# Leonhard111/M3L

Hardware: AMD Instinct MI355X
Metric: MAE fwd+bwd samples/sec (image+tactile) (higher is better)
Workload: dtype bf16; 1 GPU; BASELINE configs[1]: VTT vision+tactile MAE, 64x64 RGB + 2x32x32 tactile, ViT-Tiny 192/12/3/768 + decoder 192/4/3/768, mask 0.75; batch_per_gpu=256, global_batch=256, parallelism=dp1, grad_allreduce=none (one rank), rccl_ranks=0, step=zero_grad + mask + fwd + bwd + grad all-reduce + Adam

## Files before the change

### include/m3l_amd.h

```cpp
#ifndef M3L_AMD_H
#define M3L_AMD_H
#include <stddef.h>
#include <stdint.h>

#ifdef __cplusplus
extern "C" {
#endif

#define M3L_MAX_TACTILES 8

typedef struct m3l_geom {
    int image_h, image_w, image_patch, image_channels;
    int tactile_h, tactile_w, tactile_patch, tactile_channels;
    int num_tactiles;
    int use_vision;
    int use_tactile;
} m3l_geom;

typedef struct m3l_tf_cfg {
    int dim, depth, heads, mlp_dim;
    int project_out;
    int dtype;
    int dim_head;
} m3l_tf_cfg;

typedef struct m3l_dropout {
    float p;
    uint64_t seed;
} m3l_dropout;

int m3l_version(void);
int m3l_last_error(char* buf, size_t n);
int m3l_set_rowln(int enable);
int m3l_set_attn_block(int mode);
int m3l_set_attn_bwd_heads(int mode);
int m3l_set_attn_t192_bwd_prefetch(int mode);
int m3l_set_enc_mega(int mode);
void m3l_set_attn_phase_buffer(void* dev_buf);
int m3l_set_defer_join(int on);
int m3l_set_wgrad_inline(int on);
int m3l_side_join(void* stream);
int m3l_comm_available(void);
int m3l_comm_unique_id(void* out128);
int m3l_comm_init(const void* id128, int rank, int world);
int m3l_comm_world(void);
int m3l_comm_allreduce(float* buf, size_t count, void* after_stream);
int m3l_comm_destroy(void);
int m3l_side_fork(void* after_stream, void** side_out);
int m3l_side_mark_pending(void);
void* m3l_side_stream(void);
int m3l_side_pending(void);
int m3l_set_drop_h(int on);
int m3l_set_t192(int on);
int m3l_set_t192_tt(int tt);
int m3l_set_residual_bf16(int on);
int m3l_set_t192_stagger(int lead_mask, int prio_mask);

int m3l_mask_counts(const m3l_geom* g, double ratio, int* counts_host);
int m3l_mask_sample(const m3l_geom* g, double ratio, int B, const float* const* noise, int64_t* masked, int64_t* unmasked,
                    void* stream);

int m3l_mask_sample_counts(const m3l_geom* g, int nm_img, int nm_tac, int B, const float* const* noise, int64_t* masked,
                           int64_t* unmasked, void* stream);

size_t m3l_embed_ws_bytes(const m3l_geom* g, int D, int dtype, int B, int L);
int m3l_embed_fwd(const m3l_geom* g, int D, int dtype, int B, int L, int cnt_img, const int64_t* idx, const float* image,
                  const float* const* tactiles, const void* const* tensors, void* ws, float* tokens, void* stream);
int m3l_embed_bwd(const m3l_geom* g, int D, int dtype, int B, int L, int cnt_img, const int64_t* idx, const float* image,
                  const float* const* tactiles, const void* const* tensors, void* ws, const float* dtokens, float* const* grads,
                  void* stream);

size_t m3l_transformer_ws_bytes(const m3l_tf_cfg* c, int B, int n);
int m3l_transformer_fwd(const m3l_tf_cfg* c, int B, int n, const float* x_in, const void* const* tensors, void* ws, void* y_t,
                        float* y32, void* stream);
int m3l_transformer_bwd(const m3l_tf_cfg* c, int B, int n, const float* x_in, const void* const* tensors, void* ws, const void* dy,
                        int dy_dtype, float* dx_in, float* const* grads, void* stream);

int m3l_transformer_bwd_range(const m3l_tf_cfg* c, int B, int n, const float* x_in, const void* const* tensors, void* ws,
                              const void* dy, int dy_dtype, float* dx_in, float* const* grads, int layer_hi, int layer_lo, void* stream);

size_t m3l_transformer_ws_bytes_dropout(const m3l_tf_cfg* c, int B, int n, const m3l_dropout* drop);
int m3l_transformer_fwd_dropout(const m3l_tf_cfg* c, int B, int n, const float* x_in, const void* const* tensors, void* ws, void* y_t,
                                float* y32, const m3l_dropout* drop, void* stream);
int m3l_transformer_bwd_dropout(const m3l_tf_cfg* c, int B, int n, const float* x_in, const void* const* tensors, void* ws, const void* dy,
                                int dy_dtype, float* dx_in, float* const* grads, const m3l_dropout* drop, void* stream);
int m3l_transformer_bwd_range_dropout(const m3l_tf_cfg* c, int B, int n, const float* x_in, const void* const* tensors, void* ws,
                                      const void* dy, int dy_dtype, float* dx_in, float* const* grads, int layer_hi, int layer_lo,
                                      const m3l_dropout* drop, void* stream);

enum {
    M3L_TF_PER_OP = 0,
    M3L_TF_BLOCK = 1,
    M3L_TF_T192 = 2,
    M3L_TF_ROWLN = 3,
    M3L_TF_IN_BLOCK = 4,
    M3L_TF_TAIL_T192 = 5,
    M3L_TF_IN_TAIL = 6,
    M3L_TF_GEMM = 7,
    M3L_TF_IDENTITY = 8
};
typedef struct m3l_tf_plan {
    int per_op;
    int rowln_cfg;
    int rowln;
    int rb;
    int drop_h;
    int h_from_u;
    int mega_fwd;
    int mega_bwd;
    int dropout;
    int fwd_attn;
    int fwd_outproj;
    int fwd_mlp;
    int bwd_mlp;
    int bwd_attn;
    int bwd_qkv;
    int row_tiles;
    int qkv_tiles;
    int cs_rows;
} m3l_tf_plan;
int m3l_transformer_plan(const m3l_tf_cfg* c, int B, int n, const m3l_dropout* drop, m3l_tf_plan* out);

size_t m3l_frozen_vit_ws_bytes(const m3l_tf_cfg* c, int B, int n);
int m3l_frozen_vit_fwd(const m3l_tf_cfg* c, float ln_eps, int B, int n, const float* x, const void* const* tensors, void* ws,
                       float* y32, void* stream);

size_t m3l_unshuffle_ws_bytes(const m3l_geom* g, int D, int dd, int dtype, int B, int nvis, int nmask);
int m3l_unshuffle_fwd(const m3l_geom* g, int D, int dd, int dtype, int B, int nvis, int nmask, const int64_t* unmasked,
                      const int64_t* masked, const float* enc32, const void* enc_t, const void* const* tensors, void* ws,
                      float* dec_in, void* stream);
int m3l_unshuffle_bwd(const m3l_geom* g, int D, int dd, int dtype, int B, int nvis, int nmask, const int64_t* unmasked,
                      const int64_t* masked, const void* enc_t, const void* const* tensors, void* ws, const float* d_dec_in,
                      void* d_enc, int* d_enc_dtype, float* const* grads, void* stream);

size_t m3l_heads_ws_bytes(const m3l_geom* g, int dd, int dtype, int B, int nmask);
int m3l_heads_loss_fwd(const m3l_geom* g, int dd, int dtype, int B, int N, int nmask, int nm_img, const int64_t* masked,
                       const float* image, const float* const* tactiles, const void* dec_t, const void* const* tensors, void* ws,
                       float* loss, float* pred_img, float* tgt_img, float* pred_tac, float* tgt_tac, void* stream);
int m3l_heads_loss_fwd2(const m3l_geom* g, int dd, int dtype, int B, int N, int nmask, int nm_img, const int64_t* masked,
                        const float* image, const float* const* tactiles, const void* dec_t, const void* const* tensors, void* ws,
                        float* loss, float* loss_parts, float* pred_img, float* tgt_img, float* pred_tac, float* tgt_tac, void* stream);
int m3l_heads_loss_bwd(const m3l_geom* g, int dd, int dtype, int B, int N, int nmask, int nm_img, const int64_t* masked,
                       const void* const* tensors, void* ws, const float* dloss, void* d_dec, float* const* grads, void* stream);

typedef struct m3l_mae_cfg {
    m3l_geom geom;
    m3l_tf_cfg enc, dec;
    double masking_ratio;
    int early_conv;
    int learned_pos;
} m3l_mae_cfg;
typedef struct m3l_comm_plan {
    float* flat;
    long total, min_bucket;
    int layers_per_chunk, n_stages;
    const long* stage_end;
    long* sent_out;
} m3l_comm_plan;
int m3l_mae_step_num_tensors(const m3l_mae_cfg* c);
size_t m3l_mae_step_ws_bytes(const m3l_mae_cfg* c, int B);
int m3l_mae_step_fwd(const m3l_mae_cfg* c, int B, const float* image, const float* const* tactiles, const float* const* noise,
                     const void* const* tensors, void* ws, float* loss, int64_t* masked, int64_t* unmasked, void* stream);
int m3l_mae_step_bwd(const m3l_mae_cfg* c, int B, const float* image, const float* const* tactiles, const int64_t* masked,
                     const int64_t* unmasked, const void* const* tensors, void* ws, const float* dloss, float* const* grads,
                     const m3l_comm_plan* comm, void* stream);
size_t m3l_mae_step_ws_bytes_dropout(const m3l_mae_cfg* c, int B, const m3l_dropout* enc_drop);
int m3l_mae_step_fwd_dropout(const m3l_mae_cfg* c, int B, const float* image, const float* const* tactiles, const float* const* noise,
                             const void* const* tensors, void* ws, float* loss, int64_t* masked, int64_t* unmasked, const m3l_dropout* enc_drop,
                             void* stream);
int m3l_mae_step_bwd_dropout(const m3l_mae_cfg* c, int B, const float* image, const float* const* tactiles, const int64_t* masked,
                             const int64_t* unmasked, const void* const* tensors, void* ws, const float* dloss, float* const* grads,
                             const m3l_comm_plan* comm, const m3l_dropout* enc_drop, void* stream);

int m3l_extractor_num_tensors(const m3l_mae_cfg* c, const m3l_tf_cfg* head);
size_t m3l_extractor_ws_bytes(const m3l_mae_cfg* c, const m3l_tf_cfg* head, int B);
int m3l_extractor_fwd(const m3l_mae_cfg* c, const m3l_tf_cfg* head, int B, const float* image, const float* const* tactiles,
                      const void* const* tensors, void* ws, float* out, void* stream);
int m3l_extractor_bwd(const m3l_mae_cfg* c, const m3l_tf_cfg* head, int B, const float* image, const float* const* tactiles,
                      const void* const* tensors, void* ws, const float* dout, float* const* grads, void* stream);
size_t m3l_extractor_ws_bytes_dropout(const m3l_mae_cfg* c, const m3l_tf_cfg* head, int B, const m3l_dropout* enc_drop, const m3l_dropout* head_drop);
int m3l_extractor_fwd_dropout(const m3l_mae_cfg* c, const m3l_tf_cfg* head, int B, const float* image, const float* const* tactiles,
                              const void* const* tensors, void* ws, float* out, const m3l_dropout* enc_drop, const m3l_dropout* head_drop,
                              void* stream);
int m3l_extractor_bwd_dropout(const m3l_mae_cfg* c, const m3l_tf_cfg* head, int B, const float* image, const float* const* tactiles,
                              const void* const* tensors, void* ws, const float* dout, float* const* grads, const m3l_dropout* enc_drop,
                              const m3l_dropout* head_drop, void* stream);

typedef struct m3l_cnn_cfg {
    int in_channels, height, width, dim;
    int tactile;
    int dtype;
} m3l_cnn_cfg;
int m3l_set_direct_conv(int on);
size_t m3l_earlycnn_ws_bytes(const m3l_cnn_cfg* c, int B, int nsrc);
int m3l_earlycnn_fwd(const m3l_cnn_cfg* c, int B, int nsrc, const float* const* srcs, const void* const* tensors, void* ws, float* out,
                     void* stream);
int m3l_earlycnn_bwd(const m3l_cnn_cfg* c, int B, int nsrc, const float* const* srcs, const void* const* tensors, void* ws, const float* dout,
                     float* const* grads, void* stream);
size_t m3l_tokens_assemble_ws_bytes(const m3l_geom* g, int D);
int m3l_tokens_assemble_fwd(const m3l_geom* g, int D, int B, const float* img_tok, const float* tac_tok, const void* const* tensors,
                            float* tokens, void* stream);
int m3l_tokens_assemble_bwd(const m3l_geom* g, int D, int B, const float* dtokens, float* d_img, float* d_tac, void* ws, float* dmod,
                            void* stream);

size_t m3l_layernorm_ws_bytes(int D);
int m3l_layernorm_fwd(int out_dtype, const float* x, int M, int D, const float* gamma, const float* beta, float eps, void* y,
                      float* y32, void* stream);
int m3l_layernorm_bwd(int dy_dtype, const void* dy, const float* x, int M, int D, const float* gamma, float eps, const float* dres,
                      float* dx, void* ws, float* dgamma, float* dbeta, void* stream);
int m3l_gather_tokens(const float* src, int B, int N, int D, const int64_t* idx, int K, float* dst, void* stream);
int m3l_scatter_tokens(const float* src, int B, int N, int D, const int64_t* idx, int K, float* dst_zeroed, void* stream);
int m3l_vt_load(const float* image_nhwc, int B, int H, int W, int C, float* image_nchw, const float* tactile, int th, int tw,
                int n_sensors, int frame_stack, float* const* tactile_out, void* stream);
int m3l_vt_load2(const void* image_nhwc, int image_u8, int B, int H, int W, int C, double img_lo, double img_hi, float* image_nchw,
                 const void* tactile, int tactile_u8, int th, int tw, int n_sensors, int frame_stack, double tac_lo, double tac_hi,
                 float* const* tactile_out, void* stream);

int m3l_adam_step(float* params, const float* grads, float* exp_avg, float* exp_avg_sq, long n, float lr, float beta1, float beta2,
                  float eps, float weight_decay, int step, void* stream);
int m3l_adam_step_scaled(float* params, const float* grads, float* exp_avg, float* exp_avg_sq, long n, float lr, float beta1, float beta2,
                         float eps, float weight_decay, int step, float grad_scale, void* stream);
int m3l_adamw_step(float* params, float* grads, float* exp_avg, float* exp_avg_sq, long n, float lr, float beta1, float beta2, float eps,
                   float weight_decay, int step, float grad_scale, float max_grad_norm, float* norm_ws, int scale_grads, void* stream);
int m3l_adam_step_dev(float* params, const float* grads, float* exp_avg, float* exp_avg_sq, long n, float lr, float beta1,
                      float beta2, float eps, float weight_decay, int* step_dev, float* bias_corr_dev, void* stream);
int m3l_dino_opt_step(float* params, float* grads, float* exp_avg, float* exp_avg_sq, float* teacher, long n, const int64_t* seg_start,
                      const int32_t* seg_group, int n_segments, const float* group_lr, const float* group_weight_decay, int n_groups,
                      double beta1, double beta2, float eps, int step, float grad_scale, float max_grad_norm, float* norm_ws, int scale_grads,
                      double ema_beta, void* stream);

void m3l_prof_begin(const char* filter, int stride);
void m3l_prof_end(void);
double m3l_prof_event_overhead_us(void* stream, int n);
int m3l_prof_count(void);
int m3l_prof_get(int i, char* name, size_t n, double* ms_total, long* launches, double* flops_total, double* bytes_total);

int m3l_op_gemm_nt(int dtype, const void* A, int lda, const void* W, int ldw, int M, int N, int K, const float* bias,
                   const float* res, float* out_f32, void* out_t, void* out_pre, const void* gelu_u, int act, int ldc, void* stream);
size_t m3l_op_gemm_tn_ws_bytes(int M, int N, int K);
int m3l_op_gemm_tn(int dtype, const void* Y, int ldy, const void* X, int ldx, int M, int N, int K, void* ws, size_t ws_bytes,
                   float* out, int ldo, void* stream);
int m3l_op_gemm_tn_acc(int dtype, const void* Y, int ldy, const void* X, int ldx, int M, int N, int K, void* ws, size_t ws_bytes, float* out, int ldo,
                       int accumulate, void* stream);
size_t m3l_op_gemm_tn_grouped_ws_bytes(int dtype, int count, int M, const int* N, const int* K);
int m3l_op_gemm_tn_grouped(int dtype, int count, int M, const void* const* Y, const int* ldy, const void* const* X, const int* ldx, const int* N,
                           const int* K, float* const* out, void* ws, size_t ws_bytes, void* stream);
size_t m3l_op_colsum_ws_bytes(int N);
int m3l_op_colsum(int dtype, const void* Y, int M, int N, int ld, void* ws, float* out, void* stream);
int m3l_op_prep_weight(int dtype, const float* src, int rows, int cols, void* dst, void* dstT, void* stream);
int m3l_op_mask_scale(int mode, const float* src, const void* ref, float scale, long count, float* out, void* stream);
int m3l_op_concat2(float* a, int na, float* b, int nb, int rows, float* cat, int split, void* stream);
int m3l_op_patch_cols(int dtype, const float* x, int B, int C, int H, int W, int P, int Kpad, void* col, void* stream);
int m3l_op_vit_tokens(const float* emb, const float* cls, const float* regs, const float* pos, int B, int npatch, int R, int D, float* tok,
                      void* stream);
int m3l_op_attn_fwd(int dtype, const void* qkv, void* o, float* lse, int B, int n, int H, void* stream);
int m3l_op_attn_bwd(int dtype, const void* qkv, const void* o, const void* dO, const float* lse, float* dsum, void* dqkv, int B,
                    int n, int H, void* stream);
int m3l_op_attn_fwd_dh(int dtype, const void* qkv, void* o, float* lse, int B, int n, int H, void* stream, int dim_head);
int m3l_op_attn_bwd_dh(int dtype, const void* qkv, const void* o, const void* dO, const float* lse, float* dsum, void* dqkv, int B,
                       int n, int H, void* stream, int dim_head);
int m3l_op_dropout_mask(float p, uint64_t seed, int layer, int site, long rows, int N, uint8_t* out, void* stream);

int m3l_op_l2norm_fwd(int out_dtype, const float* x, int M, int D, float eps, void* y, float* y32, float* norm, void* stream);
int m3l_op_l2norm_bwd(const float* dy, const float* x, const float* norm, int M, int D, float eps, float* dx, void* stream);
int m3l_op_weightnorm_fwd(int dtype, const float* v, const float* g, int K, int D, void* W, float* vnorm, void* stream);
int m3l_op_weightnorm_bwd(const float* dW, const float* v, const float* g, const float* vnorm, int K, int D, float* dv, float* dg, void* stream);
size_t m3l_op_dino_ws_bytes(int rows, int K);
int m3l_op_dino_rowstats(const float* logits, int rows, int K, const float* center, float inv_temp, void* ws, float* stats, void* stream);
int m3l_op_dino_loss(const float* S, int P, const float* T, int Q, int B, int K, const float* center, float inv_ts, float inv_tt, const float* s_stats,
                     const float* t_stats, void* ws, float* loss, void* stream);
int m3l_op_dino_grad(int out_dtype, const float* S, int P, const float* T, int Q, int B, int K, const float* center, float inv_ts, float inv_tt,
                     const float* s_stats, const float* t_stats, const float* dloss, void* dST, int ldr, void* stream);
int m3l_op_dino_center_sum(const float* T, int rows, int K, float* pending, void* stream);
int m3l_op_dino_center_apply(float* center, const float* pending, int K, float momentum, float one_minus_momentum, float count, void* stream);
int m3l_op_sk_row_splits(int rows, int K);
size_t m3l_op_sk_ws_bytes(int rows, int K);
int m3l_op_sk_colstats(const float* logits, int rows, int K, float inv_temp, const float* row_stats, void* ws, float* col_pairs, void* stream);
int m3l_op_sk_colcombine(const float* parts, int nparts, int K, float temp, float* center_out, void* stream);
int m3l_op_sk_probs(const float* logits, int rows, int K, const float* center, float inv_temp, const float* row_stats, float* probs, void* stream);
size_t m3l_op_koleo_ws_bytes(int groups, int n, int D);
int m3l_op_koleo_fwd(const float* x, int groups, int n, int D, float eps, void* ws, float* y, float* norm, int* nn, long long* nn64, float* dist,
                     float* loss, void* stream);
int m3l_op_koleo_bwd(const float* dloss, const float* x, const float* y, const float* norm, const int* nn, const float* dist, int groups, int n, int D,
                     float eps, float* dx, void* stream);
size_t m3l_op_ibot_ws_bytes(int rows, int K);
int m3l_op_ibot_loss(const float* S, const float* T, int Q, int R, int K, const float* center, float inv_ts, float inv_tt, const float* s_stats,
                     const float* t_stats, void* ws, float* loss, void* stream);
int m3l_op_ibot_grad(int out_dtype, const float* S, const float* T, int Q, int R, int K, const float* center, float inv_ts, float inv_tt,
                     const float* s_stats, const float* t_stats, const float* dloss, void* dST, int ldr, void* stream);
int m3l_op_ibot_center_sum(const float* T, int rows, int K, float scale, void* ws, float* pending, void* stream);
int m3l_op_ema(float* const* dst, const float* const* src, const long* len, int count, float beta, float one_minus_beta, void* stream);

#define M3L_POLICY_MAX_HIDDEN 3
typedef struct m3l_policy_desc {
    int features, actions;
    int n_pi, n_vf;
    int pi_width[M3L_POLICY_MAX_HIDDEN], vf_width[M3L_POLICY_MAX_HIDDEN];
    float* pi_weight[M3L_POLICY_MAX_HIDDEN];
    float* pi_bias[M3L_POLICY_MAX_HIDDEN];
    float* vf_weight[M3L_POLICY_MAX_HIDDEN];
    float* vf_bias[M3L_POLICY_MAX_HIDDEN];
    float* action_weight;
    float* action_bias;
    float* value_weight;
    float* value_bias;
    float* log_std;
} m3l_policy_desc;
size_t m3l_policy_ws_bytes(const m3l_policy_desc* head, int B);
int m3l_policy_act(const m3l_policy_desc* head, int B, const float* x, const float* noise, float* actions, float* values, float* logp, void* stream);
int m3l_policy_eval_fwd(const m3l_policy_desc* head, int B, const float* x, const float* actions, void* ws, float* values, float* logp, float* entropy,
                        void* stream);
int m3l_policy_eval_bwd(const m3l_policy_desc* head, int B, const float* x, const float* actions, const float* dvalues, const float* dlogp,
                        const float* dentropy, void* ws, float* dx, const m3l_policy_desc* grads, void* stream);
int m3l_policy_ppo_loss_fwd(const float* logp, const float* values, const float* entropy, const float* old_logp, const float* advantages, const float* returns,
                            const float* old_values, int B, float clip_range, float clip_range_vf, float ent_coef, float vf_coef, int normalize_advantage,
                            float* loss, float* stats, float* coef_logp, float* coef_values, void* stream);
int m3l_policy_ppo_loss_bwd(const float* dloss, const float* coef_logp, const float* coef_values, int B, float ent_coef, float* dlogp, float* dvalues,
                            float* dentropy, void* stream);

#define M3L_SAC_MAX_HIDDEN 3
typedef struct m3l_sac_desc {
    int features, actions;
    int n_pi, n_qf;
    int pi_width[M3L_SAC_MAX_HIDDEN], qf_width[M3L_SAC_MAX_HIDDEN];
    float* pi_weight[M3L_SAC_MAX_HIDDEN];
    float* pi_bias[M3L_SAC_MAX_HIDDEN];
    float* mu_weight;
    float* mu_bias;
    float* log_std_weight;
    float* log_std_bias;
    float* qf_weight[2][M3L_SAC_MAX_HIDDEN];
    float* qf_bias[2][M3L_SAC_MAX_HIDDEN];
    float* q_weight[2];
    float* q_bias[2];
} m3l_sac_desc;
size_t m3l_sac_ws_bytes(const m3l_sac_desc* head, int B);
int m3l_sac_actor_fwd(const m3l_sac_desc* head, int B, const float* x, const float* noise, void* ws, float* actions, float* logp, void* stream);
int m3l_sac_actor_bwd(const m3l_sac_desc* head, int B, const float* x, const float* noise, const float* dactions, const float* dlogp, void* ws,
                      float* dx, const m3l_sac_desc* grads, void* stream);
int m3l_sac_critic_fwd(const m3l_sac_desc* head, int B, const float* x, const float* actions, void* ws, float* q, void* stream);
int m3l_sac_critic_bwd(const m3l_sac_desc* head, int B, const float* dq, void* ws, float* dactions, const m3l_sac_desc* grads, void* stream);
int m3l_sac_td_target(const m3l_sac_desc* head, int B, const float* x_next, const float* noise, const float* rewards, const float* dones, float gamma,
                      float ent_coef, const float* log_ent_coef, float* target_q, void* stream);
int m3l_sac_critic_loss_fwd(const float* q, const float* target_q, int B, float* loss, float* coef, void* stream);
int m3l_sac_critic_loss_bwd(const float* dloss, const float* coef, int B, float* dq, void* stream);
int m3l_sac_actor_loss_fwd(const float* logp, const float* q, int B, float ent_coef, const float* log_ent_coef, float* loss, float* coef, void* stream);
int m3l_sac_actor_loss_bwd(const float* dloss, const float* coef, int B, float* dlogp_dq, void* stream);
int m3l_sac_ent_coef_loss(const float* log_ent_coef, const float* logp, float target_entropy, int B, const float* dloss, float* loss, float* ent_coef,
                          float* dlog_ent_coef, void* stream);

int m3l_rollout_gather_load(const void* image_store, int image_u8, int H, int W, double img_lo, double img_hi, float* image,
                            const void* tactile_store, int tactile_u8, int th, int tw, int n_sensors, double tac_lo, double tac_hi,
                            float* const* tactile_out, int T, int n_envs, int frame_stack, const int64_t* idx, int B, void* stream);
int m3l_rollout_gather_rows(const float* actions, const float* values, const float* log_probs, const float* advantages, const float* returns, int T,
                            int n_envs, int A, const int64_t* idx, int B, float* actions_out, float* values_out, float* log_probs_out,
                            float* advantages_out, float* returns_out, void* stream);
int m3l_rollout_gae(const float* rewards, const float* values, const float* episode_starts, const float* last_values, const float* dones, int T,
                    int n_envs, float gamma, float gae_lambda, float* advantages, float* returns, void* stream);

int m3l_replay_gather_load(const void* image_store, const void* image_next_store, int image_u8, int H, int W, double img_lo, double img_hi,
                           float* image, float* image_next, const void* tactile_store, const void* tactile_next_store, int tactile_u8, int th, int tw,
                           int n_sensors, double tac_lo, double tac_hi, float* const* tactile_out, float* const* tactile_next_out, int T, int n_envs,
                           int frame_stack, const int64_t* rows, long row_shift, int B, void* stream);
int m3l_replay_gather_rows(const float* actions, const float* rewards, const float* dones, const float* timeouts, int T, int n_envs, int A,
                           const int64_t* rows, long row_shift, int B, float reward_scale, float reward_clip, float* actions_out,
                           float* rewards_out, float* dones_out, int64_t* rows_out, void* stream);

int m3l_replay_gather_load_frames(const void* image_frames, const void* image_next_frames, int image_u8, int H, int W, double img_lo,
                                  double img_hi, float* image, float* image_next, const void* tactile_frames, const void* tactile_next_frames,
                                  int tactile_u8, int th, int tw, int n_sensors, double tac_lo, double tac_hi, float* const* tactile_out,
                                  float* const* tactile_next_out, const int32_t* ages, int T, int n_envs, int frame_stack, const int64_t* rows,
                                  long row_shift, int B, void* stream);

#ifdef __cplusplus
}
#endif
#endif
```

### m3l_amd/_lib.py

```python
import ctypes as C
import os

_HERE = os.path.dirname(os.path.abspath(__file__))
LIB_PATH = os.environ.get("M3L_LIB_PATH") or os.path.join(_HERE, "lib", "libm3l_amd.so")

c_p = C.c_void_p
c_i = C.c_int
c_sz = C.c_size_t


class Geom(C.Structure):
    _fields_ = [(n, c_i) for n in ("image_h", "image_w", "image_patch", "image_channels", "tactile_h", "tactile_w",
                                   "tactile_patch", "tactile_channels", "num_tactiles", "use_vision", "use_tactile")]


class CnnCfg(C.Structure):
    _fields_ = [(n, c_i) for n in ("in_channels", "height", "width", "dim", "tactile", "dtype")]


class TfCfg(C.Structure):
    _fields_ = [(n, c_i) for n in ("dim", "depth", "heads", "mlp_dim", "project_out", "dtype", "dim_head")]


class MaeCfg(C.Structure):
    _fields_ = [("geom", Geom), ("enc", TfCfg), ("dec", TfCfg), ("masking_ratio", C.c_double), ("early_conv", c_i), ("learned_pos", c_i)]


class Dropout(C.Structure):
    _fields_ = [("p", C.c_float), ("seed", C.c_uint64)]


class TfPlan(C.Structure):
    _fields_ = [(n, c_i) for n in ("per_op", "rowln_cfg", "rowln", "rb", "drop_h", "h_from_u", "mega_fwd", "mega_bwd", "dropout",
                                   "fwd_attn", "fwd_outproj", "fwd_mlp", "bwd_mlp", "bwd_attn", "bwd_qkv", "row_tiles", "qkv_tiles", "cs_rows")]


TF_PER_OP, TF_BLOCK, TF_T192, TF_ROWLN, TF_IN_BLOCK, TF_TAIL_T192, TF_IN_TAIL, TF_GEMM, TF_IDENTITY = range(9)


class CommPlan(C.Structure):
    _fields_ = [("flat", c_p), ("total", C.c_long), ("min_bucket", C.c_long), ("layers_per_chunk", c_i), ("n_stages", c_i),
                ("stage_end", C.POINTER(C.c_long)), ("sent_out", C.POINTER(C.c_long))]


class PolicyDesc(C.Structure):
    _fields_ = [("features", c_i), ("actions", c_i), ("n_pi", c_i), ("n_vf", c_i), ("pi_width", c_i * 3), ("vf_width", c_i * 3),
                ("pi_weight", c_p * 3), ("pi_bias", c_p * 3), ("vf_weight", c_p * 3), ("vf_bias", c_p * 3),
                ("action_weight", c_p), ("action_bias", c_p), ("value_weight", c_p), ("value_bias", c_p), ("log_std", c_p)]


class SacDesc(C.Structure):
    _fields_ = [("features", c_i), ("actions", c_i), ("n_pi", c_i), ("n_qf", c_i), ("pi_width", c_i * 3), ("qf_width", c_i * 3),
                ("pi_weight", c_p * 3), ("pi_bias", c_p * 3), ("mu_weight", c_p), ("mu_bias", c_p), ("log_std_weight", c_p), ("log_std_bias", c_p),
                ("qf_weight", (c_p * 3) * 2), ("qf_bias", (c_p * 3) * 2), ("q_weight", c_p * 2), ("q_bias", c_p * 2)]


_SIGS = {
    "m3l_version": (c_i, []),
    "m3l_last_error": (c_i, [C.c_char_p, c_sz]),
    "m3l_set_rowln": (c_i, [c_i]),
    "m3l_set_attn_block": (c_i, [c_i]),
    "m3l_set_attn_phase_buffer": (None, [c_p]),
    "m3l_set_attn_bwd_heads": (c_i, [c_i]),
    "m3l_set_attn_t192_bwd_prefetch": (c_i, [c_i]),
    "m3l_set_enc_mega": (c_i, [c_i]),
    "m3l_set_drop_h": (c_i, [c_i]),
    "m3l_set_direct_conv": (c_i, [c_i]),
    "m3l_set_t192": (c_i, [c_i]),
    "m3l_set_t192_tt": (c_i, [c_i]),
    "m3l_set_t192_stagger": (c_i, [c_i, c_i]),
    "m3l_set_residual_bf16": (c_i, [c_i]),
    "m3l_set_defer_join": (c_i, [c_i]),
    "m3l_set_wgrad_inline": (c_i, [c_i]),
    "m3l_side_join": (c_i, [c_p]),
    "m3l_side_stream": (c_p, []),
    "m3l_side_fork": (c_i, [c_p, C.POINTER(c_p)]),
    "m3l_side_mark_pending": (c_i, []),
    "m3l_comm_available": (c_i, []),
    "m3l_comm_unique_id": (c_i, [c_p]),
    "m3l_comm_init": (c_i, [c_p, c_i, c_i]),
    "m3l_comm_world": (c_i, []),
    "m3l_comm_allreduce": (c_i, [c_p, c_sz, c_p]),
    "m3l_comm_destroy": (c_i, []),
    "m3l_side_pending": (c_i, []),
    "m3l_mask_counts": (c_i, [C.POINTER(Geom), C.c_double, C.POINTER(c_i)]),
    "m3l_mask_sample": (c_i, [C.POINTER(Geom), C.c_double, c_i, c_p, c_p, c_p, c_p]),
    "m3l_mask_sample_counts": (c_i, [C.POINTER(Geom), c_i, c_i, c_i, c_p, c_p, c_p, c_p]),
    "m3l_embed_ws_bytes": (c_sz, [C.POINTER(Geom), c_i, c_i, c_i, c_i]),
    "m3l_embed_fwd": (c_i, [C.POINTER(Geom), c_i, c_i, c_i, c_i, c_i, c_p, c_p, c_p, c_p, c_p, c_p, c_p]),
    "m3l_embed_bwd": (c_i, [C.POINTER(Geom), c_i, c_i, c_i, c_i, c_i, c_p, c_p, c_p, c_p, c_p, c_p, c_p, c_p]),
    "m3l_transformer_ws_bytes": (c_sz, [C.POINTER(TfCfg), c_i, c_i]),
    "m3l_transformer_fwd": (c_i, [C.POINTER(TfCfg), c_i, c_i, c_p, c_p, c_p, c_p, c_p, c_p]),
    "m3l_transformer_bwd": (c_i, [C.POINTER(TfCfg), c_i, c_i, c_p, c_p, c_p, c_p, c_i, c_p, c_p, c_p]),
    "m3l_transformer_bwd_range": (c_i, [C.POINTER(TfCfg), c_i, c_i, c_p, c_p, c_p, c_p, c_i, c_p, c_p, c_i, c_i, c_p]),
    "m3l_transformer_ws_bytes_dropout": (c_sz, [C.POINTER(TfCfg), c_i, c_i, C.POINTER(Dropout)]),
    "m3l_transformer_fwd_dropout": (c_i, [C.POINTER(TfCfg), c_i, c_i, c_p, c_p, c_p, c_p, c_p, C.POINTER(Dropout), c_p]),
    "m3l_transformer_bwd_dropout": (c_i, [C.POINTER(TfCfg), c_i, c_i, c_p, c_p, c_p, c_p, c_i, c_p, c_p, C.POINTER(Dropout), c_p]),
    "m3l_transformer_bwd_range_dropout": (c_i, [C.POINTER(TfCfg), c_i, c_i, c_p, c_p, c_p, c_p, c_i, c_p, c_p, c_i, c_i, C.POINTER(Dropout), c_p]),
    "m3l_transformer_plan": (c_i, [C.POINTER(TfCfg), c_i, c_i, C.POINTER(Dropout), C.POINTER(TfPlan)]),
    "m3l_frozen_vit_ws_bytes": (c_sz, [C.POINTER(TfCfg), c_i, c_i]),
    "m3l_frozen_vit_fwd": (c_i, [C.POINTER(TfCfg), C.c_float, c_i, c_i, c_p, c_p, c_p, c_p, c_p]),
    "m3l_unshuffle_ws_bytes": (c_sz, [C.POINTER(Geom), c_i, c_i, c_i, c_i, c_i, c_i]),
    "m3l_unshuffle_fwd": (c_i, [C.POINTER(Geom), c_i, c_i, c_i, c_i, c_i, c_i, c_p, c_p, c_p, c_p, c_p, c_p, c_p, c_p]),
    "m3l_unshuffle_bwd": (c_i, [C.POINTER(Geom), c_i, c_i, c_i, c_i, c_i, c_i, c_p, c_p, c_p, c_p, c_p, c_p, c_p,
                                C.POINTER(c_i), c_p, c_p]),
    "m3l_heads_ws_bytes": (c_sz, [C.POINTER(Geom), c_i, c_i, c_i, c_i]),
    "m3l_heads_loss_fwd": (c_i, [C.POINTER(Geom), c_i, c_i, c_i, c_i, c_i, c_i, c_p, c_p, c_p, c_p, c_p, c_p, c_p, c_p, c_p,
                                 c_p, c_p, c_p]),
    "m3l_heads_loss_fwd2": (c_i, [C.POINTER(Geom), c_i, c_i, c_i, c_i, c_i, c_i, c_p, c_p, c_p, c_p, c_p, c_p, c_p, c_p, c_p,
                                  c_p, c_p, c_p, c_p]),
    "m3l_heads_loss_bwd": (c_i, [C.POINTER(Geom), c_i, c_i, c_i, c_i, c_i, c_i, c_p, c_p, c_p, c_p, c_p, c_p, c_p]),
    "m3l_mae_step_num_tensors": (c_i, [C.POINTER(MaeCfg)]),
    "m3l_mae_step_ws_bytes": (c_sz, [C.POINTER(MaeCfg), c_i]),
    "m3l_mae_step_fwd": (c_i, [C.POINTER(MaeCfg), c_i, c_p, c_p, c_p, c_p, c_p, c_p, c_p, c_p, c_p]),
    "m3l_mae_step_bwd": (c_i, [C.POINTER(MaeCfg), c_i, c_p, c_p, c_p, c_p, c_p, c_p, c_p, c_p, C.POINTER(CommPlan), c_p]),
    "m3l_mae_step_ws_bytes_dropout": (c_sz, [C.POINTER(MaeCfg), c_i, C.POINTER(Dropout)]),
    "m3l_mae_step_fwd_dropout": (c_i, [C.POINTER(MaeCfg), c_i, c_p, c_p, c_p, c_p, c_p, c_p, c_p, c_p, C.POINTER(Dropout), c_p]),
    "m3l_mae_step_bwd_dropout": (c_i, [C.POINTER(MaeCfg), c_i, c_p, c_p, c_p, c_p, c_p, c_p, c_p, c_p, C.POINTER(CommPlan), C.POINTER(Dropout), c_p]),
    "m3l_extractor_num_tensors": (c_i, [C.POINTER(MaeCfg), C.POINTER(TfCfg)]),
    "m3l_extractor_ws_bytes": (c_sz, [C.POINTER(MaeCfg), C.POINTER(TfCfg), c_i]),
    "m3l_extractor_fwd": (c_i, [C.POINTER(MaeCfg), C.POINTER(TfCfg), c_i, c_p, c_p, c_p, c_p, c_p, c_p]),
    "m3l_extractor_bwd": (c_i, [C.POINTER(MaeCfg), C.POINTER(TfCfg), c_i, c_p, c_p, c_p, c_p, c_p, c_p, c_p]),
    "m3l_extractor_ws_bytes_dropout": (c_sz, [C.POINTER(MaeCfg), C.POINTER(TfCfg), c_i, C.POINTER(Dropout), C.POINTER(Dropout)]),
    "m3l_extractor_fwd_dropout": (c_i, [C.POINTER(MaeCfg), C.POINTER(TfCfg), c_i, c_p, c_p, c_p, c_p, c_p, C.POINTER(Dropout), C.POINTER(Dropout), c_p]),
    "m3l_extractor_bwd_dropout": (c_i, [C.POINTER(MaeCfg), C.POINTER(TfCfg), c_i, c_p, c_p, c_p, c_p, c_p, c_p, C.POINTER(Dropout), C.POINTER(Dropout), c_p]),
    "m3l_earlycnn_ws_bytes": (c_sz, [C.POINTER(CnnCfg), c_i, c_i]),
    "m3l_earlycnn_fwd": (c_i, [C.POINTER(CnnCfg), c_i, c_i, c_p, c_p, c_p, c_p, c_p]),
    "m3l_earlycnn_bwd": (c_i, [C.POINTER(CnnCfg), c_i, c_i, c_p, c_p, c_p, c_p, c_p, c_p]),
    "m3l_tokens_assemble_ws_bytes": (c_sz, [C.POINTER(Geom), c_i]),
    "m3l_tokens_assemble_fwd": (c_i, [C.POINTER(Geom), c_i, c_i, c_p, c_p, c_p, c_p, c_p]),
    "m3l_tokens_assemble_bwd": (c_i, [C.POINTER(Geom), c_i, c_i, c_p, c_p, c_p, c_p, c_p, c_p]),
    "m3l_layernorm_ws_bytes": (c_sz, [c_i]),
    "m3l_layernorm_fwd": (c_i, [c_i, c_p, c_i, c_i, c_p, c_p, C.c_float, c_p, c_p, c_p]),
    "m3l_layernorm_bwd": (c_i, [c_i, c_p, c_p, c_i, c_i, c_p, C.c_float, c_p, c_p, c_p, c_p, c_p, c_p]),
    "m3l_gather_tokens": (c_i, [c_p, c_i, c_i, c_i, c_p, c_i, c_p, c_p]),
    "m3l_scatter_tokens": (c_i, [c_p, c_i, c_i, c_i, c_p, c_i, c_p, c_p]),
    "m3l_vt_load": (c_i, [c_p, c_i, c_i, c_i, c_i, c_p, c_p, c_i, c_i, c_i, c_i, c_p, c_p]),
    "m3l_vt_load2": (c_i, [c_p, c_i, c_i, c_i, c_i, c_i, C.c_double, C.c_double, c_p, c_p, c_i, c_i, c_i, c_i, c_i, C.c_double, C.c_double, c_p, c_p]),
    "m3l_adam_step_dev": (c_i, [c_p, c_p, c_p, c_p, C.c_long, C.c_float, C.c_float, C.c_float, C.c_float, C.c_float, c_p, c_p, c_p]),
    "m3l_adamw_step": (c_i, [c_p, c_p, c_p, c_p, C.c_long, C.c_float, C.c_float, C.c_float, C.c_float, C.c_float, c_i, C.c_float, C.c_float, c_p, c_i, c_p]),
    "m3l_adam_step": (c_i, [c_p, c_p, c_p, c_p, C.c_long, C.c_float, C.c_float, C.c_float, C.c_float, C.c_float, c_i, c_p]),
    "m3l_adam_step_scaled": (c_i, [c_p, c_p, c_p, c_p, C.c_long, C.c_float, C.c_float, C.c_float, C.c_float, C.c_float, c_i, C.c_float, c_p]),
    "m3l_dino_opt_step": (c_i, [c_p, c_p, c_p, c_p, c_p, C.c_long, c_p, c_p, c_i, C.POINTER(C.c_float), C.POINTER(C.c_float), c_i,
                                C.c_double, C.c_double, C.c_float, c_i, C.c_float, C.c_float, c_p, c_i, C.c_double, c_p]),
    "m3l_prof_begin": (None, [C.c_char_p, c_i]),
    "m3l_prof_end": (None, []),
    "m3l_prof_event_overhead_us": (C.c_double, [c_p, c_i]),
    "m3l_prof_count": (c_i, []),
    "m3l_prof_get": (c_i, [c_i, C.c_char_p, c_sz, C.POINTER(C.c_double), C.POINTER(C.c_long), C.POINTER(C.c_double),
                           C.POINTER(C.c_double)]),
    "m3l_op_gemm_nt": (c_i, [c_i, c_p, c_i, c_p, c_i, c_i, c_i, c_i, c_p, c_p, c_p, c_p, c_p, c_p, c_i, c_i, c_p]),
    "m3l_op_gemm_tn_ws_bytes": (c_sz, [c_i, c_i, c_i]),
    "m3l_op_gemm_tn": (c_i, [c_i, c_p, c_i, c_p, c_i, c_i, c_i, c_i, c_p, c_sz, c_p, c_i, c_p]),
    "m3l_op_gemm_tn_acc": (c_i, [c_i, c_p, c_i, c_p, c_i, c_i, c_i, c_i, c_p, c_sz, c_p, c_i, c_i, c_p]),
    "m3l_op_gemm_tn_grouped_ws_bytes": (c_sz, [c_i, c_i, c_i, c_p, c_p]),
    "m3l_op_gemm_tn_grouped": (c_i, [c_i, c_i, c_i, c_p, c_p, c_p, c_p, c_p, c_p, c_p, c_p, c_sz, c_p]),
    "m3l_op_colsum_ws_bytes": (c_sz, [c_i]),
    "m3l_op_colsum": (c_i, [c_i, c_p, c_i, c_i, c_i, c_p, c_p, c_p]),
    "m3l_op_prep_weight": (c_i, [c_i, c_p, c_i, c_i, c_p, c_p, c_p]),
    "m3l_op_mask_scale": (c_i, [c_i, c_p, c_p, C.c_float, C.c_long, c_p, c_p]),
    "m3l_op_concat2": (c_i, [c_p, c_i, c_p, c_i, c_i, c_p, c_i, c_p]),
    "m3l_op_patch_cols": (c_i, [c_i, c_p, c_i, c_i, c_i, c_i, c_i, c_i, c_p, c_p]),
    "m3l_op_vit_tokens": (c_i, [c_p, c_p, c_p, c_p, c_i, c_i, c_i, c_i, c_p, c_p]),
    "m3l_op_attn_fwd": (c_i, [c_i, c_p, c_p, c_p, c_i, c_i, c_i, c_p]),
    "m3l_op_attn_bwd": (c_i, [c_i, c_p, c_p, c_p, c_p, c_p, c_p, c_i, c_i, c_i, c_p]),
    "m3l_op_attn_fwd_dh": (c_i, [c_i, c_p, c_p, c_p, c_i, c_i, c_i, c_p, c_i]),
    "m3l_op_attn_bwd_dh": (c_i, [c_i, c_p, c_p, c_p, c_p, c_p, c_p, c_i, c_i, c_i, c_p, c_i]),
    "m3l_op_dropout_mask": (c_i, [C.c_float, C.c_uint64, c_i, c_i, C.c_long, c_i, c_p, c_p]),
    "m3l_op_l2norm_fwd": (c_i, [c_i, c_p, c_i, c_i, C.c_float, c_p, c_p, c_p, c_p]),
    "m3l_op_l2norm_bwd": (c_i, [c_p, c_p, c_p, c_i, c_i, C.c_float, c_p, c_p]),
    "m3l_op_weightnorm_fwd": (c_i, [c_i, c_p, c_p, c_i, c_i, c_p, c_p, c_p]),
    "m3l_op_weightnorm_bwd": (c_i, [c_p, c_p, c_p, c_p, c_i, c_i, c_p, c_p, c_p]),
    "m3l_op_dino_ws_bytes": (c_sz, [c_i, c_i]),
    "m3l_op_dino_rowstats": (c_i, [c_p, c_i, c_i, c_p, C.c_float, c_p, c_p, c_p]),
    "m3l_op_dino_loss": (c_i, [c_p, c_i, c_p, c_i, c_i, c_i, c_p, C.c_float, C.c_float, c_p, c_p, c_p, c_p, c_p]),
    "m3l_op_dino_grad": (c_i, [c_i, c_p, c_i, c_p, c_i, c_i, c_i, c_p, C.c_float, C.c_float, c_p, c_p, c_p, c_p, c_i, c_p]),
    "m3l_op_dino_center_sum": (c_i, [c_p, c_i, c_i, c_p, c_p]),
    "m3l_op_dino_center_apply": (c_i, [c_p, c_p, c_i, C.c_float, C.c_float, C.c_float, c_p]),
    "m3l_op_sk_row_splits": (c_i, [c_i, c_i]),
    "m3l_op_sk_ws_bytes": (c_sz, [c_i, c_i]),
    "m3l_op_sk_colstats": (c_i, [c_p, c_i, c_i, C.c_float, c_p, c_p, c_p, c_p]),
    "m3l_op_sk_colcombine": (c_i, [c_p, c_i, c_i, C.c_float, c_p, c_p]),
    "m3l_op_sk_probs": (c_i, [c_p, c_i, c_i, c_p, C.c_float, c_p, c_p, c_p]),
    "m3l_op_koleo_ws_bytes": (c_sz, [c_i, c_i, c_i]),
    "m3l_op_koleo_fwd": (c_i, [c_p, c_i, c_i, c_i, C.c_float, c_p, c_p, c_p, c_p, c_p, c_p, c_p, c_p]),
    "m3l_op_koleo_bwd": (c_i, [c_p, c_p, c_p, c_p, c_p, c_p, c_i, c_i, c_i, C.c_float, c_p, c_p]),
    "m3l_op_ibot_ws_bytes": (c_sz, [c_i, c_i]),
    "m3l_op_ibot_loss": (c_i, [c_p, c_p, c_i, c_i, c_i, c_p, C.c_float, C.c_float, c_p, c_p, c_p, c_p, c_p]),
    "m3l_op_ibot_grad": (c_i, [c_i, c_p, c_p, c_i, c_i, c_i, c_p, C.c_float, C.c_float, c_p, c_p, c_p, c_p, c_i, c_p]),
    "m3l_op_ibot_center_sum": (c_i, [c_p, c_i, c_i, C.c_float, c_p, c_p, c_p]),
    "m3l_op_ema": (c_i, [c_p, c_p, c_p, c_i, C.c_float, C.c_float, c_p]),
    "m3l_policy_ws_bytes": (c_sz, [C.POINTER(PolicyDesc), c_i]),
    "m3l_policy_act": (c_i, [C.POINTER(PolicyDesc), c_i, c_p, c_p, c_p, c_p, c_p, c_p]),
    "m3l_policy_eval_fwd": (c_i, [C.POINTER(PolicyDesc), c_i, c_p, c_p, c_p, c_p, c_p, c_p, c_p]),
    "m3l_policy_eval_bwd": (c_i, [C.POINTER(PolicyDesc), c_i, c_p, c_p, c_p, c_p, c_p, c_p, c_p, C.POINTER(PolicyDesc), c_p]),
    "m3l_policy_ppo_loss_fwd": (c_i, [c_p, c_p, c_p, c_p, c_p, c_p, c_p, c_i, C.c_float, C.c_float, C.c_float, C.c_float, c_i, c_p, c_p, c_p, c_p, c_p]),
    "m3l_policy_ppo_loss_bwd": (c_i, [c_p, c_p, c_p, c_i, C.c_float, c_p, c_p, c_p, c_p]),
    "m3l_sac_ws_bytes": (c_sz, [C.POINTER(SacDesc), c_i]),
    "m3l_sac_actor_fwd": (c_i, [C.POINTER(SacDesc), c_i, c_p, c_p, c_p, c_p, c_p, c_p]),
    "m3l_sac_actor_bwd": (c_i, [C.POINTER(SacDesc), c_i, c_p, c_p, c_p, c_p, c_p, c_p, C.POINTER(SacDesc), c_p]),
    "m3l_sac_critic_fwd": (c_i, [C.POINTER(SacDesc), c_i, c_p, c_p, c_p, c_p, c_p]),
    "m3l_sac_critic_bwd": (c_i, [C.POINTER(SacDesc), c_i, c_p, c_p, c_p, C.POINTER(SacDesc), c_p]),
    "m3l_sac_td_target": (c_i, [C.POINTER(SacDesc), c_i, c_p, c_p, c_p, c_p, C.c_float, C.c_float, c_p, c_p, c_p]),
    "m3l_sac_critic_loss_fwd": (c_i, [c_p, c_p, c_i, c_p, c_p, c_p]),
    "m3l_sac_critic_loss_bwd": (c_i, [c_p, c_p, c_i, c_p, c_p]),
    "m3l_sac_actor_loss_fwd": (c_i, [c_p, c_p, c_i, C.c_float, c_p, c_p, c_p, c_p]),
    "m3l_sac_actor_loss_bwd": (c_i, [c_p, c_p, c_i, c_p, c_p]),
    "m3l_sac_ent_coef_loss": (c_i, [c_p, c_p, C.c_float, c_i, c_p, c_p, c_p, c_p, c_p]),
    "m3l_rollout_gather_load": (c_i, [c_p, c_i, c_i, c_i, C.c_double, C.c_double, c_p, c_p, c_i, c_i, c_i, c_i, C.c_double, C.c_double, c_p,
                                      c_i, c_i, c_i, c_p, c_i, c_p]),
    "m3l_rollout_gather_rows": (c_i, [c_p, c_p, c_p, c_p, c_p, c_i, c_i, c_i, c_p, c_i, c_p, c_p, c_p, c_p, c_p, c_p]),
    "m3l_rollout_gae": (c_i, [c_p, c_p, c_p, c_p, c_p, c_i, c_i, C.c_float, C.c_float, c_p, c_p, c_p]),
    "m3l_replay_gather_load": (c_i, [c_p, c_p, c_i, c_i, c_i, C.c_double, C.c_double, c_p, c_p, c_p, c_p, c_i, c_i, c_i, c_i, C.c_double, C.c_double,
                                     c_p, c_p, c_i, c_i, c_i, c_p, C.c_long, c_i, c_p]),
    "m3l_replay_gather_rows": (c_i, [c_p, c_p, c_p, c_p, c_i, c_i, c_i, c_p, C.c_long, c_i, C.c_float, C.c_float, c_p, c_p, c_p, c_p, c_p]),
    "m3l_replay_gather_load_frames": (c_i, [c_p, c_p, c_i, c_i, c_i, C.c_double, C.c_double, c_p, c_p, c_p, c_p, c_i, c_i, c_i, c_i, C.c_double,
                                            C.c_double, c_p, c_p, c_p, c_i, c_i, c_i, c_p, C.c_long, c_i, c_p]),
}

EXPORTS = tuple(_SIGS.keys())
_lib = None


class M3LError(RuntimeError):
    pass


def lib():
    global _lib
    if _lib is None:
        if not os.path.exists(LIB_PATH):
            raise M3LError(
                f"{LIB_PATH} not found: the HIP extension has not been built. Run "
                "`python -c \"import __graft_entry__ as g; g.build()\"` (needs hipcc, --offload-arch=gfx950). "
                "m3l_amd has no CPU / eager fallback.")
        l = C.CDLL(LIB_PATH)
        for name, (res, args) in _SIGS.items():
            fn = getattr(l, name)
            fn.restype = res
            fn.argtypes = args
        _lib = l
    return _lib


def last_error() -> str:
    buf = C.create_string_buffer(512)
    lib().m3l_last_error(buf, 512)
    return buf.value.decode("utf-8", "replace")


def check(rc: int, what: str):
    if rc != 0:
        raise M3LError(f"{what} failed (code {rc}): {last_error()}")


def ptr(t):
    return None if t is None else t.data_ptr()


def ptr_array(tensors):
    arr = (c_p * max(1, len(tensors)))()
    for i, t in enumerate(tensors):
        arr[i] = None if t is None else t.data_ptr()
    return arr
```

### m3l_amd/csrc/elementwise.hip

```cpp
#include "common.cuh"
#include "kernels.h"
#include <cstring>
#include <vector>

namespace {

constexpr int MAXV = 16;
constexpr int WPB = 4;

__device__ __forceinline__ void store_val(float* p, float v) { *p = v; }
__device__ __forceinline__ void store_val(bf16* p, float v) { *p = (bf16)v; }


template <typename TO> __device__ __forceinline__ void store4(TO* p, f32x4 v);
template <> __device__ __forceinline__ void store4<float>(float* p, f32x4 v) { *reinterpret_cast<f32x4*>(p) = v; }
template <> __device__ __forceinline__ void store4<bf16>(bf16* p, f32x4 v) {
    bf16x4 o;
    o[0] = (bf16)v[0]; o[1] = (bf16)v[1]; o[2] = (bf16)v[2]; o[3] = (bf16)v[3];
    *reinterpret_cast<bf16x4*>(p) = o;
}
__device__ __forceinline__ f32x4 load4(const float* p) { return *reinterpret_cast<const f32x4*>(p); }
__device__ __forceinline__ f32x4 load4(const bf16* p) {
    const bf16x4 v = *reinterpret_cast<const bf16x4*>(p);
    return f32x4{(float)v[0], (float)v[1], (float)v[2], (float)v[3]};
}

template <int MAXC, typename TX>
__device__ __forceinline__ void row_stats(const TX* xr, int D, int lane, f32x4 (&v)[MAXC], float eps, float& mean, float& rstd) {
    float s = 0.f;
#pragma unroll
    for (int i = 0; i < MAXC; ++i) {
        const int e = 4 * (lane + 64 * i);
        v[i] = load4(xr + min(e, D - 4));
        if (e >= D) v[i] = f32x4{0.f, 0.f, 0.f, 0.f};
        s += (v[i][0] + v[i][1]) + (v[i][2] + v[i][3]);
    }
    mean = wave_sum(s) / D;
    float q = 0.f;
#pragma unroll
    for (int i = 0; i < MAXC; ++i) {
        const int e = 4 * (lane + 64 * i);
        if (e < D) {
            const f32x4 d = v[i] - mean;
            q += (d[0] * d[0] + d[1] * d[1]) + (d[2] * d[2] + d[3] * d[3]);
        }
    }
    rstd = rsqrtf(wave_sum(q) / D + eps);
}

template <typename TO, int MAXC, typename TX>
__global__ __launch_bounds__(256) void ln_fwd_kernel(const TX* __restrict__ x, int M, int D, const float* __restrict__ gamma,
                                                       const float* __restrict__ beta, float eps, TO* __restrict__ y,
                                                       float* __restrict__ y32) {
    const int lane = threadIdx.x & 63, row = blockIdx.x * WPB + (threadIdx.x >> 6);
    if (row >= M) return;
    f32x4 v[MAXC], gm[MAXC], bt[MAXC];
#pragma unroll
    for (int i = 0; i < MAXC; ++i) {
        const int ec = min(4 * (lane + 64 * i), D - 4);
        gm[i] = load4(gamma + ec);
        bt[i] = load4(beta + ec);
    }
    float mean, rstd;
    row_stats<MAXC>(x + (long)row * D, D, lane, v, eps, mean, rstd);
#pragma unroll
    for (int i = 0; i < MAXC; ++i) {
        const int e = 4 * (lane + 64 * i);
        if (e < D) {
            const f32x4 r = (v[i] - mean) * rstd * gm[i] + bt[i];
            if (y) store4<TO>(y + (long)row * D + e, r);
            if (y32) store4<float>(y32 + (long)row * D + e, r);
        }
    }
}

template <typename TD, typename TC, int MAXC, typename TX>
__global__ __launch_bounds__(256) void ln_bwd_kernel(const TD* __restrict__ dy, const TX* __restrict__ x, int M, int D,
                                                       const float* __restrict__ gamma, float eps, const float* __restrict__ dres,
                                                       float* __restrict__ dx_out, TC* __restrict__ dx_t_out, float* __restrict__ part) {
    __shared__ __attribute__((aligned(16))) float red[WPB][3][256];
    const int lane = threadIdx.x & 63, wave = threadIdx.x >> 6;
    f32x4 dg[MAXC], db[MAXC], dc[MAXC];
#pragma unroll
    for (int i = 0; i < MAXC; ++i) dg[i] = db[i] = dc[i] = f32x4{0.f, 0.f, 0.f, 0.f};
    f32x4 gm[MAXC];
#pragma unroll
    for (int i = 0; i < MAXC; ++i) gm[i] = load4(gamma + min(4 * (lane + 64 * i), D - 4));
    for (int row = blockIdx.x * WPB + wave; row < M; row += gridDim.x * WPB) {
        f32x4 v[MAXC], gdy[MAXC], dyv[MAXC], rs[MAXC];
        const TD* dyr = dy + (long)row * D;
#pragma unroll
        for (int i = 0; i < MAXC; ++i) {
            const int ec = min(4 * (lane + 64 * i), D - 4);
            dyv[i] = load4(dyr + ec);
            rs[i] = dres ? load4(reinterpret_cast<const TX*>(dres) + (long)row * D + ec) : f32x4{0.f, 0.f, 0.f, 0.f};
        }
        float mean, rstd;
        row_stats<MAXC>(x + (long)row * D, D, lane, v, eps, mean, rstd);
        float s1 = 0.f, s2 = 0.f;
#pragma unroll
        for (int i = 0; i < MAXC; ++i) {
            const int e = 4 * (lane + 64 * i);
            if (e < D) {
                const f32x4 xh = (v[i] - mean) * rstd;
                const f32x4 d = dyv[i];
                dg[i] += d * xh;
                db[i] += d;
                const f32x4 gd = d * gm[i];
                gdy[i] = gd;
                v[i] = xh;
                s1 += (gd[0] + gd[1]) + (gd[2] + gd[3]);
                const f32x4 t = gd * xh;
                s2 += (t[0] + t[1]) + (t[2] + t[3]);
            }
        }
        s1 = wave_sum(s1) / D;
        s2 = wave_sum(s2) / D;
#pragma unroll
        for (int i = 0; i < MAXC; ++i) {
            const int e = 4 * (lane + 64 * i);
            if (e < D) {
                f32x4 r = (gdy[i] - s1 - v[i] * s2) * rstd;
                if (dres) r += rs[i];
                dc[i] += r;
                if (dx_out) store4<float>(dx_out + (long)row * D + e, r);
                if (dx_t_out) store4<TC>(dx_t_out + (long)row * D + e, r);
            }
        }
    }
    float* out = part + (long)blockIdx.x * 3 * D;
#pragma unroll
    for (int i = 0; i < MAXC; ++i) {
        if (256 * i >= D) break;
        *reinterpret_cast<f32x4*>(&red[wave][0][4 * lane]) = dg[i];
        *reinterpret_cast<f32x4*>(&red[wave][1][4 * lane]) = db[i];
        *reinterpret_cast<f32x4*>(&red[wave][2][4 * lane]) = dc[i];
        __syncthreads();
        const int e = 256 * i + threadIdx.x;
        if (e < D) {
#pragma unroll
            for (int k = 0; k < 3; ++k)
                out[k * D + e] = (red[0][k][threadIdx.x] + red[1][k][threadIdx.x]) + (red[2][k][threadIdx.x] + red[3][k][threadIdx.x]);
        }
        __syncthreads();
    }
}

__device__ __forceinline__ void reduce_cols_32x32(const float* __restrict__ p, int G, int stride, int j, bool valid,
                                                  float* __restrict__ out, int accumulate) {
    __shared__ float red[32][33];
    const int cl = threadIdx.x & 31, sl = threadIdx.x >> 5;
    float s = 0.f;
    if (valid) {
        float a[8] = {0.f, 0.f, 0.f, 0.f, 0.f, 0.f, 0.f, 0.f};
        int g = sl;
        for (; g + 224 < G; g += 256) {
#pragma unroll
            for (int u = 0; u < 8; ++u) a[u] += p[(long)(g + 32 * u) * stride + j];
        }
        for (; g < G; g += 32) a[0] += p[(long)g * stride + j];
        s = ((a[0] + a[1]) + (a[2] + a[3])) + ((a[4] + a[5]) + (a[6] + a[7]));
    }
    red[sl][cl] = s;
    __syncthreads();
    if (sl == 0 && valid) {
        float t = red[0][cl];
#pragma unroll
        for (int i = 1; i < 32; ++i) t += red[i][cl];
        out[j] = accumulate ? out[j] + t : t;
    }
}

__global__ __launch_bounds__(1024) void reduce_rows_kernel(const float* __restrict__ part, int G, int stride, int count,
                                                             float* __restrict__ out, int accumulate) {
    const int j = blockIdx.x * 32 + (threadIdx.x & 31);
    reduce_cols_32x32(part, G, stride, j, j < count, out, accumulate);
}

__global__ __launch_bounds__(1024) void reduce_vec_kernel(const float* __restrict__ v, int G, float* __restrict__ out, int accumulate) {
    __shared__ float red[16];
    float a0 = 0.f, a1 = 0.f, a2 = 0.f, a3 = 0.f;
    int i = threadIdx.x;
    for (; i + 3072 < G; i += 4096) { a0 += v[i]; a1 += v[i + 1024]; a2 += v[i + 2048]; a3 += v[i + 3072]; }
    for (; i < G; i += 1024) a0 += v[i];
    float s = wave_sum((a0 + a1) + (a2 + a3));
    if ((threadIdx.x & 63) == 0) red[threadIdx.x >> 6] = s;
    __syncthreads();
    if (threadIdx.x == 0) {
        float t = 0.f;
#pragma unroll
        for (int w = 0; w < 16; ++w) t += red[w];
        out[0] = accumulate ? out[0] + t : t;
    }
}

struct ReduceSegs { float* out[4]; };
__global__ __launch_bounds__(1024) void reduce_rows_seg_kernel(const float* __restrict__ part, int G, int stride, int width,
                                                                 ReduceSegs segs, int accumulate) {
    float* out = segs.out[blockIdx.y];
    if (!out) return;
    const int j = blockIdx.x * 32 + (threadIdx.x & 31);
    reduce_cols_32x32(part + (long)blockIdx.y * width, G, stride, j, j < width, out, accumulate);
}

__global__ __launch_bounds__(1024) void reduce_rows_batch_kernel(ReduceBatch b, int accumulate) {
    const ReduceBatchItem it = b.it[blockIdx.z];
    float* out = it.out[blockIdx.y];
    if (!out) return;
    const int j = blockIdx.x * 32 + (threadIdx.x & 31);
    reduce_cols_32x32(it.part + (long)blockIdx.y * b.D, it.G, 3 * b.D, j, j < b.D, out, accumulate);
}

template <typename T> struct Vec4;
template <> struct Vec4<bf16> { typedef bf16x4 type; };
template <> struct Vec4<float> { typedef f32x4 type; };
template <typename T>
__global__ __launch_bounds__(256) void colsum_kernel(const T* __restrict__ Y, int M, int N, int ld, int rows_per_block,
                                                       float* __restrict__ part, int vec_ok) {
    typedef typename Vec4<T>::type V4;
    const int r0 = blockIdx.x * rows_per_block, r1 = min(M, r0 + rows_per_block);
    for (int c = threadIdx.x * 4; c < N; c += 1024) {
        if (vec_ok && c + 4 <= N) {
            f32x4 s0 = f32x4{0.f, 0.f, 0.f, 0.f}, s1 = s0, s2 = s0, s3 = s0;
            auto ld4 = [&](int r) {
                const V4 v = *reinterpret_cast<const V4*>(Y + (long)r * ld + c);
                return f32x4{to_f32(v[0]), to_f32(v[1]), to_f32(v[2]), to_f32(v[3])};
            };
            int r = r0;
            for (; r + 3 < r1; r += 4) {
                s0 += ld4(r);
                s1 += ld4(r + 1);
                s2 += ld4(r + 2);
                s3 += ld4(r + 3);
            }
            for (; r < r1; ++r) s0 += ld4(r);
            *reinterpret_cast<f32x4*>(part + (long)blockIdx.x * N + c) = (s0 + s1) + (s2 + s3);
        } else {
            for (int cc = c; cc < min(N, c + 4); ++cc) {
                float s0 = 0.f, s1 = 0.f, s2 = 0.f, s3 = 0.f;
                int r = r0;
                for (; r + 3 < r1; r += 4) {
                    s0 += to_f32(Y[(long)r * ld + cc]);
                    s1 += to_f32(Y[(long)(r + 1) * ld + cc]);
                    s2 += to_f32(Y[(long)(r + 2) * ld + cc]);
                    s3 += to_f32(Y[(long)(r + 3) * ld + cc]);
                }
                for (; r < r1; ++r) s0 += to_f32(Y[(long)r * ld + cc]);
                part[(long)blockIdx.x * N + cc] = (s0 + s1) + (s2 + s3);
            }
        }
    }
}

template <typename T>
__global__ __launch_bounds__(256) void prep_weights_kernel(WeightPack pack) {
    __shared__ float tile[64][65];
    int m = 0;
    while (m + 1 < pack.count && (int)blockIdx.x >= pack.tile0[m + 1]) ++m;
    const WeightDesc d = pack.d[m];
    const int tcols = (d.cols + 63) >> 6;
    const int t = blockIdx.x - pack.tile0[m];
    const int r0 = (t / tcols) << 6, c0 = (t % tcols) << 6;
    const int tid = threadIdx.x, q = tid & 15, p = tid >> 4;
    T* dst = reinterpret_cast<T*>(d.dst);
    T* dstT = reinterpret_cast<T*>(d.dstT);
    const bool vec_in = (d.cols & 3) == 0 && (reinterpret_cast<uintptr_t>(d.src) & 15) == 0;
#pragma unroll
    for (int k = 0; k < 4; ++k) {
        const int r = r0 + p + 16 * k, c = c0 + 4 * q;
        float v[4] = {0.f, 0.f, 0.f, 0.f};
        if (r < d.rows) {
            if (vec_in && c + 3 < d.cols) {
                const float4 f = *reinterpret_cast<const float4*>(d.src + (long)r * d.cols + c);
                v[0] = f.x; v[1] = f.y; v[2] = f.z; v[3] = f.w;
            } else {
#pragma unroll
                for (int j = 0; j < 4; ++j)
                    if (c + j < d.cols) v[j] = d.src[(long)r * d.cols + c + j];
            }
        }
        if (dst && r < d.ld_dstT) {
#pragma unroll
            for (int j = 0; j < 4; ++j)
                if (c + j < d.ld_dst) dst[(long)r * d.ld_dst + c + j] = from_f32<T>(v[j]);
        }
#pragma unroll
        for (int j = 0; j < 4; ++j) tile[p + 16 * k][4 * q + j] = v[j];
    }
    if (!dstT) return;
    __syncthreads();
#pragma unroll
    for (int k = 0; k < 4; ++k) {
        const int c = c0 + p + 16 * k, r = r0 + 4 * q;
        if (c >= d.ld_dst) continue;
#pragma unroll
        for (int j = 0; j < 4; ++j)
            if (r + j < d.ld_dstT) dstT[(long)c * d.ld_dstT + r + j] = from_f32<T>(tile[4 * q + j][p + 16 * k]);
    }
}

template <typename T>
__global__ void axpy_t_kernel(const float* __restrict__ x, const T* __restrict__ o, long count, float* __restrict__ out) {
    const long i = (long)blockIdx.x * blockDim.x + threadIdx.x;
    if (i < count) out[i] = x[i] + to_f32(o[i]);
}
template <typename T>
__global__ void cast_kernel(const float* __restrict__ x, long count, T* __restrict__ out) {
    const long i = (long)blockIdx.x * blockDim.x + threadIdx.x;
    if (i < count) out[i] = from_f32<T>(x[i]);
}

template <typename T>
__global__ void scale_by_dev_kernel(const T* __restrict__ x, long count, const float* __restrict__ s, T* __restrict__ out) {
    const long i = (long)blockIdx.x * blockDim.x + threadIdx.x;
    if (i < count) out[i] = from_f32<T>(to_f32(x[i]) * s[0]);
}

template <int MODE>
__global__ void mask_scale_kernel(const float* __restrict__ src, const void* __restrict__ ref, float scale, long count, float* __restrict__ out) {
    const long i = (long)blockIdx.x * blockDim.x + threadIdx.x;
    if (i >= count) return;
    const bool on = MODE == 0 ? reinterpret_cast<const uint8_t*>(ref)[i] != 0 : reinterpret_cast<const float*>(ref)[i] > 0.f;
    out[i] = on ? src[i] * scale : 0.f;
}
__global__ void vit_tokens_kernel(const float* __restrict__ emb, const float* __restrict__ cls, const float* __restrict__ regs,
                                  const float* __restrict__ pos, int B, int npatch, int R, int D, float* __restrict__ tok) {
    const long i = (long)blockIdx.x * blockDim.x + threadIdx.x;
    const int n = 1 + R + npatch;
    if (i >= (long)B * n * D) return;
    const int d = (int)(i % D), t = (int)((i / D) % n), b = (int)(i / ((long)D * n));
    float v;
    if (t == 0) v = cls[d] + pos[d];
    else if (t <= R) v = regs[(long)(t - 1) * D + d];
    else v = emb[((long)b * npatch + (t - 1 - R)) * D + d] + pos[(long)(t - R) * D + d];
    tok[i] = v;
}
__global__ void concat2_kernel(const float* __restrict__ a, int na, const float* __restrict__ b2, int nb, int rows, float* __restrict__ dst, int split) {
    const long i = (long)blockIdx.x * blockDim.x + threadIdx.x;
    const int w = na + nb;
    if (i >= (long)rows * w) return;
    const int r = (int)(i / w), c = (int)(i % w);
    if (!split) dst[i] = c < na ? a[(long)r * na + c] : b2[(long)r * nb + c - na];
    else if (c < na) const_cast<float*>(a)[(long)r * na + c] = dst[i];
    else if (b2) const_cast<float*>(b2)[(long)r * nb + c - na] = dst[i];
}

template <typename T>
__global__ void im2col_kernel(ConvSrc cs, int Bsrc, int Ci, int H, int W, int KH, int S, int P, int OH, int OW, int Kpad,
                              long total, T* __restrict__ col) {
    const long idx = (long)blockIdx.x * blockDim.x + threadIdx.x;
    if (idx >= total) return;
    const int k = (int)(idx % Kpad);
    const long r = idx / Kpad;
    const int ow = (int)(r % OW), oh = (int)((r / OW) % OH);
    const int b = (int)(r / ((long)OW * OH));
    float v = 0.f;
    if (k < Ci * KH * KH) {
        const int kw = k % KH, kh = (k / KH) % KH, ci = k / (KH * KH);
        const int ih = oh * S + kh - P, iw = ow * S + kw - P;
        if (ih >= 0 && ih < H && iw >= 0 && iw < W) {
            if (cs.nchw) {
                const float* src = reinterpret_cast<const float*>(cs.src[b / Bsrc]);
                v = src[(((long)(b % Bsrc) * Ci + ci) * H + ih) * W + iw];
            } else {
                v = to_f32(reinterpret_cast<const T*>(cs.src[0])[(((long)b * H + ih) * W + iw) * Ci + ci]);
            }
        }
    }
    col[idx] = from_f32<T>(v);
}

__global__ __launch_bounds__(256) void im2col4_bf16_kernel(ConvSrc cs, int Bsrc, int Ci, int H, int W, int S, int P, int OH, int OW, long total,
                                                           bf16* __restrict__ col) {
    const long idx = (long)blockIdx.x * blockDim.x + threadIdx.x;
    if (idx >= total) return;
    const int ci = (int)(idx % Ci);
    const long r = idx / Ci;
    const int ow = (int)(r % OW), oh = (int)((r / OW) % OH);
    const int b = (int)(r / ((long)OW * OH));
    bf16x8 out[2];
#pragma unroll
    for (int kh = 0; kh < 4; ++kh) {
        const int ih = oh * S + kh - P;
        const bool rok = ih >= 0 && ih < H;
#pragma unroll
        for (int kw = 0; kw < 4; ++kw) {
            const int iw = ow * S + kw - P;
            float v = 0.f;
            if (rok && iw >= 0 && iw < W) {
                if (cs.nchw) v = reinterpret_cast<const float*>(cs.src[b / Bsrc])[(((long)(b % Bsrc) * Ci + ci) * H + ih) * W + iw];
                else v = (float)reinterpret_cast<const bf16*>(cs.src[0])[(((long)b * H + ih) * W + iw) * Ci + ci];
            }
            out[kh >> 1][(kh & 1) * 4 + kw] = (bf16)v;
        }
    }
    bf16x8* dst = reinterpret_cast<bf16x8*>(col + (r * Ci + ci) * 16);
    dst[0] = out[0];
    dst[1] = out[1];
}

template <typename T>
__global__ void col2im_relu_kernel(const T* __restrict__ dcol, int Btot, int Ci, int H, int W, int KH, int S, int P, int OH, int OW,
                                   int Kpad, const T* __restrict__ act, T* __restrict__ dX) {
    const long idx = (long)blockIdx.x * blockDim.x + threadIdx.x;
    if (idx >= (long)Btot * H * W * Ci) return;
    const int ci = (int)(idx % Ci);
    const long pix = idx / Ci;
    const int iw = (int)(pix % W), ih = (int)((pix / W) % H);
    const int b = (int)(pix / ((long)W * H));
    float s = 0.f;
    if (to_f32(act[idx]) > 0.f) {
        for (int kh = 0; kh < KH; ++kh) {
            const int t = ih + P - kh;
            if (t < 0 || t % S) continue;
            const int oh = t / S;
            if (oh >= OH) continue;
            for (int kw = 0; kw < KH; ++kw) {
                const int u = iw + P - kw;
                if (u < 0 || u % S) continue;
                const int ow = u / S;
                if (ow >= OW) continue;
                s += to_f32(dcol[(((long)b * OH + oh) * OW + ow) * Kpad + (ci * KH + kh) * KH + kw]);
            }
        }
    }
    dX[idx] = from_f32<T>(s);
}

__global__ __launch_bounds__(256) void tokens_assemble_kernel(const float* __restrict__ img_tok, const float* __restrict__ tac_tok, int B,
                                                                int D, int n_img, int n_tac, int k, const float* __restrict__ mod,
                                                                const float* __restrict__ pos_img, const float* __restrict__ pos_tac,
                                                                float* __restrict__ tokens) {
    const int lane = threadIdx.x & 63;
    const long r = (long)blockIdx.x * WPB + (threadIdx.x >> 6);
    const int N = n_img + k * n_tac;
    if (r >= (long)B * N) return;
    const int b = (int)(r / N), pos = (int)(r % N);
    const float *src, *prow;
    int m;
    if (pos < n_img) {
        src = img_tok + ((long)b * n_img + pos) * D;
        prow = pos_img + (long)pos * D;
        m = 0;
    } else {
        const int local = pos - n_img, s = local / n_tac, p = local % n_tac;
        src = tac_tok + (((long)s * B + b) * n_tac + p) * D;
        prow = pos_tac + (long)local * D;
        m = 1 + s;
    }
    float* out = tokens + r * D;
    for (int e = lane; e < D; e += 64) out[e] = src[e] + mod[(long)m * D + e] + prow[e];
}
__global__ __launch_bounds__(256) void tokens_assemble_bwd_kernel(const float* __restrict__ dtok, int B, int D, int n_img, int n_tac, int k,
                                                                    float* __restrict__ d_img, float* __restrict__ d_tac,
                                                                    float* __restrict__ part) {
    extern __shared__ float sm[];
    const int lane = threadIdx.x & 63, wave = threadIdx.x >> 6;
    const int N = n_img + k * n_tac, PL = (1 + k) * D;
    for (int i = threadIdx.x; i < WPB * PL; i += 256) sm[i] = 0.f;
    __syncthreads();
    float* my = sm + wave * PL;
    for (long r = (long)blockIdx.x * WPB + wave; r < (long)B * N; r += (long)gridDim.x * WPB) {
        const int b = (int)(r / N), pos = (int)(r % N);
        float* dst;
        int m;
        if (pos < n_img) {
            dst = d_img + ((long)b * n_img + pos) * D;
            m = 0;
        } else {
            const int local = pos - n_img, s = local / n_tac, p = local % n_tac;
            dst = d_tac + (((long)s * B + b) * n_tac + p) * D;
            m = 1 + s;
        }
        const float* g = dtok + r * D;
        for (int e = lane; e < D; e += 64) {
            const float d = g[e];
            dst[e] = d;
            my[m * D + e] += d;
        }
    }
    __syncthreads();
    for (int i = threadIdx.x; i < PL; i += 256)
        part[(long)blockIdx.x * PL + i] = sm[i] + sm[PL + i] + sm[2 * PL + i] + sm[3 * PL + i];
}

template <int DEC>
__device__ __forceinline__ void adam_elem(float& p, float& g, float& m, float& v, float gscale, float lr, float omb1, float b2, float omb2,
                                          float eps, float wd, float bc1, float bc2_sqrt) {
    g = g * gscale;
    if (DEC) p = p * wd;
    const float gr = DEC ? g : g + wd * p;
    m = m + (gr - m) * omb1;
    v = v * b2 + omb2 * gr * gr;
    const float denom = sqrtf(v) / bc2_sqrt + eps;
    p = p - (lr / bc1) * (m / denom);
}

template <int DEC>
__global__ void adam_flat_kernel(float* __restrict__ p, float* __restrict__ g, float* __restrict__ m, float* __restrict__ v,
                                 long n, float lr, float b1, float b2, float eps, float wd, float bc1, float bc2_sqrt,
                                 const float* __restrict__ bc_dev, float gscale, const float* __restrict__ clip_dev, int scale_g) {
    const long i = ((long)blockIdx.x * blockDim.x + threadIdx.x) * 4;
    if (i >= n) return;
    if (bc_dev) {
        bc1 = bc_dev[0];
        bc2_sqrt = bc_dev[1];
    }
    if (clip_dev) gscale *= clip_dev[0];
    if (i + 4 <= n) {
        f32x4 pp = *reinterpret_cast<f32x4*>(p + i), gg = *reinterpret_cast<const f32x4*>(g + i);
        f32x4 mm = *reinterpret_cast<f32x4*>(m + i), vv = *reinterpret_cast<f32x4*>(v + i);
#pragma unroll
        for (int j = 0; j < 4; ++j) {
// ... 338 lines not shown
                    }
                }
                dg[k] += d[k] * (a - mean) * rstd;
                db[k] += d[k];
            }
        }
        __syncthreads();
    }
    float* out = part + (long)blockIdx.x * 2 * pd;
#pragma unroll
    for (int pass = 0; pass < 2; ++pass) {
#pragma unroll
        for (int k = 0; k < NC; ++k) *reinterpret_cast<f32x4*>(my + 4 * (lane + 64 * k)) = pass ? db[k] : dg[k];
        __syncthreads();
        for (int e = threadIdx.x; e < pd; e += 256) out[pass * pd + e] = buf[0][e] + buf[1][e] + buf[2][e] + buf[3][e];
        __syncthreads();
    }
}

__global__ __launch_bounds__(256) void embed_finalize_kernel(const float* __restrict__ E, int rows, int D, PatchGroup pg,
                                                               const int64_t* __restrict__ idx, int idx_ld, int j0, int cnt,
                                                               const float* __restrict__ gamma, const float* __restrict__ beta,
                                                               float eps, const float* __restrict__ mod, int mod0,
                                                               const float* __restrict__ pos, float* __restrict__ tokens, int L) {
    const int lane = threadIdx.x & 63, row = blockIdx.x * WPB + (threadIdx.x >> 6);
    if (row >= rows) return;
    int b, s, ph, pw, local;
    patch_locate(pg, idx, idx_ld, j0, cnt, row, b, s, ph, pw, local);
    const float* xr = E + (long)row * D;
    float v[MAXV];
    float sum = 0.f;
#pragma unroll
    for (int i = 0; i < MAXV; ++i) {
        const int e = lane + 64 * i;
        v[i] = (e < D) ? xr[e] : 0.f;
        sum += v[i];
    }
    const float mean = wave_sum(sum) / D;
    float q = 0.f;
#pragma unroll
    for (int i = 0; i < MAXV; ++i) {
        const int e = lane + 64 * i;
        const float d = (e < D) ? v[i] - mean : 0.f;
        q += d * d;
    }
    const float rstd = rsqrtf(wave_sum(q) / D + eps);
    const int jj = row % cnt;
    float* out = tokens + ((long)b * L + j0 + jj) * D;
    const float* mrow = mod + (long)(mod0 + s) * D;
    const float* prow = pos + (long)local * D;
#pragma unroll
    for (int i = 0; i < MAXV; ++i) {
        const int e = lane + 64 * i;
        if (e < D) out[e] = (v[i] - mean) * rstd * gamma[e] + beta[e] + mrow[e] + prow[e];
    }
}

template <typename T>
__global__ __launch_bounds__(256) void embed_finalize_bwd_kernel(const float* __restrict__ dtok, int L, const float* __restrict__ E,
                                                                   int rows, int D, PatchGroup pg, const int64_t* __restrict__ idx,
                                                                   int idx_ld, int j0, int cnt, const float* __restrict__ gamma,
                                                                   float eps, T* __restrict__ dE, float* __restrict__ part, int nslot) {
    extern __shared__ float sm[];
    const int lane = threadIdx.x & 63, wave = threadIdx.x >> 6;
    const int PL = (2 + nslot) * D;
    for (int i = threadIdx.x; i < WPB * PL; i += 256) sm[i] = 0.f;
    __syncthreads();
    float* my = sm + wave * PL;
    for (int row = blockIdx.x * WPB + wave; row < rows; row += gridDim.x * WPB) {
        int b, s, ph, pw, local;
        patch_locate(pg, idx, idx_ld, j0, cnt, row, b, s, ph, pw, local);
        const int jj = row % cnt;
        const float* xr = E + (long)row * D;
        const float* dyr = dtok + ((long)b * L + j0 + jj) * D;
        float v[MAXV], gdy[MAXV];
        float sum = 0.f;
#pragma unroll
        for (int i = 0; i < MAXV; ++i) {
            const int e = lane + 64 * i;
            v[i] = (e < D) ? xr[e] : 0.f;
            sum += v[i];
        }
        const float mean = wave_sum(sum) / D;
        float q = 0.f;
#pragma unroll
        for (int i = 0; i < MAXV; ++i) {
            const int e = lane + 64 * i;
            const float d = (e < D) ? v[i] - mean : 0.f;
            q += d * d;
        }
        const float rstd = rsqrtf(wave_sum(q) / D + eps);
        float s1 = 0.f, s2 = 0.f;
#pragma unroll
        for (int i = 0; i < MAXV; ++i) {
            const int e = lane + 64 * i;
            if (e < D) {
                const float xh = (v[i] - mean) * rstd;
                const float d = dyr[e];
                my[e] += d * xh;
                my[D + e] += d;
                my[(2 + s) * D + e] += d;
                const float gd = d * gamma[e];
                gdy[i] = gd;
                v[i] = xh;
                s1 += gd;
                s2 += gd * xh;
            } else {
                gdy[i] = 0.f;
                v[i] = 0.f;
            }
        }
        s1 = wave_sum(s1) / D;
        s2 = wave_sum(s2) / D;
#pragma unroll
        for (int i = 0; i < MAXV; ++i) {
            const int e = lane + 64 * i;
            if (e < D) dE[(long)row * D + e] = from_f32<T>(rstd * (gdy[i] - s1 - v[i] * s2));
        }
    }
    __syncthreads();
    for (int i = threadIdx.x; i < PL; i += 256)
        part[(long)blockIdx.x * PL + i] = sm[i] + sm[PL + i] + sm[2 * PL + i] + sm[3 * PL + i];
}

template <typename TO>
__global__ __launch_bounds__(256) void unshuffle_fwd_kernel(const float* __restrict__ src, const float* __restrict__ mask_token,
                                                              const int64_t* __restrict__ unmasked, int nvis,
                                                              const int64_t* __restrict__ masked, int nmask, int B, int dd,
                                                              int n_img, int n_tac, const float* __restrict__ dmod,
                                                              const float* __restrict__ pos_img, const float* __restrict__ pos_tac,
                                                              TO* __restrict__ dec_in) {
    const int lane = threadIdx.x & 63;
    const long r = (long)blockIdx.x * WPB + (threadIdx.x >> 6);
    const int N = nvis + nmask;
    if (r >= (long)B * N) return;
    const int b = (int)(r / N), j = (int)(r % N);
    const bool vis = j < nvis;
    const int pos = (int)(vis ? unmasked[(long)b * nvis + j] : masked[(long)b * nmask + j - nvis]);
    const float* s = vis ? src + ((long)b * nvis + j) * dd : mask_token;
    const int m = pos < n_img ? 0 : 1 + (pos - n_img) / n_tac;
    const float* prow = pos < n_img ? pos_img + (long)pos * dd : pos_tac + (long)(pos - n_img) * dd;
    TO* out = dec_in + ((long)b * N + pos) * dd;
    const float* mrow = dmod + (long)m * dd;
    for (int e = 4 * lane; e < dd; e += 256) store4<TO>(out + e, load4(s + e) + load4(mrow + e) + load4(prow + e));
}

template <int MAXC, typename TI>
__global__ __launch_bounds__(256) void unshuffle_bwd_kernel(const TI* __restrict__ dY, const int64_t* __restrict__ unmasked, int nvis,
                                                              int B, int N, int dd, int n_img, int n_tac, int nmod, int rows_per_wave,
                                                              int vis_per_wave, float* __restrict__ dsrc, float* __restrict__ part) {
    extern __shared__ float sm[];
    const int lane = threadIdx.x & 63, wave = threadIdx.x >> 6;
    const int PL = (1 + nmod) * dd;
    for (int i = threadIdx.x; i < WPB * PL; i += 256) sm[i] = 0.f;
    __syncthreads();
    float* my = sm + wave * PL;
    const long gw = (long)blockIdx.x * WPB + wave;
    f32x4 acc[MAXC];
#pragma unroll
    for (int c = 0; c < MAXC; ++c) acc[c] = f32x4{0.f, 0.f, 0.f, 0.f};
#define UNSH_FLUSH(slot, sign)                                                      \
    _Pragma("unroll") for (int c = 0; c < MAXC; ++c) {                              \
        const int e4 = (lane + 64 * c) * 4;                                         \
        if (e4 < dd) {                                                              \
            _Pragma("unroll") for (int q = 0; q < 4; ++q) {                         \
                my[e4 + q] += (sign) * acc[c][q];                                   \
                if ((slot) >= 0) my[(1 + (slot)) * dd + e4 + q] += acc[c][q];       \
            }                                                                       \
        }                                                                           \
        acc[c] = f32x4{0.f, 0.f, 0.f, 0.f};                                         \
    }
    const long total = (long)B * N;
    const long r0 = gw * rows_per_wave, r1 = r0 + rows_per_wave < total ? r0 + rows_per_wave : total;
    for (long r = r0; r < r1;) {
        const int pos = (int)(r % N);
        const int m = pos < n_img ? 0 : 1 + (pos - n_img) / n_tac;
        const int pos_end = pos < n_img ? n_img : min(N, n_img + m * n_tac);
        const long seg_end = min(r1, r - pos + pos_end);
        for (; r + 4 <= seg_end; r += 4) {
#pragma unroll
            for (int c = 0; c < MAXC; ++c) {
                const int e4 = (lane + 64 * c) * 4;
                if (e4 < dd) {
                    const TI* g = dY + r * dd + e4;
                    const f32x4 d0 = load4(g), d1 = load4(g + dd), d2 = load4(g + 2 * dd), d3 = load4(g + 3 * dd);
#pragma unroll
                    for (int q = 0; q < 4; ++q) acc[c][q] += (d0[q] + d1[q]) + (d2[q] + d3[q]);
                }
            }
        }
        for (; r < seg_end; ++r) {
#pragma unroll
            for (int c = 0; c < MAXC; ++c) {
                const int e4 = (lane + 64 * c) * 4;
                if (e4 < dd) {
                    const f32x4 d = load4(dY + r * dd + e4);
                    acc[c][0] += d[0]; acc[c][1] += d[1]; acc[c][2] += d[2]; acc[c][3] += d[3];
                }
            }
        }
        { UNSH_FLUSH(m, 1.f) }
    }
    const long vtotal = (long)B * nvis;
    const long v0 = gw * vis_per_wave, v1 = v0 + vis_per_wave < vtotal ? v0 + vis_per_wave : vtotal;
    long v = v0;
    for (; v + 4 <= v1; v += 4) {
        const TI* g[4];
#pragma unroll
        for (int u = 0; u < 4; ++u) g[u] = dY + ((long)((v + u) / nvis) * N + (int)unmasked[v + u]) * dd;
#pragma unroll
        for (int c = 0; c < MAXC; ++c) {
            const int e4 = (lane + 64 * c) * 4;
            if (e4 < dd) {
                f32x4 d[4];
#pragma unroll
                for (int u = 0; u < 4; ++u) d[u] = load4(g[u] + e4);
#pragma unroll
                for (int u = 0; u < 4; ++u) *reinterpret_cast<f32x4*>(dsrc + (v + u) * dd + e4) = d[u];
#pragma unroll
                for (int q = 0; q < 4; ++q) acc[c][q] += (d[0][q] + d[1][q]) + (d[2][q] + d[3][q]);
            }
        }
    }
    for (; v < v1; ++v) {
        const int b = (int)(v / nvis);
        const int pos = (int)unmasked[v];
        const TI* g = dY + ((long)b * N + pos) * dd;
#pragma unroll
        for (int c = 0; c < MAXC; ++c) {
            const int e4 = (lane + 64 * c) * 4;
            if (e4 < dd) {
                const f32x4 d = load4(g + e4);
                *reinterpret_cast<f32x4*>(dsrc + v * dd + e4) = d;
                acc[c][0] += d[0]; acc[c][1] += d[1]; acc[c][2] += d[2]; acc[c][3] += d[3];
            }
        }
    }
    { UNSH_FLUSH(-1, -1.f) }
#undef UNSH_FLUSH
    __syncthreads();
    for (int i = threadIdx.x; i < PL; i += 256)
        part[(long)blockIdx.x * PL + i] = sm[i] + sm[PL + i] + sm[2 * PL + i] + sm[3 * PL + i];
}

template <typename T>
__global__ __launch_bounds__(256) void gather_rows_kernel(const T* __restrict__ src, int N, int D, const int64_t* __restrict__ idx,
                                                            int idx_ld, int j0, int cnt, int rows, T* __restrict__ dst) {
    const int lane = threadIdx.x & 63, row = blockIdx.x * WPB + (threadIdx.x >> 6);
    if (row >= rows) return;
    const int b = row / cnt, jj = row % cnt;
    const long pos = idx[(long)b * idx_ld + j0 + jj];
    const T* s = src + ((long)b * N + pos) * D;
    T* d = dst + (long)row * D;
    for (int e = lane; e < D; e += 64) d[e] = s[e];
}
template <typename T>
__global__ __launch_bounds__(256) void scatter_rows_kernel(const T* __restrict__ src, int N, int D, const int64_t* __restrict__ idx,
                                                             int idx_ld, int j0, int cnt, int rows, T* __restrict__ dst) {
    const int lane = threadIdx.x & 63, row = blockIdx.x * WPB + (threadIdx.x >> 6);
    if (row >= rows) return;
    const int b = row / cnt, jj = row % cnt;
    const long pos = idx[(long)b * idx_ld + j0 + jj];
    const T* s = src + (long)row * D;
    T* d = dst + ((long)b * N + pos) * D;
    for (int e = lane; e < D; e += 64) d[e] = s[e];
}

template <typename T>
__global__ __launch_bounds__(256) void gather_rows2_kernel(const T* __restrict__ src, int N, int D, const int64_t* __restrict__ idx, int idx_ld,
                                                             int cnt0, int cnt1, int rows, T* __restrict__ dst0, T* __restrict__ dst1) {
    const int lane = threadIdx.x & 63, row = blockIdx.x * WPB + (threadIdx.x >> 6);
    if (row >= rows) return;
    const int b = row / (cnt0 + cnt1), j = row % (cnt0 + cnt1);
    const long pos = idx[(long)b * idx_ld + j];
    const uint4* s = reinterpret_cast<const uint4*>(src + ((long)b * N + pos) * D);
    uint4* d = reinterpret_cast<uint4*>(j < cnt0 ? dst0 + ((long)b * cnt0 + j) * D : dst1 + ((long)b * cnt1 + (j - cnt0)) * D);
    const int pieces = D * (int)sizeof(T) / 16;
    for (int p = lane; p < pieces; p += 64) d[p] = s[p];
}
template <typename T>
__global__ __launch_bounds__(256) void scatter_rows2_kernel(const T* __restrict__ src0, const T* __restrict__ src1, int N, int D,
                                                              const int64_t* __restrict__ idx, int idx_ld, int cnt0, int cnt1, int rows,
                                                              const float* __restrict__ scale, T* __restrict__ dst) {
    const int lane = threadIdx.x & 63, row = blockIdx.x * WPB + (threadIdx.x >> 6);
    if (row >= rows) return;
    const int b = row / (cnt0 + cnt1), j = row % (cnt0 + cnt1);
    const long pos = idx[(long)b * idx_ld + j];
    const T* s = j < cnt0 ? src0 + ((long)b * cnt0 + j) * D : src1 + ((long)b * cnt1 + (j - cnt0)) * D;
    T* d = dst + ((long)b * N + pos) * D;
    const float sc = scale ? *scale : 1.f;
    constexpr int E = 16 / (int)sizeof(T);
    const int pieces = D / E;
    for (int p = lane; p < pieces; p += 64) {
        uint4 v = reinterpret_cast<const uint4*>(s)[p];
        if (scale) {
            T* e = reinterpret_cast<T*>(&v);
#pragma unroll
            for (int k = 0; k < E; ++k) e[k] = from_f32<T>(to_f32(e[k]) * sc);
        }
        reinterpret_cast<uint4*>(d)[p] = v;
    }
}

template <typename T>
__global__ __launch_bounds__(256) void mse_kernel(const float* __restrict__ pred, int pdpad, PatchGroup pg,
                                                    const int64_t* __restrict__ idx, int idx_ld, int j0, int cnt, int rows, float w,
                                                    float* __restrict__ part, T* __restrict__ dpred, float* __restrict__ target_out, int vec) {
    extern __shared__ __attribute__((aligned(16))) float mbuf[];
    __shared__ float red[WPB];
    const int lane = threadIdx.x & 63, wave = threadIdx.x >> 6;
    const int pd = pg.C * pg.P * pg.P;
    const PatchDiv dv = patch_div(pg);
    float* my = mbuf + (long)wave * pdpad;
    float acc = 0.f;
    for (int r0 = blockIdx.x * WPB; r0 < rows; r0 += gridDim.x * WPB) {
        const int row = r0 + wave;
        const bool live = row < rows;
        if (live) {
            int b, s, ph, pw, local;
            patch_locate(pg, idx, idx_ld, j0, cnt, row, b, s, ph, pw, local);
            const float* base = patch_base(pg, b, s, ph, pw);
            for (int tb = 0; tb < pd; tb += 512) {
                const int t0 = tb + lane;
                float tv[8];
                int e[8];
#pragma unroll
                for (int u = 0; u < 8; ++u) {
                    if (tb + 64 * u >= pd) break;
                    const int t = t0 + 64 * u;
                    tv[u] = base[patch_off_t(pg, dv, min(t, pd - 1), e[u])];
                }
#pragma unroll
                for (int u = 0; u < 8; ++u) {
                    if (tb + 64 * u >= pd) break;
                    if (t0 + 64 * u < pd) my[e[u]] = tv[u];
                }
            }
        }
        __syncthreads();
        if (live) {
            const float* pr = pred + (long)row * pdpad;
            T* dp = dpred + (long)row * pdpad;
            if (vec) {
#pragma unroll 4
                for (int e = 4 * lane; e < pdpad; e += 256) {
                    f32x4 d = {0.f, 0.f, 0.f, 0.f};
                    if (e < pd) {
                        const f32x4 t = *reinterpret_cast<const f32x4*>(my + e);
                        d = load4(pr + e) - t;
                        if (target_out) store4<float>(target_out + (long)row * pd + e, t);
                    }
                    acc += d[0] * d[0];
                    acc += d[1] * d[1];
                    acc += d[2] * d[2];
                    acc += d[3] * d[3];
                    store4<T>(dp + e, d * (2.f * w));
                }
            } else {
                for (int e = lane; e < pdpad; e += 64) {
                    const float d = e < pd ? pr[e] - my[e] : 0.f;
                    if (e < pd && target_out) target_out[(long)row * pd + e] = my[e];
                    acc += d * d;
                    dp[e] = from_f32<T>(2.f * w * d);
                }
            }
        }
        __syncthreads();
    }
    acc = wave_sum(acc);
    if (lane == 0) red[wave] = acc;
    __syncthreads();
    if (threadIdx.x == 0) part[blockIdx.x] = w * (red[0] + red[1] + red[2] + red[3]);
}

}

static int ln_grid(int M) { return cdiv(M, WPB); }
static bool aligned_to(const void* p, size_t a) { return ((uintptr_t)p & (a - 1)) == 0; }
int m3l_part_blocks(void) {
    static const int nb = [] {
        const char* e = getenv("M3L_PART_BLOCKS");
        const int v = e ? atoi(e) : 1024;
        return v < 64 ? 64 : (v > M3L_MAX_PARTIAL_BLOCKS ? M3L_MAX_PARTIAL_BLOCKS : v);
    }();
    return nb;
}
static int part_grid(long rows) {
    long g = (rows + WPB - 1) / WPB;
    if (g > m3l_part_blocks()) g = m3l_part_blocks();
    return (int)(g < 1 ? 1 : g);
}

int m3l_ln_fwd(int out_dtype, const float* x, int M, int D, const float* gamma, const float* beta, float eps, void* y, float* y32,
               hipStream_t st) {
    M3L_CHECK(M > 0 && D > 0 && D % 4 == 0 && D <= 1024, "ln_fwd: bad shape M=%d D=%d (D must be a multiple of 4, <= 1024)", M, D);
    ProfScope prof("ln_fwd", M, D, out_dtype, (double)M * D * (4.0 + (y ? (out_dtype ? 2 : 4) : 0) + (y32 ? 4 : 0)), st);
#define LN_FWD(TO, C, TX) ln_fwd_kernel<TO, C, TX><<<ln_grid(M), 256, 0, st>>>((const TX*)x, M, D, gamma, beta, eps, (TO*)y, y32)
    if (m3l_call_rb()) {
        if (out_dtype == 1) { if (D <= 256) LN_FWD(bf16, 1, bf16); else if (D <= 512) LN_FWD(bf16, 2, bf16); else LN_FWD(bf16, 4, bf16); }
        else { if (D <= 256) LN_FWD(float, 1, bf16); else if (D <= 512) LN_FWD(float, 2, bf16); else LN_FWD(float, 4, bf16); }
    } else if (out_dtype == 1) {
        if (D <= 256) LN_FWD(bf16, 1, float); else if (D <= 512) LN_FWD(bf16, 2, float); else LN_FWD(bf16, 4, float);
    } else {
        if (D <= 256) LN_FWD(float, 1, float); else if (D <= 512) LN_FWD(float, 2, float); else LN_FWD(float, 4, float);
    }
#undef LN_FWD
    M3L_LAUNCH_CHECK();
    return 0;
}

int m3l_reduce_rows(const float* part, int G, int stride, int count, float* out, int accumulate, hipStream_t st) {
    if (count == 1 && stride == 1)
        reduce_vec_kernel<<<1, 1024, 0, st>>>(part, G, out, accumulate);
    else
        reduce_rows_kernel<<<cdiv(count, 32), 1024, 0, st>>>(part, G, stride, count, out, accumulate);
    M3L_LAUNCH_CHECK();
    return 0;
}

int m3l_ln_bwd_blocks(int M) {
    static const int forced = getenv("M3L_LN_ROWS_PER_WAVE") ? atoi(getenv("M3L_LN_ROWS_PER_WAVE")) : 0;
    const int rpw = forced > 0 ? forced : (M >= 12288 ? 4 : std::max(1, M / 4096));
    int G = cdiv(M, rpw * WPB);
    if (G > 2048) G = 2048;
    return G < 1 ? 1 : G;
}

int m3l_ln_bwd(int dy_dtype, const void* dy, const float* x, int M, int D, const float* gamma, float eps, const float* dres,
               float* dx_out, void* dx_t_out, int ct_dtype, float* part_ws, float* dgamma, float* dbeta, float* dbias,
               int accumulate, hipStream_t st) {
    M3L_CHECK(M > 0 && D > 0 && D % 4 == 0 && D <= 1024, "ln_bwd: bad shape M=%d D=%d (D must be a multiple of 4, <= 1024)", M, D);
    const int G = m3l_ln_bwd_blocks(M);
    {
        ProfScope prof("ln_bwd", M, D, dy_dtype,
                       (double)M * D * ((m3l_call_rb() ? 2.0 : 4.0) + (dy_dtype ? 2 : 4) + (dres ? (m3l_call_rb() ? 2 : 4) : 0) + (dx_out ? 4 : 0) + (dx_t_out ? (ct_dtype ? 2 : 4) : 0)), st);
#define LN_BWD(TD, TC, C, TX) ln_bwd_kernel<TD, TC, C, TX><<<G, 256, 0, st>>>((const TD*)dy, (const TX*)x, M, D, gamma, eps, dres, dx_out, (TC*)dx_t_out, part_ws)
#define LN_BWD_C(TD, TC, TX) { if (D <= 256) LN_BWD(TD, TC, 1, TX); else if (D <= 512) LN_BWD(TD, TC, 2, TX); else LN_BWD(TD, TC, 4, TX); }
        if (m3l_call_rb()) {
            M3L_CHECK(!dx_out && dx_t_out && ct_dtype == 1, "ln_bwd: bf16 residual mode writes the compute-type gradient only");
            if (dy_dtype == 1) LN_BWD_C(bf16, bf16, bf16) else LN_BWD_C(float, bf16, bf16)
        }
        else if (dy_dtype == 1) LN_BWD_C(bf16, bf16, float)
        else if (ct_dtype == 1) LN_BWD_C(float, bf16, float)
        else LN_BWD_C(float, float, float)
#undef LN_BWD_C
#undef LN_BWD
    }
    M3L_LAUNCH_CHECK();
    if (!dgamma && !dbeta && !dbias) return 0;
    ReduceSegs segs = {{dgamma, dbeta, dbias, nullptr}};
    reduce_rows_seg_kernel<<<dim3(cdiv(D, 32), 3), 1024, 0, st>>>(part_ws, G, 3 * D, D, segs, accumulate);
    M3L_LAUNCH_CHECK();
    return 0;
}

int m3l_reduce_rows_batch(const ReduceBatch* b, int accumulate, hipStream_t st) {
    if (b->count <= 0) return 0;
    M3L_CHECK(b->count <= M3L_REDUCE_BATCH_MAX && b->D > 0, "reduce_rows_batch: count=%d D=%d", b->count, b->D);
    ProfScope prof("reduce_batch", b->count, b->D, 0, 0.0, st);
    reduce_rows_batch_kernel<<<dim3(cdiv(b->D, 32), 3, b->count), 1024, 0, st>>>(*b, accumulate);
    M3L_LAUNCH_CHECK();
    return 0;
}

int m3l_reduce_rows_seg3(const float* part, int G, int D, float* out0, float* out1, float* out2, int accumulate, hipStream_t st) {
    ReduceSegs segs = {{out0, out1, out2, nullptr}};
    reduce_rows_seg_kernel<<<dim3(cdiv(D, 32), 3), 1024, 0, st>>>(part, G, 3 * D, D, segs, accumulate);
    M3L_LAUNCH_CHECK();
    return 0;
}

int m3l_colsum(int dtype, const void* Y, int M, int N, int ld, float* part_ws, float* out, int accumulate, hipStream_t st) {
    M3L_CHECK(M > 0 && N > 0, "colsum: bad shape");
    int G = cdiv(M, N > 512 ? 16 : 64);
    if (G > m3l_part_blocks()) G = m3l_part_blocks();
    const int rpb = cdiv(M, G);
    G = cdiv(M, rpb);
    ProfScope prof("colsum", M, N, dtype, (double)M * N * (dtype ? 2 : 4), st);
    const int vec_ok = (ld % 4 == 0) && (N % 4 == 0) && (((unsigned long)Y) % 16 == 0) && (((unsigned long)part_ws) % 16 == 0);
    if (dtype == 1)
        colsum_kernel<bf16><<<G, 256, 0, st>>>((const bf16*)Y, M, N, ld, rpb, part_ws, vec_ok);
    else
        colsum_kernel<float><<<G, 256, 0, st>>>((const float*)Y, M, N, ld, rpb, part_ws, vec_ok);
    M3L_LAUNCH_CHECK();
    return m3l_reduce_rows(part_ws, G, N, N, out, accumulate, st);
}

static thread_local int g_prep_mode = 0;
static thread_local int g_prep_dtype = -1;
static thread_local std::vector<WeightDesc>* g_prep_list = nullptr;
int m3l_prep_mode(void) { return g_prep_mode; }
void m3l_prep_set_mode(int mode) {
    g_prep_mode = mode;
    if (mode == 1) {
        if (!g_prep_list) g_prep_list = new std::vector<WeightDesc>();
        g_prep_list->clear();
        g_prep_dtype = -1;
    }
}
int m3l_prep_flush(hipStream_t st) {
    const int saved = g_prep_mode;
    g_prep_mode = 0;
    int rc = 0;
    if (g_prep_list && !g_prep_list->empty()) {
        for (size_t i = 0; i < g_prep_list->size() && !rc; i += M3L_WPACK) {
            WeightPack pk;
            memset(&pk, 0, sizeof(pk));
            for (size_t k = i; k < g_prep_list->size() && k < i + M3L_WPACK; ++k) pk.d[pk.count++] = (*g_prep_list)[k];
            rc = m3l_prep_weights(g_prep_dtype, &pk, st);
        }
        g_prep_list->clear();
    }
    g_prep_mode = saved;
    return rc;
}

int m3l_prep_weights(int dtype, const WeightPack* pack_in, hipStream_t st) {
    if (pack_in->count <= 0) return 0;
    M3L_CHECK(pack_in->count <= M3L_WPACK, "prep_weights: %d matrices in one pack (max %d)", pack_in->count, M3L_WPACK);
    if (g_prep_mode == 2) return 0;
    if (g_prep_mode == 1) {
        M3L_CHECK(g_prep_dtype < 0 || g_prep_dtype == dtype, "prep_weights: modules of one chain disagree on the compute type");
        g_prep_dtype = dtype;
        for (int i = 0; i < pack_in->count; ++i) g_prep_list->push_back(pack_in->d[i]);
        return 0;
    }
    WeightPack pack = *pack_in;
    int tiles = 0;
    for (int i = 0; i < pack.count; ++i) {
        const WeightDesc& d = pack.d[i];
        M3L_CHECK(d.ld_dst >= d.cols && d.ld_dstT >= d.rows && d.ld_dst <= ((d.cols + 63) / 64) * 64 && d.ld_dstT <= ((d.rows + 63) / 64) * 64,
                  "prep_weights: padding of matrix %d ([%d, %d] -> [%d, %d]) must stay inside its last 64 x 64 tiles", i, d.rows, d.cols, d.ld_dstT, d.ld_dst);
        pack.tile0[i] = tiles;
        tiles += ((d.rows + 63) / 64) * ((d.cols + 63) / 64);
    }
    pack.tile0[pack.count] = tiles;
    if (tiles == 0) return 0;
    ProfScope prof("prep_weights", pack.count, dtype, 0, 0.0, st);
    if (dtype == 1)
        prep_weights_kernel<bf16><<<tiles, 256, 0, st>>>(pack);
    else
        prep_weights_kernel<float><<<tiles, 256, 0, st>>>(pack);
    M3L_LAUNCH_CHECK();
    return 0;
}

int m3l_axpy_t(int dtype, const float* x, const void* o, long count, float* out, hipStream_t st) {
    if (dtype == 1)
        axpy_t_kernel<bf16><<<cdiv(count, 256), 256, 0, st>>>(x, (const bf16*)o, count, out);
    else
        axpy_t_kernel<float><<<cdiv(count, 256), 256, 0, st>>>(x, (const float*)o, count, out);
    M3L_LAUNCH_CHECK();
    return 0;
}

__global__ void cast8_f32_bf16_kernel(const float* __restrict__ x, long n8, bf16* __restrict__ out) {
    const long i = (long)blockIdx.x * blockDim.x + threadIdx.x;
    if (i >= n8) return;
    const f32x4 a = *reinterpret_cast<const f32x4*>(x + 8 * i), b = *reinterpret_cast<const f32x4*>(x + 8 * i + 4);
    bf16x8 o;
    o[0] = (bf16)a[0]; o[1] = (bf16)a[1]; o[2] = (bf16)a[2]; o[3] = (bf16)a[3];
    o[4] = (bf16)b[0]; o[5] = (bf16)b[1]; o[6] = (bf16)b[2]; o[7] = (bf16)b[3];
    *reinterpret_cast<bf16x8*>(out + 8 * i) = o;
}
__global__ void cast8_bf16_f32_kernel(const bf16* __restrict__ x, long n8, float* __restrict__ out) {
    const long i = (long)blockIdx.x * blockDim.x + threadIdx.x;
    if (i >= n8) return;
    const bf16x8 v = *reinterpret_cast<const bf16x8*>(x + 8 * i);
    *reinterpret_cast<f32x4*>(out + 8 * i) = f32x4{(float)v[0], (float)v[1], (float)v[2], (float)v[3]};
    *reinterpret_cast<f32x4*>(out + 8 * i + 4) = f32x4{(float)v[4], (float)v[5], (float)v[6], (float)v[7]};
}
int m3l_cast_bf16_f32(const void* x, long count, float* out, hipStream_t st) {
    M3L_CHECK(count % 8 == 0, "cast_bf16_f32: count %ld must be a multiple of 8", count);
    cast8_bf16_f32_kernel<<<cdiv(count / 8, 256), 256, 0, st>>>((const bf16*)x, count / 8, out);
    M3L_LAUNCH_CHECK();
    return 0;
}

int m3l_cast_f32(int dtype, const float* x, long count, void* out, hipStream_t st) {
    ProfScope prof("cast", count, dtype, 0, (double)count * (4.0 + (dtype ? 2 : 4)), st);
    if (dtype == 1 && count % 8 == 0 && ((uintptr_t)x & 15) == 0 && ((uintptr_t)out & 15) == 0)
        cast8_f32_bf16_kernel<<<cdiv(count / 8, 256), 256, 0, st>>>(x, count / 8, (bf16*)out);
    else if (dtype == 1)
        cast_kernel<bf16><<<cdiv(count, 256), 256, 0, st>>>(x, count, (bf16*)out);
    else
        cast_kernel<float><<<cdiv(count, 256), 256, 0, st>>>(x, count, (float*)out);
    M3L_LAUNCH_CHECK();
    return 0;
}

int m3l_im2col(int dtype, const ConvSrc* src, int Bsrc, int Ci, int H, int W, int KH, int S, int P, int OH, int OW, int Kpad, void* col,
               hipStream_t st) {
    const int Btot = src->nchw ? Bsrc * src->nsrc : Bsrc;
    const long total = (long)Btot * OH * OW * Kpad;
    if (dtype == 1 && KH == 4 && Kpad == Ci * 16) {
        const long pairs = (long)Btot * OH * OW * Ci;
        im2col4_bf16_kernel<<<cdiv(pairs, 256), 256, 0, st>>>(*src, Bsrc, Ci, H, W, S, P, OH, OW, pairs, (bf16*)col);
        M3L_LAUNCH_CHECK();
        return 0;
    }
    if (dtype == 1)
        im2col_kernel<bf16><<<cdiv(total, 256), 256, 0, st>>>(*src, Bsrc, Ci, H, W, KH, S, P, OH, OW, Kpad, total, (bf16*)col);
    else
        im2col_kernel<float><<<cdiv(total, 256), 256, 0, st>>>(*src, Bsrc, Ci, H, W, KH, S, P, OH, OW, Kpad, total, (float*)col);
    M3L_LAUNCH_CHECK();
    return 0;
}

int m3l_col2im_relu(int dtype, const void* dcol, int Btot, int Ci, int H, int W, int KH, int S, int P, int OH, int OW, int Kpad,
                    const void* act, void* dX, hipStream_t st) {
    const long total = (long)Btot * H * W * Ci;
    if (dtype == 1)
        col2im_relu_kernel<bf16><<<cdiv(total, 256), 256, 0, st>>>((const bf16*)dcol, Btot, Ci, H, W, KH, S, P, OH, OW, Kpad, (const bf16*)act, (bf16*)dX);
    else
        col2im_relu_kernel<float><<<cdiv(total, 256), 256, 0, st>>>((const float*)dcol, Btot, Ci, H, W, KH, S, P, OH, OW, Kpad, (const float*)act, (float*)dX);
    M3L_LAUNCH_CHECK();
    return 0;
}

int k_tokens_assemble(const float* img_tok, const float* tac_tok, int B, int D, int n_img, int n_tac, int k, const float* mod,
                        const float* pos_img, const float* pos_tac, float* tokens, hipStream_t st) {
    const long rows = (long)B * (n_img + k * n_tac);
    tokens_assemble_kernel<<<cdiv(rows, WPB), 256, 0, st>>>(img_tok, tac_tok, B, D, n_img, n_tac > 0 ? n_tac : 1, k, mod, pos_img, pos_tac, tokens);
    M3L_LAUNCH_CHECK();
    return 0;
}

int k_tokens_assemble_bwd(const float* dtok, int B, int D, int n_img, int n_tac, int k, float* d_img, float* d_tac, float* part_ws,
                            float* dmod, int accumulate, hipStream_t st) {
    const long rows = (long)B * (n_img + k * n_tac);
    const int PL = (1 + k) * D;
    const int G = part_grid(rows);
    tokens_assemble_bwd_kernel<<<G, 256, WPB * PL * sizeof(float), st>>>(dtok, B, D, n_img, n_tac > 0 ? n_tac : 1, k, d_img, d_tac, part_ws);
    M3L_LAUNCH_CHECK();
    reduce_rows_kernel<<<cdiv(PL, 32), 1024, 0, st>>>(part_ws, G, PL, PL, dmod, accumulate);
    M3L_LAUNCH_CHECK();
    return 0;
}

int m3l_adam_flat(float* p, const float* g, float* m, float* v, long n, float lr, float b1, float b2, float eps, float wd, int step,
                  float gscale, hipStream_t st) {
    M3L_CHECK(n > 0 && step >= 1, "adam: n=%ld step=%d", n, step);
    const float bc1 = 1.0f - powf(b1, (float)step);
    const float bc2_sqrt = sqrtf(1.0f - powf(b2, (float)step));
    adam_flat_kernel<0><<<cdiv(cdiv(n, 4), 256), 256, 0, st>>>(p, const_cast<float*>(g), m, v, n, lr, b1, b2, eps, wd, bc1, bc2_sqrt, nullptr, gscale, nullptr, 0);
    M3L_LAUNCH_CHECK();
    return 0;
}

int m3l_adamw_flat(float* p, float* g, float* m, float* v, long n, float lr, float b1, float b2, float eps, float wd, int step, float gscale,
                   float max_norm, float* norm_ws, int scale_grads, hipStream_t st) {
    M3L_CHECK(n > 0 && step >= 1, "adamw: n=%ld step=%d", n, step);
    M3L_CHECK(max_norm <= 0.f || norm_ws, "adamw: clipping needs the norm workspace");
    const float bc1 = 1.0f - powf(b1, (float)step);
    const float bc2_sqrt = sqrtf(1.0f - powf(b2, (float)step));
    const float* clip = nullptr;
    if (max_norm > 0.f) {
        const int G = (int)std::min<long>(1024, cdiv(cdiv(n, 4), 256));
        gradnorm_part_kernel<<<G, 256, 0, st>>>(g, n, norm_ws);
        M3L_LAUNCH_CHECK();
        gradnorm_final_kernel<<<1, 64, 0, st>>>(norm_ws, G, gscale, max_norm, norm_ws + 1024);
        M3L_LAUNCH_CHECK();
        clip = norm_ws + 1024;
    }
    const float decay = (float)(1.0 - (double)lr * (double)wd);
    adam_flat_kernel<1><<<cdiv(cdiv(n, 4), 256), 256, 0, st>>>(p, g, m, v, n, lr, b1, b2, eps, decay, bc1, bc2_sqrt, nullptr, gscale, clip,
                                                              scale_grads && (clip || gscale != 1.0f));
    M3L_LAUNCH_CHECK();
    return 0;
}

int m3l_dino_opt_flat(float* p, float* g, float* m, float* v, float* teacher, long n, const int64_t* seg_start, const int* seg_group, int S,
                      const float* lr, const float* wd, int n_groups, double beta1, double beta2, float eps, int step, float gscale, float max_norm,
                      float* norm_ws, int scale_grads, double ema_beta, hipStream_t st) {
    M3L_CHECK(p && g && m && v && seg_start && seg_group && lr && wd, "dino_opt: a buffer, a segment table or a hyper-parameter array is null");
    M3L_CHECK(n >= 1 && step >= 1 && S >= 1, "dino_opt: n=%ld step=%d segments=%d (each must be >= 1)", n, step, S);
    M3L_CHECK(n_groups >= 1 && n_groups <= DOPT_MAX_GROUPS, "dino_opt: %d groups (1 to %d)", n_groups, DOPT_MAX_GROUPS);
    M3L_CHECK((((uintptr_t)p | (uintptr_t)g | (uintptr_t)m | (uintptr_t)v | (uintptr_t)teacher) & 15) == 0,
              "dino_opt: params, grads, both moments and the teacher must be 16-byte aligned");
    M3L_CHECK(max_norm <= 0.f || norm_ws, "dino_opt: clipping needs the norm workspace");
    const long blocks = (n + DOPT_BLOCK_ELEMS - 1) / DOPT_BLOCK_ELEMS;
    M3L_CHECK(blocks < 2147483647L, "dino_opt: too many elements for one launch");
    const float bc1 = (float)(1.0 - pow(beta1, (double)step));
    const float bc2_sqrt = (float)sqrt(1.0 - pow(beta2, (double)step));
    DinoOptHyper hp;
    memset(&hp, 0, sizeof(hp));
    hp.count = n_groups;
    for (int k = 0; k < n_groups; ++k) {
        hp.lr[k] = lr[k];
        hp.decay[k] = (float)(1.0 - (double)lr[k] * (double)wd[k]);
    }
    const float* clip = nullptr;
    if (max_norm > 0.f) {
        const int G = (int)std::min<long>(1024, cdiv(cdiv(n, 4), 256));
        gradnorm_part_kernel<<<G, 256, 0, st>>>(g, n, norm_ws);
        M3L_LAUNCH_CHECK();
        gradnorm_final_kernel<<<1, 64, 0, st>>>(norm_ws, G, gscale, max_norm, norm_ws + 1024);
        M3L_LAUNCH_CHECK();
        clip = norm_ws + 1024;
    }
    ProfScope prof("dino_opt", n, S, teacher ? 1 : 0, 12.0 * n, st, 4.0 * (teacher ? 9.0 : 7.0) * n);
    dino_opt_kernel<<<(int)blocks, 256, 0, st>>>(p, g, m, v, teacher, n, seg_start, seg_group, S, hp, (float)(1.0 - beta1), (float)beta2, (float)(1.0 - beta2), eps, bc1,
                                                 bc2_sqrt, gscale, clip,
                                                 scale_grads && (clip || gscale != 1.0f), (float)ema_beta, (float)(1.0 - ema_beta));
    M3L_LAUNCH_CHECK();
    return 0;
}

int m3l_adam_flat_dev(float* p, const float* g, float* m, float* v, long n, float lr, float b1, float b2, float eps, float wd,
                      int* step_dev, float* bc_dev, hipStream_t st) {
    M3L_CHECK(n > 0 && step_dev && bc_dev, "adam (device step): n=%ld", n);
    adam_bias_kernel<<<1, 1, 0, st>>>(step_dev, b1, b2, bc_dev);
    M3L_LAUNCH_CHECK();
    adam_flat_kernel<0><<<cdiv(cdiv(n, 4), 256), 256, 0, st>>>(p, const_cast<float*>(g), m, v, n, lr, b1, b2, eps, wd, 1.0f, 1.0f, bc_dev, 1.0f, nullptr, 0);
    M3L_LAUNCH_CHECK();
    return 0;
}

int m3l_scale_by_dev(int dtype, const void* x, long count, const float* scale_dev, void* out, hipStream_t st) {
    if (dtype == 1)
        scale_by_dev_kernel<bf16><<<cdiv(count, 256), 256, 0, st>>>((const bf16*)x, count, scale_dev, (bf16*)out);
    else
        scale_by_dev_kernel<float><<<cdiv(count, 256), 256, 0, st>>>((const float*)x, count, scale_dev, (float*)out);
    M3L_LAUNCH_CHECK();
    return 0;
}

int m3l_mask_scale(int mode, const float* src, const void* ref, float scale, long count, float* out, hipStream_t st) {
    M3L_CHECK((mode == 0 || mode == 1) && count > 0 && src && ref && out, "mask_scale: bad arguments");
    if (mode == 0) mask_scale_kernel<0><<<cdiv(count, 256), 256, 0, st>>>(src, ref, scale, count, out);
    else mask_scale_kernel<1><<<cdiv(count, 256), 256, 0, st>>>(src, ref, scale, count, out);
    M3L_LAUNCH_CHECK();
    return 0;
}
int m3l_vit_tokens(const float* emb, const float* cls, const float* regs, const float* pos, int B, int npatch, int R, int D, float* tok,
                   hipStream_t st) {
    M3L_CHECK(B > 0 && npatch > 0 && R >= 0 && D > 0 && emb && cls && pos && tok && (R == 0 || regs), "vit_tokens: bad arguments");
    vit_tokens_kernel<<<cdiv((long)B * (1 + R + npatch) * D, 256), 256, 0, st>>>(emb, cls, regs, pos, B, npatch, R, D, tok);
    M3L_LAUNCH_CHECK();
    return 0;
}
int m3l_concat2(float* a, int na, float* b2, int nb, int rows, float* cat, int split, hipStream_t st) {
    M3L_CHECK(rows > 0 && na > 0 && nb > 0 && a && cat && (split || b2), "concat2: bad arguments");
    concat2_kernel<<<cdiv((long)rows * (na + nb), 256), 256, 0, st>>>(a, na, b2, nb, rows, cat, split);
    M3L_LAUNCH_CHECK();
    return 0;
}

int m3l_vt_load_launch(const void* image_nhwc, int image_u8, int B, int H, int W, int C, float img_lo, float img_span, float* image_nchw,
                       const void* tactile, int tactile_u8, int th, int tw, int n_sensors, int frame_stack, float tac_lo, float tac_span,
                       float* const* tactile_out, hipStream_t st) {
    if (image_nhwc) {
        M3L_CHECK(img_span != 0.f, "vt_load: empty image normalisation range");
        const long total = (long)B * C * H * W;
        if (image_u8)
            vt_image_kernel<uint8_t><<<cdiv(total, 256), 256, 0, st>>>((const uint8_t*)image_nhwc, B, H, W, C, img_lo, img_span, image_nchw);
        else
            vt_image_kernel<float><<<cdiv(total, 256), 256, 0, st>>>((const float*)image_nhwc, B, H, W, C, img_lo, img_span, image_nchw);
        M3L_LAUNCH_CHECK();
    }
    if (tactile) {
        M3L_CHECK(n_sensors >= 1 && n_sensors <= M3L_MAX_SENSORS, "vt_load: n_sensors=%d", n_sensors);
        M3L_CHECK(tac_span != 0.f, "vt_load: empty tactile normalisation range");
        VtTactileOut o;
        for (int s = 0; s < n_sensors; ++s) o.p[s] = tactile_out[s];
        const long total = (long)B * 3 * n_sensors * frame_stack * th * tw;
        if (tactile_u8)
            vt_tactile_kernel<uint8_t><<<cdiv(total, 256), 256, 0, st>>>((const uint8_t*)tactile, B, th, tw, n_sensors, frame_stack, tac_lo,
                                                                         tac_span, o);
        else
            vt_tactile_kernel<float><<<cdiv(total, 256), 256, 0, st>>>((const float*)tactile, B, th, tw, n_sensors, frame_stack, tac_lo,
                                                                       tac_span, o);
        M3L_LAUNCH_CHECK();
    }
    return 0;
}

int m3l_mask_rank_groups(const MaskRankArgs* args, int B, int64_t* masked, int masked_ld, int64_t* unmasked, int unmasked_ld, hipStream_t st) {
    M3L_CHECK(B > 0 && args->count >= 1 && args->count <= M3L_MAX_SENSORS + 1, "mask_rank: B=%d groups=%d", B, args->count);
    int nmax = 0;
    for (int i = 0; i < args->count; ++i) {
        const MaskRankGroup& g = args->g[i];
        M3L_CHECK(g.n > 0 && g.nm >= 0 && g.nm <= g.n, "mask_rank: bad shape n=%d nm=%d", g.n, g.nm);
        M3L_CHECK(g.n <= 8192, "mask_rank: n=%d too large", g.n);
        nmax = std::max(nmax, g.n);
    }
    const int threads = nmax <= 64 ? 64 : (nmax <= 128 ? 128 : 256);
    mask_rank_kernel<<<dim3(B, args->count), threads, nmax * sizeof(float), st>>>(*args, masked, masked_ld, unmasked, unmasked_ld);
    M3L_LAUNCH_CHECK();
    return 0;
}
int m3l_mask_rank(const float* noise, int B, int n, int nm, int token_offset, int64_t* masked, int masked_ld, int masked_off,
                  int64_t* unmasked, int unmasked_ld, int unmasked_off, hipStream_t st) {
    MaskRankArgs a;
    memset(&a, 0, sizeof(a));
    a.count = 1;
    a.g[0] = MaskRankGroup{noise, n, nm, token_offset, masked_off, unmasked_off};
    return m3l_mask_rank_groups(&a, B, masked, masked_ld, unmasked, unmasked_ld, st);
}

constexpr int PATCH_NV_MAX = 40;
static int check_pg(const PatchGroup& pg) {
    const int pd = pg.C * pg.P * pg.P;
    M3L_CHECK(pg.nsrc >= 1 && pg.nsrc <= M3L_MAX_SENSORS, "patch group: nsrc=%d", pg.nsrc);
    M3L_CHECK(pd <= 64 * PATCH_NV_MAX, "patch dim %d > %d unsupported", pd, 64 * PATCH_NV_MAX);
    M3L_CHECK(pg.H % pg.P == 0 && pg.W % pg.P == 0, "image dims must be divisible by the patch size");
    return 0;
}

int m3l_patch_ln(int dtype, const PatchGroup* pg, const int64_t* idx, int idx_ld, int j0, int cnt, int B, const float* gamma,
                 const float* beta, float eps, void* xn, int pdpad, hipStream_t st) {
    if (check_pg(*pg)) return 1;
    const int rows = B * cnt;
    if (rows == 0) return 0;
    const int pd_ = pg->C * pg->P * pg->P, esz = dtype == 1 ? 2 : 4;
    const bool wide = pd_ > 64 * MAXV, tiny = pd_ <= 256;
    const int vec = pd_ % 4 == 0 && pdpad % 4 == 0 && aligned_to(gamma, 16) && aligned_to(beta, 16) && aligned_to(xn, 4 * esz);
#define PATCH_LN(T, NV) patch_ln_kernel<T, NV><<<ln_grid(rows), 256, 0, st>>>(*pg, idx, idx_ld, j0, cnt, rows, gamma, beta, eps, (T*)xn, pdpad, vec)
    if (dtype == 1) {
        if (wide) PATCH_LN(bf16, PATCH_NV_MAX); else if (tiny) PATCH_LN(bf16, 4); else PATCH_LN(bf16, MAXV);
    } else {
        if (wide) PATCH_LN(float, PATCH_NV_MAX); else if (tiny) PATCH_LN(float, 4); else PATCH_LN(float, MAXV);
    }
#undef PATCH_LN
    M3L_LAUNCH_CHECK();
    return 0;
}

int m3l_patch_ln_bwd(int dtype, const PatchGroup* pg, const int64_t* idx, int idx_ld, int j0, int cnt, int B, float eps,
                     const void* dxn, int pdpad, float* part_ws, float* dgamma, float* dbeta, int accumulate, hipStream_t st) {
    if (check_pg(*pg)) return 1;
    const int rows = B * cnt;
    if (rows == 0) return 0;
    const int pd = pg->C * pg->P * pg->P;
    const int G = part_grid(rows);
    const bool wide = pd > 64 * MAXV, tiny = pd <= 256;
    const int vec = pd % 4 == 0 && pdpad % 4 == 0 && aligned_to(dxn, 4 * (dtype == 1 ? 2 : 4));
#define PATCH_LN_BWD(T, NV) patch_ln_bwd_kernel<T, NV><<<G, 256, 0, st>>>(*pg, idx, idx_ld, j0, cnt, rows, eps, (const T*)dxn, pdpad, part_ws, vec)
    if (dtype == 1) {
        if (wide) PATCH_LN_BWD(bf16, PATCH_NV_MAX); else if (tiny) PATCH_LN_BWD(bf16, 4); else PATCH_LN_BWD(bf16, MAXV);
    } else {
        if (wide) PATCH_LN_BWD(float, PATCH_NV_MAX); else if (tiny) PATCH_LN_BWD(float, 4); else PATCH_LN_BWD(float, MAXV);
    }
#undef PATCH_LN_BWD
    M3L_LAUNCH_CHECK();
    ReduceSegs segs = {{dgamma, dbeta, nullptr, nullptr}};
    reduce_rows_seg_kernel<<<dim3(cdiv(pd, 32), 2), 1024, 0, st>>>(part_ws, G, 2 * pd, pd, segs, accumulate);
    M3L_LAUNCH_CHECK();
    return 0;
}

int m3l_embed_finalize(const float* E, int D, const PatchGroup* pg, const int64_t* idx, int idx_ld, int j0, int cnt, int B,
                       const float* gamma, const float* beta, float eps, const float* mod, int mod0, const float* pos,
                       float* tokens, int L, hipStream_t st) {
    const int rows = B * cnt;
    if (rows == 0) return 0;
    M3L_CHECK(D <= 64 * MAXV, "embed_finalize: D=%d too large", D);
    embed_finalize_kernel<<<ln_grid(rows), 256, 0, st>>>(E, rows, D, *pg, idx, idx_ld, j0, cnt, gamma, beta, eps, mod, mod0, pos, tokens, L);
    M3L_LAUNCH_CHECK();
    return 0;
}

int m3l_embed_finalize_bwd(int dtype, const float* dtok, int L, const float* E, int D, const PatchGroup* pg, const int64_t* idx,
                           int idx_ld, int j0, int cnt, int B, const float* gamma, float eps, void* dE, float* part_ws,
                           float* dgamma, float* dbeta, float* dmod, int mod0, int accumulate, hipStream_t st) {
    const int rows = B * cnt;
    if (rows == 0) return 0;
    const int nslot = pg->nsrc;
    const int PL = (2 + nslot) * D;
    const int G = part_grid(rows);
    if (dtype == 1)
        embed_finalize_bwd_kernel<bf16><<<G, 256, WPB * PL * sizeof(float), st>>>(dtok, L, E, rows, D, *pg, idx, idx_ld, j0, cnt, gamma, eps, (bf16*)dE, part_ws, nslot);
    else
        embed_finalize_bwd_kernel<float><<<G, 256, WPB * PL * sizeof(float), st>>>(dtok, L, E, rows, D, *pg, idx, idx_ld, j0, cnt, gamma, eps, (float*)dE, part_ws, nslot);
    M3L_LAUNCH_CHECK();
    if (nslot <= 2) {
        float* dm = dmod + (long)mod0 * D;
        ReduceSegs segs = {{dgamma, dbeta, dm, nslot > 1 ? dm + D : nullptr}};
        reduce_rows_seg_kernel<<<dim3(cdiv(D, 32), 2 + nslot), 1024, 0, st>>>(part_ws, G, PL, D, segs, accumulate);
    } else {
        reduce_rows_kernel<<<cdiv(D, 32), 1024, 0, st>>>(part_ws, G, PL, D, dgamma, accumulate);
        reduce_rows_kernel<<<cdiv(D, 32), 1024, 0, st>>>(part_ws + D, G, PL, D, dbeta, accumulate);
        reduce_rows_kernel<<<cdiv(nslot * D, 32), 1024, 0, st>>>(part_ws + 2 * D, G, PL, nslot * D, dmod + (long)mod0 * D, accumulate);
    }
    M3L_LAUNCH_CHECK();
    return 0;
}

int k_unshuffle_fwd(const float* src, const float* mask_token, const int64_t* unmasked, int nvis, const int64_t* masked,
                      int nmask, int B, int dd, int n_img, int n_tac, const float* dmod, const float* pos_img, const float* pos_tac,
                      float* dec_in, hipStream_t st) {
    const long rows = (long)B * (nvis + nmask);
    M3L_CHECK(dd % 4 == 0, "unshuffle_fwd: dd=%d must be a multiple of 4", dd);
    if (m3l_call_io())
        unshuffle_fwd_kernel<bf16><<<cdiv(rows, WPB), 256, 0, st>>>(src, mask_token, unmasked, nvis, masked, nmask, B, dd, n_img, n_tac > 0 ? n_tac : 1, dmod,
                                                                     pos_img, pos_tac, reinterpret_cast<bf16*>(dec_in));
    else
        unshuffle_fwd_kernel<float><<<cdiv(rows, WPB), 256, 0, st>>>(src, mask_token, unmasked, nvis, masked, nmask, B, dd, n_img, n_tac > 0 ? n_tac : 1, dmod,
                                                                      pos_img, pos_tac, dec_in);
    M3L_LAUNCH_CHECK();
    return 0;
}

int k_unshuffle_bwd(const float* dY, const int64_t* unmasked, int nvis, const int64_t* masked, int nmask, int B, int dd, int n_img,
                      int n_tac, int nmod, float* dsrc, float* part_ws, float* dmask_token, float* ddmod, int accumulate,
                      hipStream_t st) {
    const long rows = (long)B * (nvis + nmask);
    const int PL = (1 + nmod) * dd;
    M3L_CHECK(dd % 4 == 0 && dd <= 1024, "unshuffle_bwd: dd=%d must be a multiple of 4, <= 1024", dd);
    (void)masked;
    int rpw = 16;
    while (cdiv(cdiv(rows, rpw), WPB) > m3l_part_blocks()) rpw *= 2;
    const int G = cdiv(cdiv(rows, rpw), WPB);
    const int vpw = cdiv((long)B * nvis, (long)G * WPB);
    const int N = nvis + nmask, nt = n_tac > 0 ? n_tac : 1;
    const size_t lds = WPB * PL * sizeof(float);
#define UNSH_BWD(C, TI) unshuffle_bwd_kernel<C, TI><<<G, 256, lds, st>>>((const TI*)dY, unmasked, nvis, B, N, dd, n_img, nt, nmod, rpw, vpw, dsrc, part_ws)
    if (m3l_call_io()) {
        if (dd <= 256) UNSH_BWD(1, bf16); else if (dd <= 512) UNSH_BWD(2, bf16); else UNSH_BWD(4, bf16);
    } else {
        if (dd <= 256) UNSH_BWD(1, float); else if (dd <= 512) UNSH_BWD(2, float); else UNSH_BWD(4, float);
    }
#undef UNSH_BWD
    M3L_LAUNCH_CHECK();
    if (nmod <= 3) {
        ReduceSegs segs = {{dmask_token, ddmod, nmod > 1 ? ddmod + dd : nullptr, nmod > 2 ? ddmod + 2 * dd : nullptr}};
        reduce_rows_seg_kernel<<<dim3(cdiv(dd, 32), 1 + nmod), 1024, 0, st>>>(part_ws, G, PL, dd, segs, accumulate);
    } else {
        reduce_rows_kernel<<<cdiv(dd, 32), 1024, 0, st>>>(part_ws, G, PL, dd, dmask_token, accumulate);
        reduce_rows_kernel<<<cdiv(nmod * dd, 32), 1024, 0, st>>>(part_ws + dd, G, PL, nmod * dd, ddmod, accumulate);
    }
    M3L_LAUNCH_CHECK();
    return 0;
}

int m3l_gather_rows(int dtype, const void* src, int N, int D, const int64_t* idx, int idx_ld, int j0, int cnt, int B, void* dst,
                    hipStream_t st) {
    const int rows = B * cnt;
    if (rows == 0) return 0;
    if (dtype == 1)
        gather_rows_kernel<bf16><<<ln_grid(rows), 256, 0, st>>>((const bf16*)src, N, D, idx, idx_ld, j0, cnt, rows, (bf16*)dst);
    else
        gather_rows_kernel<float><<<ln_grid(rows), 256, 0, st>>>((const float*)src, N, D, idx, idx_ld, j0, cnt, rows, (float*)dst);
    M3L_LAUNCH_CHECK();
    return 0;
}

int m3l_gather_rows2(int dtype, const void* src, int N, int D, const int64_t* idx, int idx_ld, int cnt0, int cnt1, int B, void* dst0, void* dst1,
                     hipStream_t st) {
    const int rows = B * (cnt0 + cnt1);
    if (rows == 0) return 0;
    M3L_CHECK((D * (dtype ? 2 : 4)) % 16 == 0, "gather_rows2: rows of %d elements are not 16-byte pieces", D);
    if (dtype == 1)
        gather_rows2_kernel<bf16><<<ln_grid(rows), 256, 0, st>>>((const bf16*)src, N, D, idx, idx_ld, cnt0, cnt1, rows, (bf16*)dst0, (bf16*)dst1);
    else
        gather_rows2_kernel<float><<<ln_grid(rows), 256, 0, st>>>((const float*)src, N, D, idx, idx_ld, cnt0, cnt1, rows, (float*)dst0, (float*)dst1);
    M3L_LAUNCH_CHECK();
    return 0;
}
int m3l_scatter_rows2(int dtype, const void* src0, const void* src1, int N, int D, const int64_t* idx, int idx_ld, int cnt0, int cnt1, int B,
                      const float* scale_dev, void* dst, hipStream_t st) {
    const int rows = B * (cnt0 + cnt1);
    if (rows == 0) return 0;
    M3L_CHECK((D * (dtype ? 2 : 4)) % 16 == 0, "scatter_rows2: rows of %d elements are not 16-byte pieces", D);
    if (dtype == 1)
        scatter_rows2_kernel<bf16><<<ln_grid(rows), 256, 0, st>>>((const bf16*)src0, (const bf16*)src1, N, D, idx, idx_ld, cnt0, cnt1, rows, scale_dev,
                                                                  (bf16*)dst);
    else
        scatter_rows2_kernel<float><<<ln_grid(rows), 256, 0, st>>>((const float*)src0, (const float*)src1, N, D, idx, idx_ld, cnt0, cnt1, rows,
                                                                   scale_dev, (float*)dst);
    M3L_LAUNCH_CHECK();
    return 0;
}

int m3l_scatter_rows(int dtype, const void* src, int N, int D, const int64_t* idx, int idx_ld, int j0, int cnt, int B, void* dst,
                     hipStream_t st) {
    const int rows = B * cnt;
    if (rows == 0) return 0;
    if (dtype == 1)
        scatter_rows_kernel<bf16><<<ln_grid(rows), 256, 0, st>>>((const bf16*)src, N, D, idx, idx_ld, j0, cnt, rows, (bf16*)dst);
    else
        scatter_rows_kernel<float><<<ln_grid(rows), 256, 0, st>>>((const float*)src, N, D, idx, idx_ld, j0, cnt, rows, (float*)dst);
    M3L_LAUNCH_CHECK();
    return 0;
}

int m3l_mse(int dtype, const float* pred, int pdpad, const PatchGroup* pg, const int64_t* idx, int idx_ld, int j0, int cnt, int B,
            float weight, float* part_ws, int* nblocks_out, void* dpred, float* target_out, hipStream_t st) {
    if (check_pg(*pg)) return 1;
    const int rows = B * cnt;
    if (nblocks_out) *nblocks_out = 0;
    if (rows == 0) return 0;
    const int pd = pg->C * pg->P * pg->P;
    const float w = weight / ((float)rows * (float)pd);
    const int G = part_grid(rows);
    M3L_CHECK(pdpad >= pd, "mse: pdpad %d < patch dim %d", pdpad, pd);
    const int vec = pd % 4 == 0 && pdpad % 4 == 0 && aligned_to(pred, 16) && aligned_to(dpred, 4 * (dtype == 1 ? 2 : 4)) &&
                    (!target_out || aligned_to(target_out, 16));
    const size_t lds = (size_t)WPB * pdpad * sizeof(float);
    M3L_CHECK(lds <= 64 * 1024, "mse: padded patch dim %d too wide", pdpad);
    if (dtype == 1)
        mse_kernel<bf16><<<G, 256, lds, st>>>(pred, pdpad, *pg, idx, idx_ld, j0, cnt, rows, w, part_ws, (bf16*)dpred, target_out, vec);
    else
        mse_kernel<float><<<G, 256, lds, st>>>(pred, pdpad, *pg, idx, idx_ld, j0, cnt, rows, w, part_ws, (float*)dpred, target_out, vec);
    M3L_LAUNCH_CHECK();
    if (nblocks_out) *nblocks_out = G;
    return 0;
}

DropCtx m3l_drop_ctx(float p, uint64_t seed, int layer, int site) {
    DropCtx d;
    memset(&d, 0, sizeof(d));
    d.on = p > 0.f ? 1 : 0;
    const double pd = p;
    const double t = floor(pd * 4294967296.0);
    d.thr = t >= 4294967295.0 ? 0xFFFFFFFFu : (uint32_t)t;
    d.scale = pd >= 1.0 ? 0.f : (float)(1.0 / (1.0 - pd));
    d.k0 = (uint32_t)seed;
    d.k1 = (uint32_t)(seed >> 32);
    d.ctr2 = (uint32_t)(4 * layer + site);
    return d;
}

namespace {
template <typename T>
__global__ __launch_bounds__(256) void dropout_bwd_kernel(const T* __restrict__ dy, T* __restrict__ out, float* __restrict__ part, int M, int N,
                                                           int rpb, DropCtx dr) {
    __shared__ float red[1024];
    const int NQ = N >> 2, RY = blockDim.y, tx = threadIdx.x, ty = threadIdx.y;
    const int r0 = blockIdx.x * rpb, r1 = min(M, r0 + rpb);
    float cs[4] = {0.f, 0.f, 0.f, 0.f};
    for (int r = r0 + ty; r < r1; r += RY) {
        const long o = (long)r * N + 4 * tx;
        const uint4 wd = drop_words(dr.k0, dr.k1, dr.ctr2, (uint64_t)r * NQ + tx);
        const uint32_t w[4] = {wd.x, wd.y, wd.z, wd.w};
#pragma unroll
        for (int j = 0; j < 4; ++j) {
            const T v = from_f32<T>(to_f32(dy[o + j]) * (w[j] >= dr.thr ? dr.scale : 0.f));
            out[o + j] = v;
            cs[j] += to_f32(v);
        }
    }
#pragma unroll
    for (int j = 0; j < 4; ++j) red[ty * N + 4 * tx + j] = cs[j];
    __syncthreads();
    if (ty == 0) {
#pragma unroll
        for (int j = 0; j < 4; ++j) {
            float s = 0.f;
            for (int y = 0; y < RY; ++y) s += red[y * N + 4 * tx + j];
            part[(long)blockIdx.x * N + 4 * tx + j] = s;
        }
    }
}

__global__ void dropout_mask_kernel(DropCtx dr, long rows, int N, uint8_t* __restrict__ out) {
    const int NQ = (N + 3) >> 2;
    const long i = (long)blockIdx.x * blockDim.x + threadIdx.x;
    if (i >= rows * NQ) return;
    const long r = i / NQ;
    const int c0 = (int)(i % NQ) * 4;
    const uint4 wd = drop_words(dr.k0, dr.k1, dr.ctr2, (uint64_t)i);
    const uint32_t w[4] = {wd.x, wd.y, wd.z, wd.w};
    for (int j = 0; j < 4 && c0 + j < N; ++j) out[r * N + c0 + j] = w[j] >= dr.thr ? 1 : 0;
}

int dropout_rows_per_block(int M) { return std::max(32, cdiv(M, 1024)); }
}

int m3l_dropout_bwd_blocks(int M) { return cdiv(M, dropout_rows_per_block(M)); }

int m3l_dropout_bwd(int dtype, const void* dy, int M, int N, const DropCtx* drop, void* out, float* part, hipStream_t st) {
    M3L_CHECK(dtype == 0 || dtype == 1, "dropout_bwd: bad dtype %d", dtype);
    M3L_CHECK(M > 0 && N > 0 && N % 4 == 0 && N <= 1024, "dropout_bwd: M=%d N=%d (N must be a multiple of 4, <= 1024)", M, N);
    const int rpb = dropout_rows_per_block(M), NQ = N / 4;
    const dim3 blk(NQ, std::max(1, 256 / NQ));
    const int G = cdiv(M, rpb);
    ProfScope prof("dropout_bwd", M, N, 0, 0.0, st, (double)M * N * (dtype ? 4.0 : 8.0));
    if (dtype == 1)
        dropout_bwd_kernel<bf16><<<G, blk, 0, st>>>((const bf16*)dy, (bf16*)out, part, M, N, rpb, *drop);
    else
        dropout_bwd_kernel<float><<<G, blk, 0, st>>>((const float*)dy, (float*)out, part, M, N, rpb, *drop);
    M3L_LAUNCH_CHECK();
    return 0;
}

int m3l_dropout_mask(const DropCtx* drop, long rows, int N, uint8_t* out, hipStream_t st) {
    M3L_CHECK(rows > 0 && N > 0, "dropout_mask: rows=%ld N=%d", rows, N);
    const long total = rows * ((N + 3) / 4);
    dropout_mask_kernel<<<(unsigned)((total + 255) / 256), 256, 0, st>>>(*drop, rows, N, out);
    M3L_LAUNCH_CHECK();
    return 0;
}
```

### m3l_amd/csrc/mae_plan.hip

```cpp
#include <stdarg.h>
#include <stdio.h>
#include <stdlib.h>
#include <string.h>

#include <algorithm>
#include <map>
#include <mutex>
#include <vector>

#include "../../include/m3l_amd.h"
#include "common.cuh"
#include "kernels.h"
#include "tf_plan.h"


namespace {

constexpr float LN_EPS = 1e-5f;

struct SideStream {
    hipStream_t s = nullptr;
    std::vector<hipEvent_t> ev;
    int next = 0;
};
// ... 1244 lines not shown
    void *col[3], *act[3], *w[4], *wT[4];
    void *dout_t, *dpreA, *dpreB, *dcol;
    void *wf[3], *wd[3];
    float* slab;
    bool direct;
    float* scratch;
    size_t scratch_b, total;
};
int g_direct_conv = -1;
bool cnn_direct(const m3l_cnn_cfg* c) {
    if (g_direct_conv < 0) g_direct_conv = getenv("M3L_DIRECT_CONV") ? (atoi(getenv("M3L_DIRECT_CONV")) > 0 ? 1 : 0) : 1;
    if (!g_direct_conv || c->dtype != 1) return false;
    const int D = c->dim, co[3] = {D / 8, D / 4, D / 2};
    int ci = c->in_channels;
    for (int l = 0; l < 3; ++l) {
        const bool k3 = l == 2 && c->tactile;
        if (!m3l_conv_direct_supported(c->dtype, ci, co[l], k3 ? 3 : 4, k3 ? 1 : 2, 1, l == 0)) return false;
        ci = co[l];
    }
    return true;
}
CnnWs cnn_layout(const m3l_cnn_cfg* c, int Btot, void* ws) {
    Arena a(ws);
    CnnWs w;
    const int D = c->dim;
    const int co[4] = {D / 8, D / 4, D / 2, D};
    int ci = c->in_channels, H = c->height, W = c->width;
    for (int l = 0; l < 4; ++l) {
        ConvL& L = w.L[l];
        L.Ci = ci; L.Co = co[l]; L.H = H; L.W = W;
        if (l == 3) { L.KH = 1; L.S = 1; L.P = 0; }
        else if (l == 2 && c->tactile) { L.KH = 3; L.S = 1; L.P = 1; }
        else { L.KH = 4; L.S = 2; L.P = 1; }
        L.OH = (H + 2 * L.P - L.KH) / L.S + 1;
        L.OW = (W + 2 * L.P - L.KH) / L.S + 1;
        L.K = L.Ci * L.KH * L.KH;
        L.Kpad = pad8(L.K);
        L.M = (long)Btot * L.OH * L.OW;
        ci = L.Co; H = L.OH; W = L.OW;
    }
    const size_t e = esz(c->dtype);
    size_t max_pre = 0, max_col = 0, max_slab = 0;
    w.direct = cnn_direct(c);
    for (int l = 0; l < 4; ++l) {
        const ConvL& L = w.L[l];
        w.w[l] = a.take((size_t)L.Co * L.Kpad * e);
        w.wT[l] = a.take((size_t)L.Kpad * L.Co * e);
        if (l < 3) {
            w.col[l] = w.direct ? nullptr : a.take((size_t)L.M * L.Kpad * e);
            w.act[l] = a.take((size_t)L.M * L.Co * e);
            max_col = std::max(max_col, (size_t)L.M * L.Kpad);
            w.wf[l] = w.wd[l] = nullptr;
            if (w.direct) {
                w.wf[l] = a.take(m3l_conv_wf_elems(L.Ci, L.Co, L.KH) * 2);
                if (l) w.wd[l] = a.take(m3l_conv_wd_elems(L.Ci, L.Co, L.KH, L.S) * 2);
                max_slab = std::max(max_slab, m3l_conv_wgrad_slab_elems(Btot, L.Ci, L.H, L.W, L.Co, L.KH, L.S, L.P));
            }
        }
        max_pre = std::max(max_pre, (size_t)L.M * L.Co);
    }
    w.dout_t = a.take((size_t)w.L[3].M * D * e);
    w.dpreA = a.take(max_pre * e);
    w.dpreB = a.take(max_pre * e);
    w.dcol = w.direct ? nullptr : a.take(max_col * e);
    w.slab = w.direct ? reinterpret_cast<float*>(a.take(max_slab * sizeof(float))) : nullptr;
    std::vector<std::pair<int, int>> shapes;
    long Mmax = 1;
    for (int l = 0; l < 4; ++l) { shapes.push_back({w.L[l].Co, w.L[l].Kpad}); Mmax = std::max(Mmax, w.L[l].M); }
    w.scratch_b = 0;
    for (int l = 0; l < 4; ++l) w.scratch_b = std::max(w.scratch_b, m3l_gemm_tn_ws_bytes((int)w.L[l].M, w.L[l].Co, w.L[l].Kpad, nullptr));
    w.scratch_b = std::max(w.scratch_b, (size_t)M3L_MAX_PARTIAL_BLOCKS * D * sizeof(float));
    w.scratch = reinterpret_cast<float*>(a.take(w.scratch_b));
    w.total = a.off + 256;
    return w;
}
int check_cnn(const m3l_cnn_cfg* c, int B, int nsrc) {
    M3L_CHECK(c->dtype == 0 || c->dtype == 1, "earlycnn: bad dtype");
    M3L_CHECK(c->dim % 64 == 0, "earlycnn: dim=%d must be a multiple of 64", c->dim);
    M3L_CHECK(B > 0 && nsrc >= 1 && nsrc <= M3L_MAX_SENSORS, "earlycnn: B=%d nsrc=%d", B, nsrc);
    M3L_CHECK(c->height % 8 == 0 && c->width % 8 == 0 || (c->tactile && c->height % 4 == 0 && c->width % 4 == 0), "earlycnn: image size");
    return 0;
}
}

int m3l_set_direct_conv(int on) {
    if (g_direct_conv < 0) g_direct_conv = getenv("M3L_DIRECT_CONV") ? (atoi(getenv("M3L_DIRECT_CONV")) > 0 ? 1 : 0) : 1;
    const int old = g_direct_conv;
    g_direct_conv = on ? 1 : 0;
    return old;
}

size_t m3l_earlycnn_ws_bytes(const m3l_cnn_cfg* c, int B, int nsrc) {
    if (check_cnn(c, B, nsrc)) return 0;
    return cnn_layout(c, B * nsrc, nullptr).total;
}

int m3l_earlycnn_fwd(const m3l_cnn_cfg* c, int B, int nsrc, const float* const* srcs, const void* const* tensors, void* ws, float* out,
                     void* stream) {
    if (check_cnn(c, B, nsrc)) return 1;
    hipStream_t st = (hipStream_t)stream;
    const int Btot = B * nsrc, dt = c->dtype;
    CnnWs w = cnn_layout(c, Btot, ws);
    for (int l = 0; l < 4; ++l) {
        const ConvL& L = w.L[l];
        WeightPack pk;
        memset(&pk, 0, sizeof(pk));
        pk.d[0] = WeightDesc{(const float*)tensors[2 * l], w.w[l], w.wT[l], L.Co, L.K, L.Kpad, L.Co};
        pk.count = 1;
        if (m3l_prep_weights(dt, &pk, st)) return 1;
    }
    if (m3l_prep_mode() == 1) return 0;
    ConvSrc cs;
    memset(&cs, 0, sizeof(cs));
    for (int i = 0; i < nsrc; ++i) cs.src[i] = srcs[i];
    cs.nsrc = nsrc; cs.nchw = 1;
    for (int l = 0; l < 3; ++l) {
        const ConvL& L = w.L[l];
        if (w.direct) {
            if (m3l_conv_prep((const float*)tensors[2 * l], L.Ci, L.Co, L.KH, L.S, w.wf[l], w.wd[l], st)) return 1;
            if (m3l_conv_fwd(&cs, B, Btot, L.Ci, L.H, L.W, L.Co, L.KH, L.S, L.P, w.wf[l], (const float*)tensors[2 * l + 1], w.act[l], st)) return 1;
            memset(&cs, 0, sizeof(cs));
            cs.src[0] = w.act[l]; cs.nsrc = 1; cs.nchw = 0;
            continue;
        }
        if (m3l_im2col(dt, &cs, l == 0 ? B : Btot, L.Ci, L.H, L.W, L.KH, L.S, L.P, L.OH, L.OW, L.Kpad, w.col[l], st)) return 1;
        GemmEpi e = epi0(L.Co);
        e.bias = (const float*)tensors[2 * l + 1];
        e.act = 2;
        e.out_t = w.act[l];
        if (m3l_gemm_nt(dt, w.col[l], L.Kpad, w.w[l], L.Kpad, (int)L.M, L.Co, L.Kpad, &e, st)) return 1;
        memset(&cs, 0, sizeof(cs));
        cs.src[0] = w.act[l]; cs.nsrc = 1; cs.nchw = 0;
    }
    const ConvL& L3 = w.L[3];
    GemmEpi e = epi0(L3.Co);
    e.bias = (const float*)tensors[7];
    e.out_f32 = out;
    return m3l_gemm_nt(dt, w.act[2], L3.Kpad, w.w[3], L3.Kpad, (int)L3.M, L3.Co, L3.Kpad, &e, st);
}

int m3l_earlycnn_bwd(const m3l_cnn_cfg* c, int B, int nsrc, const float* const* srcs, const void* const* tensors, void* ws, const float* dout,
                     float* const* grads, void* stream) {
    if (check_cnn(c, B, nsrc)) return 1;
    (void)tensors;
    hipStream_t st = (hipStream_t)stream;
    const int Btot = B * nsrc, dt = c->dtype, D = c->dim;
    CnnWs w = cnn_layout(c, Btot, ws);
    const ConvL& L3 = w.L[3];
    if (m3l_cast_f32(dt, dout, L3.M * D, w.dout_t, st)) return 1;
    if (m3l_gemm_tn(dt, w.dout_t, D, w.act[2], L3.Kpad, (int)L3.M, D, L3.Kpad, w.scratch, w.scratch_b, grads[6], L3.K, D, L3.K, 0, st)) return 1;
    if (m3l_colsum(0, dout, (int)L3.M, D, D, w.scratch, grads[7], 0, st)) return 1;
    void* dpre = w.dpreA;
    void* dnext = w.dpreB;
    {
        GemmEpi e = epi0(L3.Kpad);
        e.out_t = dpre; e.relu_ref = w.act[2];
        if (m3l_gemm_nt(dt, w.dout_t, D, w.wT[3], D, (int)L3.M, L3.Kpad, D, &e, st)) return 1;
    }
    for (int l = 2; l >= 0; --l) {
        const ConvL& L = w.L[l];
        if (w.direct) {
            M3L_CHECK(srcs != nullptr, "earlycnn_bwd: the direct convolutions read the stem's input frames again (srcs)");
            ConvSrc cs;
            memset(&cs, 0, sizeof(cs));
            if (l == 0) {
                for (int i = 0; i < nsrc; ++i) cs.src[i] = srcs[i];
                cs.nsrc = nsrc; cs.nchw = 1;
            } else {
                cs.src[0] = w.act[l - 1]; cs.nsrc = 1; cs.nchw = 0;
            }
            if (m3l_conv_wgrad(&cs, B, Btot, L.Ci, L.H, L.W, L.Co, L.KH, L.S, L.P, dpre, w.slab, grads[2 * l], st)) return 1;
            if (m3l_colsum(dt, dpre, (int)L.M, L.Co, L.Co, w.scratch, grads[2 * l + 1], 0, st)) return 1;
            if (l == 0) break;
            if (m3l_conv_dgrad(dpre, Btot, L.Ci, L.H, L.W, L.Co, L.KH, L.S, L.P, w.wd[l], w.act[l - 1], dnext, st)) return 1;
            std::swap(dpre, dnext);
            continue;
        }
        if (m3l_gemm_tn(dt, dpre, L.Co, w.col[l], L.Kpad, (int)L.M, L.Co, L.Kpad, w.scratch, w.scratch_b, grads[2 * l], L.K, L.Co, L.K, 0, st))
            return 1;
        if (m3l_colsum(dt, dpre, (int)L.M, L.Co, L.Co, w.scratch, grads[2 * l + 1], 0, st)) return 1;
        if (l == 0) break;
        GemmEpi e = epi0(L.Kpad);
        e.out_t = w.dcol;
        if (m3l_gemm_nt(dt, dpre, L.Co, w.wT[l], L.Co, (int)L.M, L.Kpad, L.Co, &e, st)) return 1;
        if (m3l_col2im_relu(dt, w.dcol, Btot, L.Ci, L.H, L.W, L.KH, L.S, L.P, L.OH, L.OW, L.Kpad, w.act[l - 1], dnext, st)) return 1;
        std::swap(dpre, dnext);
    }
    return 0;
}

size_t m3l_tokens_assemble_ws_bytes(const m3l_geom* g, int D) {
    return (size_t)M3L_MAX_PARTIAL_BLOCKS * (1 + (g->num_tactiles > 0 ? g->num_tactiles : 0)) * D * sizeof(float) + 256;
}
int m3l_tokens_assemble_fwd(const m3l_geom* g, int D, int B, const float* img_tok, const float* tac_tok, const void* const* tensors,
                            float* tokens, void* stream) {
    if (check_geom(g)) return 1;
    const Geo ge = geo_of(g);
    return k_tokens_assemble(img_tok, tac_tok, B, D, ge.n_img, ge.n_tac, ge.k, (const float*)tensors[0], (const float*)tensors[1],
                             (const float*)tensors[2], tokens, (hipStream_t)stream);
}
int m3l_tokens_assemble_bwd(const m3l_geom* g, int D, int B, const float* dtokens, float* d_img, float* d_tac, void* ws, float* dmod,
                            void* stream) {
    if (check_geom(g)) return 1;
    const Geo ge = geo_of(g);
    float* part = (float*)ws;
    return k_tokens_assemble_bwd(dtokens, B, D, ge.n_img, ge.n_tac, ge.k, d_img, d_tac, part, dmod, 0, (hipStream_t)stream);
}

size_t m3l_layernorm_ws_bytes(int D) { return (size_t)2048 * 3 * D * sizeof(float) + 256; }

int m3l_layernorm_fwd(int out_dtype, const float* x, int M, int D, const float* gamma, const float* beta, float eps, void* y,
                      float* y32, void* stream) {
    return m3l_ln_fwd(out_dtype, x, M, D, gamma, beta, eps, y, y32, (hipStream_t)stream);
}
int m3l_layernorm_bwd(int dy_dtype, const void* dy, const float* x, int M, int D, const float* gamma, float eps, const float* dres,
                      float* dx, void* ws, float* dgamma, float* dbeta, void* stream) {
    return m3l_ln_bwd(dy_dtype, dy, x, M, D, gamma, eps, dres, dx, nullptr, dy_dtype, (float*)ws, dgamma, dbeta, nullptr, 0, (hipStream_t)stream);
}
int m3l_gather_tokens(const float* src, int B, int N, int D, const int64_t* idx, int K, float* dst, void* stream) {
    return m3l_gather_rows(0, src, N, D, idx, K, 0, K, B, dst, (hipStream_t)stream);
}
int m3l_scatter_tokens(const float* src, int B, int N, int D, const int64_t* idx, int K, float* dst_zeroed, void* stream) {
    return m3l_scatter_rows(0, src, N, D, idx, K, 0, K, B, dst_zeroed, (hipStream_t)stream);
}
int m3l_vt_load(const float* image_nhwc, int B, int H, int W, int C, float* image_nchw, const float* tactile, int th, int tw,
                int n_sensors, int frame_stack, float* const* tactile_out, void* stream) {
    return m3l_vt_load_launch(image_nhwc, 0, B, H, W, C, 0.f, 1.f, image_nchw, tactile, 0, th, tw, n_sensors, frame_stack, -1.f, 2.f, tactile_out,
                              (hipStream_t)stream);
}
int m3l_vt_load2(const void* image_nhwc, int image_u8, int B, int H, int W, int C, double img_lo, double img_hi, float* image_nchw,
                 const void* tactile, int tactile_u8, int th, int tw, int n_sensors, int frame_stack, double tac_lo, double tac_hi,
                 float* const* tactile_out, void* stream) {
    return m3l_vt_load_launch(image_nhwc, image_u8, B, H, W, C, (float)img_lo, (float)(img_hi - img_lo), image_nchw, tactile, tactile_u8, th, tw,
                              n_sensors, frame_stack, (float)tac_lo, (float)(tac_hi - tac_lo), tactile_out, (hipStream_t)stream);
}

int m3l_adam_step(float* params, const float* grads, float* exp_avg, float* exp_avg_sq, long n, float lr, float beta1, float beta2,
                  float eps, float weight_decay, int step, void* stream) {
    return m3l_adam_flat(params, grads, exp_avg, exp_avg_sq, n, lr, beta1, beta2, eps, weight_decay, step, 1.0f, (hipStream_t)stream);
}
int m3l_adam_step_scaled(float* params, const float* grads, float* exp_avg, float* exp_avg_sq, long n, float lr, float beta1, float beta2,
                         float eps, float weight_decay, int step, float grad_scale, void* stream) {
    return m3l_adam_flat(params, grads, exp_avg, exp_avg_sq, n, lr, beta1, beta2, eps, weight_decay, step, grad_scale, (hipStream_t)stream);
}

int m3l_adamw_step(float* params, float* grads, float* exp_avg, float* exp_avg_sq, long n, float lr, float beta1, float beta2, float eps,
                   float weight_decay, int step, float grad_scale, float max_grad_norm, float* norm_ws, int scale_grads, void* stream) {
    return m3l_adamw_flat(params, grads, exp_avg, exp_avg_sq, n, lr, beta1, beta2, eps, weight_decay, step, grad_scale, max_grad_norm, norm_ws,
                          scale_grads, (hipStream_t)stream);
}

int m3l_dino_opt_step(float* params, float* grads, float* exp_avg, float* exp_avg_sq, float* teacher, long n, const int64_t* seg_start,
                      const int32_t* seg_group, int n_segments, const float* group_lr, const float* group_weight_decay, int n_groups,
                      double beta1, double beta2, float eps, int step, float grad_scale, float max_grad_norm, float* norm_ws, int scale_grads,
                      double ema_beta, void* stream) {
    return m3l_dino_opt_flat(params, grads, exp_avg, exp_avg_sq, teacher, n, seg_start, seg_group, n_segments, group_lr, group_weight_decay,
                             n_groups, beta1, beta2, eps, step, grad_scale, max_grad_norm, norm_ws, scale_grads, ema_beta, (hipStream_t)stream);
}

int m3l_adam_step_dev(float* params, const float* grads, float* exp_avg, float* exp_avg_sq, long n, float lr, float beta1,
                      float beta2, float eps, float weight_decay, int* step_dev, float* bias_corr_dev, void* stream) {
    return m3l_adam_flat_dev(params, grads, exp_avg, exp_avg_sq, n, lr, beta1, beta2, eps, weight_decay, step_dev, bias_corr_dev,
                             (hipStream_t)stream);
}

int m3l_op_gemm_nt(int dtype, const void* A, int lda, const void* W, int ldw, int M, int N, int K, const float* bias,
                   const float* res, float* out_f32, void* out_t, void* out_pre, const void* gelu_u, int act, int ldc, void* stream) {
    GemmEpi e = epi0(ldc);
    e.bias = bias; e.res = res; e.out_f32 = out_f32; e.out_t = out_t; e.out_pre = out_pre; e.gelu_u = gelu_u; e.act = act;
    return m3l_gemm_nt(dtype, A, lda, W, ldw, M, N, K, &e, (hipStream_t)stream);
}
size_t m3l_op_gemm_tn_ws_bytes(int M, int N, int K) { return m3l_gemm_tn_ws_bytes(M, N, K, nullptr); }
int m3l_op_gemm_tn(int dtype, const void* Y, int ldy, const void* X, int ldx, int M, int N, int K, void* ws, size_t ws_bytes,
                   float* out, int ldo, void* stream) {
    return m3l_gemm_tn(dtype, Y, ldy, X, ldx, M, N, K, (float*)ws, ws_bytes, out, ldo, N, K, 0, (hipStream_t)stream);
}
int m3l_op_gemm_tn_acc(int dtype, const void* Y, int ldy, const void* X, int ldx, int M, int N, int K, void* ws, size_t ws_bytes, float* out, int ldo,
                       int accumulate, void* stream) {
    return m3l_gemm_tn(dtype, Y, ldy, X, ldx, M, N, K, (float*)ws, ws_bytes, out, ldo, N, K, accumulate ? 1 : 0, (hipStream_t)stream);
}
size_t m3l_op_gemm_tn_grouped_ws_bytes(int dtype, int count, int M, const int* N, const int* K) {
    (void)dtype;
    if (count < 1 || count > M3L_TN_MAX_PROBLEMS || M <= 0 || !N || !K) return 0;
    TnProblem pr[M3L_TN_MAX_PROBLEMS];
    memset(pr, 0, sizeof(pr));
    for (int i = 0; i < count; ++i) { pr[i].N = N[i]; pr[i].K = K[i]; }
    return m3l_gemm_tn_grouped_ws_bytes(M, pr, count);
}
int m3l_op_gemm_tn_grouped(int dtype, int count, int M, const void* const* Y, const int* ldy, const void* const* X, const int* ldx, const int* N,
                           const int* K, float* const* out, void* ws, size_t ws_bytes, void* stream) {
    M3L_CHECK(count >= 1 && count <= M3L_TN_MAX_PROBLEMS && Y && X && ldy && ldx && N && K && out && ws, "gemm_tn_grouped: bad arguments (count %d)", count);
    TnProblem pr[M3L_TN_MAX_PROBLEMS];
    memset(pr, 0, sizeof(pr));
    for (int i = 0; i < count; ++i) {
        pr[i].Y = Y[i]; pr[i].X = X[i]; pr[i].ldy = ldy[i]; pr[i].ldx = ldx[i]; pr[i].N = N[i]; pr[i].K = K[i];
        pr[i].out = out[i]; pr[i].ldo = K[i]; pr[i].nvalid = N[i]; pr[i].kvalid = K[i];
    }
    return m3l_gemm_tn_grouped(dtype, pr, count, M, (float*)ws, ws_bytes, 0, (hipStream_t)stream);
}
int m3l_op_colsum(int dtype, const void* Y, int M, int N, int ld, void* ws, float* out, void* stream) {
    return m3l_colsum(dtype, Y, M, N, ld, (float*)ws, out, 0, (hipStream_t)stream);
}
size_t m3l_op_colsum_ws_bytes(int N) { return (size_t)M3L_MAX_PARTIAL_BLOCKS * N * sizeof(float) + 256; }
int m3l_op_prep_weight(int dtype, const float* src, int rows, int cols, void* dst, void* dstT, void* stream) {
    WeightPack pk;
    memset(&pk, 0, sizeof(pk));
    pk.d[0] = WeightDesc{src, dst, dstT, rows, cols, cols, rows};
    pk.count = 1;
    return m3l_prep_weights(dtype, &pk, (hipStream_t)stream);
}
int m3l_op_mask_scale(int mode, const float* src, const void* ref, float scale, long count, float* out, void* stream) {
    return m3l_mask_scale(mode, src, ref, scale, count, out, (hipStream_t)stream);
}
int m3l_op_concat2(float* a, int na, float* b, int nb, int rows, float* cat, int split, void* stream) {
    return m3l_concat2(a, na, b, nb, rows, cat, split, (hipStream_t)stream);
}
int m3l_op_patch_cols(int dtype, const float* x, int B, int C, int H, int W, int P, int Kpad, void* col, void* stream) {
    M3L_CHECK(x && col && B > 0 && P > 0 && H % P == 0 && W % P == 0 && Kpad >= C * P * P, "patch_cols: bad arguments");
    ConvSrc cs;
    memset(&cs, 0, sizeof(cs));
    cs.src[0] = x; cs.nsrc = 1; cs.nchw = 1;
    return m3l_im2col(dtype, &cs, B, C, H, W, P, P, 0, H / P, W / P, Kpad, col, (hipStream_t)stream);
}
int m3l_op_vit_tokens(const float* emb, const float* cls, const float* regs, const float* pos, int B, int npatch, int R, int D, float* tok,
                      void* stream) {
    return m3l_vit_tokens(emb, cls, regs, pos, B, npatch, R, D, tok, (hipStream_t)stream);
}
int m3l_op_dropout_mask(float p, uint64_t seed, int layer, int site, long rows, int N, uint8_t* out, void* stream) {
    M3L_CHECK(p >= 0.f && p <= 1.f && site >= 0 && site < 4 && layer >= 0, "op_dropout_mask: p=%g site=%d layer=%d", (double)p, site, layer);
    const DropCtx d = m3l_drop_ctx(p, seed, layer, site);
    return m3l_dropout_mask(&d, rows, N, out, (hipStream_t)stream);
}
int m3l_op_attn_fwd(int dtype, const void* qkv, void* o, float* lse, int B, int n, int H, void* stream) {
    return m3l_attn_fwd(dtype, qkv, o, lse, B, n, H, 64, (hipStream_t)stream);
}
int m3l_op_attn_bwd(int dtype, const void* qkv, const void* o, const void* dO, const float* lse, float* dsum, void* dqkv, int B,
                    int n, int H, void* stream) {
    return m3l_attn_bwd(dtype, qkv, o, dO, lse, dsum, dqkv, B, n, H, 64, (hipStream_t)stream);
}
int m3l_op_attn_fwd_dh(int dtype, const void* qkv, void* o, float* lse, int B, int n, int H, void* stream, int dim_head) {
    return m3l_attn_fwd(dtype, qkv, o, lse, B, n, H, dim_head, (hipStream_t)stream);
}
int m3l_op_attn_bwd_dh(int dtype, const void* qkv, const void* o, const void* dO, const float* lse, float* dsum, void* dqkv, int B,
                       int n, int H, void* stream, int dim_head) {
    return m3l_attn_bwd(dtype, qkv, o, dO, lse, dsum, dqkv, B, n, H, dim_head, (hipStream_t)stream);
}

}
```

Baseline: 75290 samples/s.

## Vectorize partial-row reductions and pack several MSE rows per wavefront

The column-reduction kernels now use 256-thread blocks where each thread loads float4 slices with deeper unrolling, in place of 1024-thread blocks doing scalar loads. The MSE loss kernel assigns several patch rows to each wavefront when the patch dimension is small, gathers target pixels as float4 when alignment allows, and orders LDS access with wave-level fences instead of block barriers. It also adds profiling byte counts and a batched reduce entry point. The aim is to cut latency and idle lanes in small reduction and loss kernels, at the cost of more code paths and reliance on the alignment checks being correct.

```diff
diff --git a/include/m3l_amd.h b/include/m3l_amd.h
--- a/include/m3l_amd.h
+++ b/include/m3l_amd.h
@@ -247,6 +247,7 @@
                            const int* K, float* const* out, void* ws, size_t ws_bytes, void* stream);
 size_t m3l_op_colsum_ws_bytes(int N);
 int m3l_op_colsum(int dtype, const void* Y, int M, int N, int ld, void* ws, float* out, void* stream);
+int m3l_op_reduce_rows_batch(int count, int D, const float* const* parts, const int* G, float* const* outs, int accumulate, void* stream);
 int m3l_op_prep_weight(int dtype, const float* src, int rows, int cols, void* dst, void* dstT, void* stream);
 int m3l_op_mask_scale(int mode, const float* src, const void* ref, float scale, long count, float* out, void* stream);
 int m3l_op_concat2(float* a, int na, float* b, int nb, int rows, float* cat, int split, void* stream);
diff --git a/m3l_amd/_lib.py b/m3l_amd/_lib.py
--- a/m3l_amd/_lib.py
+++ b/m3l_amd/_lib.py
@@ -157,6 +157,7 @@
     "m3l_op_gemm_tn_grouped": (c_i, [c_i, c_i, c_i, c_p, c_p, c_p, c_p, c_p, c_p, c_p, c_p, c_sz, c_p]),
     "m3l_op_colsum_ws_bytes": (c_sz, [c_i]),
     "m3l_op_colsum": (c_i, [c_i, c_p, c_i, c_i, c_i, c_p, c_p, c_p]),
+    "m3l_op_reduce_rows_batch": (c_i, [c_i, c_i, c_p, c_p, c_p, c_i, c_p]),
     "m3l_op_prep_weight": (c_i, [c_i, c_p, c_i, c_i, c_p, c_p, c_p]),
     "m3l_op_mask_scale": (c_i, [c_i, c_p, c_p, C.c_float, C.c_long, c_p, c_p]),
     "m3l_op_concat2": (c_i, [c_p, c_i, c_p, c_i, c_i, c_p, c_i, c_p]),
diff --git a/m3l_amd/csrc/elementwise.hip b/m3l_amd/csrc/elementwise.hip
--- a/m3l_amd/csrc/elementwise.hip
+++ b/m3l_amd/csrc/elementwise.hip
@@ -146,35 +146,73 @@
     }
 }
 
-__device__ __forceinline__ void reduce_cols_32x32(const float* __restrict__ p, int G, int stride, int j, bool valid,
+constexpr int RED_THREADS = 256;
+
+template <bool VEC>
+__device__ __forceinline__ f32x4 red_load(const float* __restrict__ p, long off, int nv) {
+    if (VEC) return *reinterpret_cast<const f32x4*>(p + off);
+    f32x4 v = {0.f, 0.f, 0.f, 0.f};
+#pragma unroll
+    for (int k = 0; k < 4; ++k)
+        if (k < nv) v[k] = p[off + k];
+    return v;
+}
+template <bool VEC, int NT>
+__device__ __forceinline__ void red_steps(const float* __restrict__ p, int g, int stride, int j, int nv, f32x4 (&a)[8]) {
+    f32x4 v[8 * NT];
+#pragma unroll
+    for (int i = 0; i < 8 * NT; ++i) v[i] = red_load<VEC>(p, (long)(g + 32 * i) * stride + j, nv);
+#pragma unroll
+    for (int i = 0; i < 8 * NT; ++i) a[i & 7] += v[i];
+}
+template <bool VEC>
+__device__ __forceinline__ f32x4 red_slice(const float* __restrict__ p, int G, int stride, int j, int nv, int sl) {
+    f32x4 a[8];
+#pragma unroll
+    for (int u = 0; u < 8; ++u) a[u] = f32x4{0.f, 0.f, 0.f, 0.f};
+    int g = sl;
+    if (VEC) {
+        for (; g + 224 + 768 < G; g += 1024) red_steps<VEC, 4>(p, g, stride, j, nv, a);
+        if (g + 224 + 256 < G) { red_steps<VEC, 2>(p, g, stride, j, nv, a); g += 512; }
+    }
+    for (; g + 224 < G; g += 256) red_steps<VEC, 1>(p, g, stride, j, nv, a);
+    if (g < G) {
+        f32x4 v[7];
+#pragma unroll
+        for (int i = 0; i < 7; ++i) v[i] = red_load<VEC>(p, (long)min(g + 32 * i, G - 1) * stride + j, nv);
+#pragma unroll
+        for (int i = 0; i < 7; ++i)
+            if (g + 32 * i < G) a[0] += v[i];
+    }
+    return ((a[0] + a[1]) + (a[2] + a[3])) + ((a[4] + a[5]) + (a[6] + a[7]));
+}
+
+__device__ __forceinline__ void reduce_cols_32x32(const float* __restrict__ p, int G, int stride, int j0, int count,
                                                   float* __restrict__ out, int accumulate) {
     __shared__ float red[32][33];
-    const int cl = threadIdx.x & 31, sl = threadIdx.x >> 5;
-    float s = 0.f;
-    if (valid) {
-        float a[8] = {0.f, 0.f, 0.f, 0.f, 0.f, 0.f, 0.f, 0.f};
-        int g = sl;
-        for (; g + 224 < G; g += 256) {
-#pragma unroll
-            for (int u = 0; u < 8; ++u) a[u] += p[(long)(g + 32 * u) * stride + j];
-        }
-        for (; g < G; g += 32) a[0] += p[(long)g * stride + j];
-        s = ((a[0] + a[1]) + (a[2] + a[3])) + ((a[4] + a[5]) + (a[6] + a[7]));
-    }
-    red[sl][cl] = s;
+    const int q = threadIdx.x & 7, sl = threadIdx.x >> 3;
+    const int j = j0 + 4 * q;
+    const int nv = min(4, count - j);
+    f32x4 s = {0.f, 0.f, 0.f, 0.f};
+    if (nv == 4 && (stride & 3) == 0 && (reinterpret_cast<uintptr_t>(p) & 15) == 0)
+        s = red_slice<true>(p, G, stride, j, nv, sl);
+    else if (nv > 0)
+        s = red_slice<false>(p, G, stride, j, nv, sl);
+#pragma unroll
+    for (int k = 0; k < 4; ++k) red[sl][4 * q + k] = s[k];
     __syncthreads();
-    if (sl == 0 && valid) {
-        float t = red[0][cl];
-#pragma unroll
-        for (int i = 1; i < 32; ++i) t += red[i][cl];
-        out[j] = accumulate ? out[j] + t : t;
-    }
-}
-
-__global__ __launch_bounds__(1024) void reduce_rows_kernel(const float* __restrict__ part, int G, int stride, int count,
+    const int c = threadIdx.x;
+    if (c < 32 && j0 + c < count) {
+        float t = red[0][c];
+#pragma unroll
+        for (int i = 1; i < 32; ++i) t += red[i][c];
+        out[j0 + c] = accumulate ? out[j0 + c] + t : t;
+    }
+}
+
+__global__ __launch_bounds__(RED_THREADS) void reduce_rows_kernel(const float* __restrict__ part, int G, int stride, int count,
                                                              float* __restrict__ out, int accumulate) {
-    const int j = blockIdx.x * 32 + (threadIdx.x & 31);
-    reduce_cols_32x32(part, G, stride, j, j < count, out, accumulate);
+    reduce_cols_32x32(part, G, stride, blockIdx.x * 32, count, out, accumulate);
 }
 
 __global__ __launch_bounds__(1024) void reduce_vec_kernel(const float* __restrict__ v, int G, float* __restrict__ out, int accumulate) {
@@ -195,20 +233,19 @@
 }
 
 struct ReduceSegs { float* out[4]; };
-__global__ __launch_bounds__(1024) void reduce_rows_seg_kernel(const float* __restrict__ part, int G, int stride, int width,
+__global__ __launch_bounds__(RED_THREADS) void reduce_rows_seg_kernel(const float* __restrict__ part, int G, int stride, int width,
                                                                  ReduceSegs segs, int accumulate) {
-    float* out = segs.out[blockIdx.y];
+    const int y = blockIdx.y;
+    float* out = y == 0 ? segs.out[0] : (y == 1 ? segs.out[1] : (y == 2 ? segs.out[2] : segs.out[3]));
     if (!out) return;
-    const int j = blockIdx.x * 32 + (threadIdx.x & 31);
-    reduce_cols_32x32(part + (long)blockIdx.y * width, G, stride, j, j < width, out, accumulate);
-}
-
-__global__ __launch_bounds__(1024) void reduce_rows_batch_kernel(ReduceBatch b, int accumulate) {
-    const ReduceBatchItem it = b.it[blockIdx.z];
-    float* out = it.out[blockIdx.y];
+    reduce_cols_32x32(part + (long)blockIdx.y * width, G, stride, blockIdx.x * 32, width, out, accumulate);
+}
+
+__global__ __launch_bounds__(RED_THREADS) void reduce_rows_batch_kernel(ReduceBatch b, int accumulate) {
+    const ReduceBatchItem& it = b.it[blockIdx.z];
+    float* out = blockIdx.y == 0 ? it.out[0] : (blockIdx.y == 1 ? it.out[1] : it.out[2]);
     if (!out) return;
-    const int j = blockIdx.x * 32 + (threadIdx.x & 31);
-    reduce_cols_32x32(it.part + (long)blockIdx.y * b.D, it.G, 3 * b.D, j, j < b.D, out, accumulate);
+    reduce_cols_32x32(it.part + (long)blockIdx.y * b.D, it.G, 3 * b.D, blockIdx.x * 32, b.D, out, accumulate);
 }
 
 template <typename T> struct Vec4;
@@ -1153,53 +1190,82 @@
     }
 }
 
+__device__ __forceinline__ void wave_lds_order() {
+    __builtin_amdgcn_fence(__ATOMIC_RELEASE, "wavefront");
+    __builtin_amdgcn_wave_barrier();
+    __builtin_amdgcn_fence(__ATOMIC_ACQUIRE, "wavefront");
+}
 template <typename T>
 __global__ __launch_bounds__(256) void mse_kernel(const float* __restrict__ pred, int pdpad, PatchGroup pg,
                                                     const int64_t* __restrict__ idx, int idx_ld, int j0, int cnt, int rows, float w,
-                                                    float* __restrict__ part, T* __restrict__ dpred, float* __restrict__ target_out, int vec) {
+                                                    float* __restrict__ part, T* __restrict__ dpred, float* __restrict__ target_out, int vec,
+                                                    int lpr, int gvec) {
     extern __shared__ __attribute__((aligned(16))) float mbuf[];
     __shared__ float red[WPB];
     const int lane = threadIdx.x & 63, wave = threadIdx.x >> 6;
+    const int rpw = 64 / lpr, sub = lane / lpr, sl = lane & (lpr - 1);
     const int pd = pg.C * pg.P * pg.P;
     const PatchDiv dv = patch_div(pg);
-    float* my = mbuf + (long)wave * pdpad;
+    float* my = mbuf + ((long)wave * rpw + sub) * pdpad;
     float acc = 0.f;
-    for (int r0 = blockIdx.x * WPB; r0 < rows; r0 += gridDim.x * WPB) {
-        const int row = r0 + wave;
+    for (long r0 = ((long)blockIdx.x * WPB + wave) * rpw; r0 < rows; r0 += (long)gridDim.x * WPB * rpw) {
+        const long row = r0 + sub;
         const bool live = row < rows;
         if (live) {
             int b, s, ph, pw, local;
-            patch_locate(pg, idx, idx_ld, j0, cnt, row, b, s, ph, pw, local);
+            patch_locate(pg, idx, idx_ld, j0, cnt, (int)row, b, s, ph, pw, local);
             const float* base = patch_base(pg, b, s, ph, pw);
-            for (int tb = 0; tb < pd; tb += 512) {
-                const int t0 = tb + lane;
-                float tv[8];
-                int e[8];
-#pragma unroll
-                for (int u = 0; u < 8; ++u) {
-                    if (tb + 64 * u >= pd) break;
-                    const int t = t0 + 64 * u;
-                    tv[u] = base[patch_off_t(pg, dv, min(t, pd - 1), e[u])];
+            if (gvec) {
+                const int np = pd >> 2;
+                for (int tb = 0; tb < np; tb += 8 * lpr) {
+                    f32x4 tv[8];
+                    int e[8];
+#pragma unroll
+                    for (int u = 0; u < 8; ++u) {
+                        if (tb + lpr * u >= np) break;
+                        const int t = tb + sl + lpr * u;
+                        tv[u] = *reinterpret_cast<const f32x4*>(base + patch_off_t(pg, dv, 4 * min(t, np - 1), e[u]));
+                    }
+#pragma unroll
+                    for (int u = 0; u < 8; ++u) {
+                        if (tb + lpr * u >= np) break;
+                        if (tb + sl + lpr * u < np) {
+#pragma unroll
+                            for (int k = 0; k < 4; ++k) my[e[u] + k * pg.C] = tv[u][k];
+                        }
+                    }
                 }
-#pragma unroll
-                for (int u = 0; u < 8; ++u) {
-                    if (tb + 64 * u >= pd) break;
-                    if (t0 + 64 * u < pd) my[e[u]] = tv[u];
+            } else {
+                for (int tb = 0; tb < pd; tb += 8 * lpr) {
+                    const int t0 = tb + sl;
+                    float tv[8];
+                    int e[8];
+#pragma unroll
+                    for (int u = 0; u < 8; ++u) {
+                        if (tb + lpr * u >= pd) break;
+                        const int t = t0 + lpr * u;
+                        tv[u] = base[patch_off_t(pg, dv, min(t, pd - 1), e[u])];
+                    }
+#pragma unroll
+                    for (int u = 0; u < 8; ++u) {
+                        if (tb + lpr * u >= pd) break;
+                        if (t0 + lpr * u < pd) my[e[u]] = tv[u];
+                    }
                 }
             }
         }
-        __syncthreads();
+        wave_lds_order();
         if (live) {
-            const float* pr = pred + (long)row * pdpad;
-            T* dp = dpred + (long)row * pdpad;
+            const float* pr = pred + row * pdpad;
+            T* dp = dpred + row * pdpad;
             if (vec) {
 #pragma unroll 4
-                for (int e = 4 * lane; e < pdpad; e += 256) {
+                for (int e = 4 * sl; e < pdpad; e += 4 * lpr) {
                     f32x4 d = {0.f, 0.f, 0.f, 0.f};
                     if (e < pd) {
                         const f32x4 t = *reinterpret_cast<const f32x4*>(my + e);
                         d = load4(pr + e) - t;
-                        if (target_out) store4<float>(target_out + (long)row * pd + e, t);
+                        if (target_out) store4<float>(target_out + row * pd + e, t);
                     }
                     acc += d[0] * d[0];
                     acc += d[1] * d[1];
@@ -1208,15 +1274,15 @@
                     store4<T>(dp + e, d * (2.f * w));
                 }
             } else {
-                for (int e = lane; e < pdpad; e += 64) {
+                for (int e = sl; e < pdpad; e += lpr) {
                     const float d = e < pd ? pr[e] - my[e] : 0.f;
-                    if (e < pd && target_out) target_out[(long)row * pd + e] = my[e];
+                    if (e < pd && target_out) target_out[row * pd + e] = my[e];
                     acc += d * d;
                     dp[e] = from_f32<T>(2.f * w * d);
                 }
             }
         }
-        __syncthreads();
+        wave_lds_order();
     }
     acc = wave_sum(acc);
     if (lane == 0) red[wave] = acc;
@@ -1264,7 +1330,7 @@
     if (count == 1 && stride == 1)
         reduce_vec_kernel<<<1, 1024, 0, st>>>(part, G, out, accumulate);
     else
-        reduce_rows_kernel<<<cdiv(count, 32), 1024, 0, st>>>(part, G, stride, count, out, accumulate);
+        reduce_rows_kernel<<<cdiv(count, 32), RED_THREADS, 0, st>>>(part, G, stride, count, out, accumulate);
     M3L_LAUNCH_CHECK();
     return 0;
 }
@@ -1283,8 +1349,8 @@
     M3L_CHECK(M > 0 && D > 0 && D % 4 == 0 && D <= 1024, "ln_bwd: bad shape M=%d D=%d (D must be a multiple of 4, <= 1024)", M, D);
     const int G = m3l_ln_bwd_blocks(M);
     {
-        ProfScope prof("ln_bwd", M, D, dy_dtype,
-                       (double)M * D * ((m3l_call_rb() ? 2.0 : 4.0) + (dy_dtype ? 2 : 4) + (dres ? (m3l_call_rb() ? 2 : 4) : 0) + (dx_out ? 4 : 0) + (dx_t_out ? (ct_dtype ? 2 : 4) : 0)), st);
+        const double ln_bytes = (double)M * D * ((m3l_call_rb() ? 2.0 : 4.0) + (dy_dtype ? 2 : 4) + (dres ? (m3l_call_rb() ? 2 : 4) : 0) + (dx_out ? 4 : 0) + (dx_t_out ? (ct_dtype ? 2 : 4) : 0));
+        ProfScope prof("ln_bwd", M, D, dy_dtype, 0.0, st, ln_bytes);
 #define LN_BWD(TD, TC, C, TX) ln_bwd_kernel<TD, TC, C, TX><<<G, 256, 0, st>>>((const TD*)dy, (const TX*)x, M, D, gamma, eps, dres, dx_out, (TC*)dx_t_out, part_ws)
 #define LN_BWD_C(TD, TC, TX) { if (D <= 256) LN_BWD(TD, TC, 1, TX); else if (D <= 512) LN_BWD(TD, TC, 2, TX); else LN_BWD(TD, TC, 4, TX); }
         if (m3l_call_rb()) {
@@ -1300,7 +1366,7 @@
     M3L_LAUNCH_CHECK();
     if (!dgamma && !dbeta && !dbias) return 0;
     ReduceSegs segs = {{dgamma, dbeta, dbias, nullptr}};
-    reduce_rows_seg_kernel<<<dim3(cdiv(D, 32), 3), 1024, 0, st>>>(part_ws, G, 3 * D, D, segs, accumulate);
+    reduce_rows_seg_kernel<<<dim3(cdiv(D, 32), 3), RED_THREADS, 0, st>>>(part_ws, G, 3 * D, D, segs, accumulate);
     M3L_LAUNCH_CHECK();
     return 0;
 }
@@ -1308,15 +1374,19 @@
 int m3l_reduce_rows_batch(const ReduceBatch* b, int accumulate, hipStream_t st) {
     if (b->count <= 0) return 0;
     M3L_CHECK(b->count <= M3L_REDUCE_BATCH_MAX && b->D > 0, "reduce_rows_batch: count=%d D=%d", b->count, b->D);
-    ProfScope prof("reduce_batch", b->count, b->D, 0, 0.0, st);
-    reduce_rows_batch_kernel<<<dim3(cdiv(b->D, 32), 3, b->count), 1024, 0, st>>>(*b, accumulate);
+    double bytes = 0.0;
+    for (int i = 0; i < b->count; ++i)
+        for (int k = 0; k < 3; ++k)
+            if (b->it[i].out[k]) bytes += ((double)b->it[i].G + 1.0) * b->D * 4;
+    ProfScope prof("reduce_batch", b->count, b->D, 0, 0.0, st, bytes);
+    reduce_rows_batch_kernel<<<dim3(cdiv(b->D, 32), 3, b->count), RED_THREADS, 0, st>>>(*b, accumulate);
     M3L_LAUNCH_CHECK();
     return 0;
 }
 
 int m3l_reduce_rows_seg3(const float* part, int G, int D, float* out0, float* out1, float* out2, int accumulate, hipStream_t st) {
     ReduceSegs segs = {{out0, out1, out2, nullptr}};
-    reduce_rows_seg_kernel<<<dim3(cdiv(D, 32), 3), 1024, 0, st>>>(part, G, 3 * D, D, segs, accumulate);
+    reduce_rows_seg_kernel<<<dim3(cdiv(D, 32), 3), RED_THREADS, 0, st>>>(part, G, 3 * D, D, segs, accumulate);
     M3L_LAUNCH_CHECK();
     return 0;
 }
@@ -1327,7 +1397,7 @@
     if (G > m3l_part_blocks()) G = m3l_part_blocks();
     const int rpb = cdiv(M, G);
     G = cdiv(M, rpb);
-    ProfScope prof("colsum", M, N, dtype, (double)M * N * (dtype ? 2 : 4), st);
+    ProfScope prof("colsum", M, N, dtype, 0.0, st, (double)M * N * (dtype ? 2 : 4) + 2.0 * G * N * 4);
     const int vec_ok = (ld % 4 == 0) && (N % 4 == 0) && (((unsigned long)Y) % 16 == 0) && (((unsigned long)part_ws) % 16 == 0);
     if (dtype == 1)
         colsum_kernel<bf16><<<G, 256, 0, st>>>((const bf16*)Y, M, N, ld, rpb, part_ws, vec_ok);
@@ -1484,7 +1554,7 @@
     const int G = part_grid(rows);
     tokens_assemble_bwd_kernel<<<G, 256, WPB * PL * sizeof(float), st>>>(dtok, B, D, n_img, n_tac > 0 ? n_tac : 1, k, d_img, d_tac, part_ws);
     M3L_LAUNCH_CHECK();
-    reduce_rows_kernel<<<cdiv(PL, 32), 1024, 0, st>>>(part_ws, G, PL, PL, dmod, accumulate);
+    reduce_rows_kernel<<<cdiv(PL, 32), RED_THREADS, 0, st>>>(part_ws, G, PL, PL, dmod, accumulate);
     M3L_LAUNCH_CHECK();
     return 0;
 }
@@ -1569,6 +1639,7 @@
 }
 
 int m3l_scale_by_dev(int dtype, const void* x, long count, const float* scale_dev, void* out, hipStream_t st) {
+    ProfScope prof("scale_by_dev", count, dtype, 0, 0.0, st, 2.0 * count * (dtype == 1 ? 2 : 4));
     if (dtype == 1)
         scale_by_dev_kernel<bf16><<<cdiv(count, 256), 256, 0, st>>>((const bf16*)x, count, scale_dev, (bf16*)out);
     else
@@ -1696,7 +1767,7 @@
 #undef PATCH_LN_BWD
     M3L_LAUNCH_CHECK();
     ReduceSegs segs = {{dgamma, dbeta, nullptr, nullptr}};
-    reduce_rows_seg_kernel<<<dim3(cdiv(pd, 32), 2), 1024, 0, st>>>(part_ws, G, 2 * pd, pd, segs, accumulate);
+    reduce_rows_seg_kernel<<<dim3(cdiv(pd, 32), 2), RED_THREADS, 0, st>>>(part_ws, G, 2 * pd, pd, segs, accumulate);
     M3L_LAUNCH_CHECK();
     return 0;
 }
@@ -1720,6 +1791,7 @@
     const int nslot = pg->nsrc;
     const int PL = (2 + nslot) * D;
     const int G = part_grid(rows);
+    ProfScope prof("embed_finalize_bwd", rows, D, dtype, 0.0, st, (double)rows * D * (8.0 + (dtype ? 2 : 4)) + 2.0 * G * PL * 4);
     if (dtype == 1)
         embed_finalize_bwd_kernel<bf16><<<G, 256, WPB * PL * sizeof(float), st>>>(dtok, L, E, rows, D, *pg, idx, idx_ld, j0, cnt, gamma, eps, (bf16*)dE, part_ws, nslot);
     else
@@ -1728,11 +1800,11 @@
     if (nslot <= 2) {
         float* dm = dmod + (long)mod0 * D;
         ReduceSegs segs = {{dgamma, dbeta, dm, nslot > 1 ? dm + D : nullptr}};
-        reduce_rows_seg_kernel<<<dim3(cdiv(D, 32), 2 + nslot), 1024, 0, st>>>(part_ws, G, PL, D, segs, accumulate);
+        reduce_rows_seg_kernel<<<dim3(cdiv(D, 32), 2 + nslot), RED_THREADS, 0, st>>>(part_ws, G, PL, D, segs, accumulate);
     } else {
-        reduce_rows_kernel<<<cdiv(D, 32), 1024, 0, st>>>(part_ws, G, PL, D, dgamma, accumulate);
-        reduce_rows_kernel<<<cdiv(D, 32), 1024, 0, st>>>(part_ws + D, G, PL, D, dbeta, accumulate);
-        reduce_rows_kernel<<<cdiv(nslot * D, 32), 1024, 0, st>>>(part_ws + 2 * D, G, PL, nslot * D, dmod + (long)mod0 * D, accumulate);
+        reduce_rows_kernel<<<cdiv(D, 32), RED_THREADS, 0, st>>>(part_ws, G, PL, D, dgamma, accumulate);
+        reduce_rows_kernel<<<cdiv(D, 32), RED_THREADS, 0, st>>>(part_ws + D, G, PL, D, dbeta, accumulate);
+        reduce_rows_kernel<<<cdiv(nslot * D, 32), RED_THREADS, 0, st>>>(part_ws + 2 * D, G, PL, nslot * D, dmod + (long)mod0 * D, accumulate);
     }
     M3L_LAUNCH_CHECK();
     return 0;
@@ -1743,6 +1815,7 @@
                       float* dec_in, hipStream_t st) {
     const long rows = (long)B * (nvis + nmask);
     M3L_CHECK(dd % 4 == 0, "unshuffle_fwd: dd=%d must be a multiple of 4", dd);
+    ProfScope prof("unshuffle_fwd", rows, dd, m3l_call_io() ? 1 : 0, 0.0, st, ((double)B * nvis * 4 + (double)rows * (m3l_call_io() ? 2 : 4)) * dd);
     if (m3l_call_io())
         unshuffle_fwd_kernel<bf16><<<cdiv(rows, WPB), 256, 0, st>>>(src, mask_token, unmasked, nvis, masked, nmask, B, dd, n_img, n_tac > 0 ? n_tac : 1, dmod,
                                                                      pos_img, pos_tac, reinterpret_cast<bf16*>(dec_in));
@@ -1766,6 +1839,8 @@
     const int vpw = cdiv((long)B * nvis, (long)G * WPB);
     const int N = nvis + nmask, nt = n_tac > 0 ? n_tac : 1;
     const size_t lds = WPB * PL * sizeof(float);
+    ProfScope prof("unshuffle_bwd", rows, dd, m3l_call_io() ? 1 : 0, 0.0, st,
+                   ((double)rows * (m3l_call_io() ? 2 : 4) + (double)B * nvis * 4) * dd + 2.0 * G * PL * 4);
 #define UNSH_BWD(C, TI) unshuffle_bwd_kernel<C, TI><<<G, 256, lds, st>>>((const TI*)dY, unmasked, nvis, B, N, dd, n_img, nt, nmod, rpw, vpw, dsrc, part_ws)
     if (m3l_call_io()) {
         if (dd <= 256) UNSH_BWD(1, bf16); else if (dd <= 512) UNSH_BWD(2, bf16); else UNSH_BWD(4, bf16);
@@ -1776,10 +1851,10 @@
     M3L_LAUNCH_CHECK();
     if (nmod <= 3) {
         ReduceSegs segs = {{dmask_token, ddmod, nmod > 1 ? ddmod + dd : nullptr, nmod > 2 ? ddmod + 2 * dd : nullptr}};
-        reduce_rows_seg_kernel<<<dim3(cdiv(dd, 32), 1 + nmod), 1024, 0, st>>>(part_ws, G, PL, dd, segs, accumulate);
+        reduce_rows_seg_kernel<<<dim3(cdiv(dd, 32), 1 + nmod), RED_THREADS, 0, st>>>(part_ws, G, PL, dd, segs, accumulate);
     } else {
-        reduce_rows_kernel<<<cdiv(dd, 32), 1024, 0, st>>>(part_ws, G, PL, dd, dmask_token, accumulate);
-        reduce_rows_kernel<<<cdiv(nmod * dd, 32), 1024, 0, st>>>(part_ws + dd, G, PL, nmod * dd, ddmod, accumulate);
+        reduce_rows_kernel<<<cdiv(dd, 32), RED_THREADS, 0, st>>>(part_ws, G, PL, dd, dmask_token, accumulate);
+        reduce_rows_kernel<<<cdiv(nmod * dd, 32), RED_THREADS, 0, st>>>(part_ws + dd, G, PL, nmod * dd, ddmod, accumulate);
     }
     M3L_LAUNCH_CHECK();
     return 0;
@@ -1802,6 +1877,7 @@
     const int rows = B * (cnt0 + cnt1);
     if (rows == 0) return 0;
     M3L_CHECK((D * (dtype ? 2 : 4)) % 16 == 0, "gather_rows2: rows of %d elements are not 16-byte pieces", D);
+    ProfScope prof("gather_rows2", rows, D, dtype, 0.0, st, 2.0 * rows * D * (dtype ? 2 : 4));
     if (dtype == 1)
         gather_rows2_kernel<bf16><<<ln_grid(rows), 256, 0, st>>>((const bf16*)src, N, D, idx, idx_ld, cnt0, cnt1, rows, (bf16*)dst0, (bf16*)dst1);
     else
@@ -1814,6 +1890,7 @@
     const int rows = B * (cnt0 + cnt1);
     if (rows == 0) return 0;
     M3L_CHECK((D * (dtype ? 2 : 4)) % 16 == 0, "scatter_rows2: rows of %d elements are not 16-byte pieces", D);
+    ProfScope prof("scatter_rows2", rows, D, dtype, 0.0, st, 2.0 * rows * D * (dtype ? 2 : 4));
     if (dtype == 1)
         scatter_rows2_kernel<bf16><<<ln_grid(rows), 256, 0, st>>>((const bf16*)src0, (const bf16*)src1, N, D, idx, idx_ld, cnt0, cnt1, rows, scale_dev,
                                                                   (bf16*)dst);
@@ -1844,16 +1921,22 @@
     if (rows == 0) return 0;
     const int pd = pg->C * pg->P * pg->P;
     const float w = weight / ((float)rows * (float)pd);
-    const int G = part_grid(rows);
     M3L_CHECK(pdpad >= pd, "mse: pdpad %d < patch dim %d", pdpad, pd);
+    int lpr = 1;
+    while (lpr < 64 && 4 * lpr < pdpad) lpr *= 2;
+    const int rpw = 64 / lpr;
+    const int G = part_grid(cdiv(rows, rpw));
     const int vec = pd % 4 == 0 && pdpad % 4 == 0 && aligned_to(pred, 16) && aligned_to(dpred, 4 * (dtype == 1 ? 2 : 4)) &&
                     (!target_out || aligned_to(target_out, 16));
-    const size_t lds = (size_t)WPB * pdpad * sizeof(float);
+    const size_t lds = (size_t)WPB * rpw * pdpad * sizeof(float);
     M3L_CHECK(lds <= 64 * 1024, "mse: padded patch dim %d too wide", pdpad);
+    int gvec = pg->P % 4 == 0 && pg->W % 4 == 0;
+    for (int i = 0; i < pg->nsrc; ++i) gvec = gvec && aligned_to(pg->src[i], 16);
+    ProfScope prof("mse", rows, pd, dtype, 0.0, st, (double)rows * (pd * (8.0 + (target_out ? 4 : 0)) + (double)pdpad * (dtype == 1 ? 2 : 4)));
     if (dtype == 1)
-        mse_kernel<bf16><<<G, 256, lds, st>>>(pred, pdpad, *pg, idx, idx_ld, j0, cnt, rows, w, part_ws, (bf16*)dpred, target_out, vec);
+        mse_kernel<bf16><<<G, 256, lds, st>>>(pred, pdpad, *pg, idx, idx_ld, j0, cnt, rows, w, part_ws, (bf16*)dpred, target_out, vec, lpr, gvec);
     else
-        mse_kernel<float><<<G, 256, lds, st>>>(pred, pdpad, *pg, idx, idx_ld, j0, cnt, rows, w, part_ws, (float*)dpred, target_out, vec);
+        mse_kernel<float><<<G, 256, lds, st>>>(pred, pdpad, *pg, idx, idx_ld, j0, cnt, rows, w, part_ws, (float*)dpred, target_out, vec, lpr, gvec);
     M3L_LAUNCH_CHECK();
     if (nblocks_out) *nblocks_out = G;
     return 0;
diff --git a/m3l_amd/csrc/mae_plan.hip b/m3l_amd/csrc/mae_plan.hip
--- a/m3l_amd/csrc/mae_plan.hip
+++ b/m3l_amd/csrc/mae_plan.hip
@@ -1570,6 +1570,20 @@
     return m3l_colsum(dtype, Y, M, N, ld, (float*)ws, out, 0, (hipStream_t)stream);
 }
 size_t m3l_op_colsum_ws_bytes(int N) { return (size_t)M3L_MAX_PARTIAL_BLOCKS * N * sizeof(float) + 256; }
+int m3l_op_reduce_rows_batch(int count, int D, const float* const* parts, const int* G, float* const* outs, int accumulate, void* stream) {
+    M3L_CHECK(count >= 0 && D > 0 && (count == 0 || (parts && G && outs)), "op_reduce_rows_batch: bad arguments (count %d, D %d)", count, D);
+    for (int i0 = 0; i0 < count; i0 += M3L_REDUCE_BATCH_MAX) {
+        ReduceBatch bt;
+        memset(&bt, 0, sizeof(bt));
+        bt.D = D;
+        for (int i = i0; i < count && i < i0 + M3L_REDUCE_BATCH_MAX; ++i) {
+            M3L_CHECK(parts[i] && G[i] > 0, "op_reduce_rows_batch: slab %d is empty", i);
+            bt.it[bt.count++] = ReduceBatchItem{parts[i], {outs[3 * i], outs[3 * i + 1], outs[3 * i + 2]}, G[i]};
+        }
+        if (m3l_reduce_rows_batch(&bt, accumulate, (hipStream_t)stream)) return 1;
+    }
+    return 0;
+}
 int m3l_op_prep_weight(int dtype, const float* src, int rows, int cols, void* dst, void* dstT, void* stream) {
     WeightPack pk;
     memset(&pk, 0, sizeof(pk));
```

Measured after the change: 75570 samples/s, median of 6. About the same (+0.4%).
